# buq2/camera_calibrator

Hardware: AMD Instinct MI355X
Metric: LM residuals/sec (2*N_obs per LM iteration), single-camera intrinsics BA (higher is better)
Workload: dtype f64; 1 GPU; BASELINE.json configs[2]: single-camera intrinsics, 1000 frames x 500 pts per GPU, radial-tangential distortion, Zhang init, reference solver options (calibrator.cpp:314-321); frames_total=1000, points_per_frame=500, observations_total=500000, parallelism=frame-sharded x1, exchange=none

## Files before the change

### camera_calibrator_amd/capi.py

```python
import ctypes as C
import os

import numpy as np

_HERE = os.path.dirname(os.path.abspath(__file__))
LIB_PATH = os.environ.get("CC_LIB_PATH", os.path.join(_HERE, "libcc_hip.so"))

K_NAMES = ["sweep", "decide", "elim", "solve", "allreduce", "update", "reduce"]
TERMINATION = {0: "NO_CONVERGENCE", 1: "GRADIENT", 2: "PARAMETER", 3: "FUNCTION",
               4: "FAILURE_INVALID_STEPS", 5: "MIN_RADIUS", 6: "FAILURE_EXCHANGE"}


class CcError(RuntimeError):
    pass


class Options(C.Structure):
    _fields_ = [
        ("max_iterations", C.c_int32),
        ("use_nonmonotonic_steps", C.c_int32),
        ("max_consecutive_nonmonotonic_steps", C.c_int32),
        ("jacobi_scaling", C.c_int32),
        ("max_consecutive_invalid_steps", C.c_int32),
        ("check_interval", C.c_int32),
        ("function_tolerance", C.c_double),
        ("gradient_tolerance", C.c_double),
        ("parameter_tolerance", C.c_double),
        ("initial_radius", C.c_double),
        ("max_radius", C.c_double),
        ("min_radius", C.c_double),
        ("min_relative_decrease", C.c_double),
        ("min_lm_diagonal", C.c_double),
        ("max_lm_diagonal", C.c_double),
        ("use_graph", C.c_int32),
        ("profile_kernels", C.c_int32),
    ]


class Iteration(C.Structure):
    _fields_ = [
        ("cost", C.c_double),
        ("cost_change", C.c_double),
        ("model_cost_change", C.c_double),
        ("relative_decrease", C.c_double),
        ("gradient_max_norm", C.c_double),
        ("step_norm", C.c_double),
        ("radius", C.c_double),
        ("accepted", C.c_int32),
        ("valid", C.c_int32),
    ]


class IntrStartOptions(C.Structure):
    _fields_ = [
        ("centre", C.c_double * 2),
        ("theta_lo", C.c_double),
        ("theta_hi", C.c_double),
        ("candidates", C.c_int32),
        ("search_views", C.c_int32),
        ("refine_iterations", C.c_int32),
    ]


class IntrStartReport(C.Structure):
    _fields_ = [
        ("centre", C.c_double * 2),
        ("r_max", C.c_double),
        ("focal", C.c_double),
        ("best_candidate", C.c_int32),
        ("candidates_qualified", C.c_int32),
        ("views", C.c_int64),
        ("views_searched", C.c_int64),
        ("views_invalid", C.c_int64),
    ]


class Summary(C.Structure):
    _fields_ = [
        ("iterations", C.c_int32),
        ("successful_steps", C.c_int32),
        ("termination", C.c_int32),
        ("log_len", C.c_int32),
        ("initial_cost", C.c_double),
        ("final_cost", C.c_double),
        ("seconds", C.c_double),
        ("log", C.POINTER(Iteration)),
        ("log_capacity", C.c_int32),
        ("sweeps", C.c_int32),
        ("kernel_ms", C.c_double * 8),
        ("kernel_launches", C.c_int32 * 8),
        ("kernel_idle_ms", C.c_double * 8),
        ("kernel_idle_launches", C.c_int32 * 8),
    ]


EXPORTED_SYMBOLS = [
    "cc_options_init", "cc_last_error", "cc_version", "cc_device_count", "cc_release_caches", "cc_parallel_for", "cc_parallel_parts", "cc_host_pool_threads", "cc_last_call_solver_status",
    "cc_intrinsics_create", "cc_intrinsics_destroy", "cc_intrinsics_set_state",
    "cc_intrinsics_reset", "cc_intrinsics_get_state", "cc_intrinsics_eval",
    "cc_intrinsics_solve", "cc_intrinsics_solver_form", "cc_intrinsics_solver_status", "cc_intrinsics_profile_sweep", "cc_intrinsics_profile_solve", "cc_intrinsics_optimize", "cc_intrinsics_estimate", "cc_intrinsics_estimate_views", "cc_intrinsics_optimize_views", "cc_host_staging_acquire", "cc_host_staging_release", "cc_last_call_timing", "cc_comm_get_unique_id",
    "cc_intrinsics_comm_init", "cc_intrinsics_exchange_export", "cc_intrinsics_exchange_attach", "cc_partition_frames", "cc_distort", "cc_undistort",
    "cc_rig_create", "cc_rig_destroy", "cc_rig_set_state", "cc_rig_reset", "cc_rig_solve",
    "cc_rig_get_state", "cc_rig_solver_form", "cc_rig_solver_status", "cc_rig_eval", "cc_rig_optimize", "cc_rig_comm_init", "cc_rig_exchange_export", "cc_rig_exchange_attach", "cc_rigk_create",
    "cc_rigk_set_intrinsics", "cc_rigk_get_intrinsics", "cc_rigk_create_per_camera", "cc_rigk_set_camera_intrinsics",
    "cc_rigk_get_camera_intrinsics", "cc_rigk_set_model", "cc_rigk_get_model", "cc_rigk_set_camera_model", "cc_rigk_get_camera_model", "cc_rigk_estimate_start", "cc_rigk_start_points", "cc_rigk_estimate_start_bearing", "cc_rigk_start_bearings", "cc_zhang_init", "cc_intrinsics_optimize_multi", "cc_rig_optimize_multi", "cc_rig_optimize_frames", "cc_rig_optimize_columns",
    "cc_rig_set_inner_iterations", "cc_rig_inner_pass", "cc_rig_inner_status",
    "cc_rig_start_options_init", "cc_rig_estimate_start", "cc_rig_start_views", "cc_rig_estimate",
    "cc_intrinsics_batch_create", "cc_intrinsics_batch_destroy", "cc_intrinsics_batch_set_state", "cc_intrinsics_batch_get_state",
    "cc_intrinsics_batch_solve", "cc_intrinsics_batch_optimize", "cc_intrinsics_batch_estimate",
    "cc_intrinsics_set_huber", "cc_intrinsics_obs_cost", "cc_intrinsics_optimize_views_huber", "cc_intrinsics_estimate_views_huber",
    "cc_intrinsics_batch_set_huber", "cc_intrinsics_batch_estimate_huber",
    "cc_intrinsics_set_model", "cc_intrinsics_get_model", "cc_intrinsics_optimize_views_model", "cc_intrinsics_estimate_views_model",
    "cc_distort_fisheye", "cc_undistort_fisheye",
    "cc_intrinsics_batch_set_model", "cc_intrinsics_batch_get_model", "cc_intrinsics_batch_estimate_model",
    "cc_intr_start_options_init", "cc_intrinsics_estimate_start_fisheye", "cc_intrinsics_start_scores", "cc_intrinsics_estimate_views_start",
]
MODEL_RADTAN, MODEL_FISHEYE = 0, 1
MODEL_MIXED = 2
HARNESS_SYMBOLS = [
    "cc_generator_create", "cc_generator_destroy", "cc_generator_set_k", "cc_generator_set_distortion",
    "cc_generator_set_noise", "cc_generator_planar", "cc_generator_points", "cc_rig_scenario", "cc_affine_to_qt",
]

_lib = None


def lib():
    global _lib
    if _lib is None:
        if not os.path.exists(LIB_PATH):
            raise CcError(f"{LIB_PATH} is missing: build it with __graft_entry__.build() "
                          "(hipcc --offload-arch=gfx950); there is no CPU fallback")
        _lib = C.CDLL(LIB_PATH)
        _lib.cc_last_error.restype = C.c_char_p
        _lib.cc_version.restype = C.c_char_p
        _lib.cc_generator_create.restype = C.c_void_p
        _lib.cc_generator_planar.restype = C.c_int64
        _lib.cc_generator_points.restype = C.c_int64
    return _lib


def _check(rc):
    if rc != 0:
        raise CcError(f"cc error {rc}: {lib().cc_last_error().decode()}")


def _p(a, t):
    return a.ctypes.data_as(C.POINTER(t))


def _f32(a):
    return np.ascontiguousarray(a, dtype=np.float32)


def _f64(a):
    return np.ascontiguousarray(a, dtype=np.float64)


def default_options(**kw):
    o = Options()
    lib().cc_options_init(C.byref(o))
    for k, v in kw.items():
        if not hasattr(o, k):
            raise AttributeError(k)
        setattr(o, k, v)
    return o


def intr_start_options(**kw):
    o = IntrStartOptions()
    lib().cc_intr_start_options_init(C.byref(o))
    for k, v in kw.items():
        if not hasattr(o, k):
            raise AttributeError(k)
        if k == "centre":
            o.centre[0], o.centre[1] = float(v[0]), float(v[1])
        else:
            setattr(o, k, v)
    return o


def device_count():
    return int(lib().cc_device_count())


def partition_frames(frame_offsets, nranks):
    off = np.ascontiguousarray(frame_offsets, dtype=np.int64)
    first = np.zeros(nranks + 1, dtype=np.int64)
    _check(lib().cc_partition_frames(C.c_int64(len(off) - 1), _p(off, C.c_int64), C.c_int32(nranks),
                                     _p(first, C.c_int64)))
    return first


def _summary_dict(s, log):
    names = [f[0] for f in Iteration._fields_]
    return {
        "iterations": s.iterations, "successful_steps": s.successful_steps,
        "termination": TERMINATION.get(s.termination, str(s.termination)),
        "initial_cost": s.initial_cost, "final_cost": s.final_cost, "seconds": s.seconds,
        "sweeps": s.sweeps,
        "kernel_ms": {K_NAMES[i]: s.kernel_ms[i] for i in range(len(K_NAMES))},
        "kernel_launches": {K_NAMES[i]: s.kernel_launches[i] for i in range(len(K_NAMES))},
        "kernel_idle_ms": {K_NAMES[i]: s.kernel_idle_ms[i] for i in range(len(K_NAMES))},
        "kernel_idle_launches": {K_NAMES[i]: s.kernel_idle_launches[i] for i in range(len(K_NAMES))},
        "log": [{k: getattr(log[i], k) for k in names} for i in range(s.log_len)],
    }


class IntrinsicsProblem:

    def __init__(self, frame_offsets, uv, xyz, device=0):
        self._h = C.c_void_p()
        off = np.ascontiguousarray(frame_offsets, dtype=np.int64)
        self.n_frames = len(off) - 1
        self.n_obs = int(off[-1])
        uv, xyz = _f32(uv), _f32(xyz)
        assert uv.size == 2 * self.n_obs and xyz.size == 3 * self.n_obs
        _check(lib().cc_intrinsics_create(C.c_int32(device), C.c_int64(self.n_frames),
                                          _p(off, C.c_int64), _p(uv, C.c_float), _p(xyz, C.c_float),
                                          C.byref(self._h)))

    def close(self):
        if self._h:
            lib().cc_intrinsics_destroy(self._h)
            self._h = C.c_void_p()

    def __del__(self):
        try:
            self.close()
        except Exception:
            pass

    def set_state(self, intr, q, t, const_mask=0):
        intr, q, t = _f64(intr), _f64(q), _f64(t)
        assert intr.size == 9 and q.size == 4 * self.n_frames and t.size == 3 * self.n_frames
        _check(lib().cc_intrinsics_set_state(self._h, _p(intr, C.c_double), C.c_uint32(const_mask),
                                             _p(q, C.c_double), _p(t, C.c_double)))

    def reset(self):
        _check(lib().cc_intrinsics_reset(self._h))

    def get_state(self):
        intr = np.zeros(9)
        q = np.zeros((self.n_frames, 4))
        t = np.zeros((self.n_frames, 3))
        _check(lib().cc_intrinsics_get_state(self._h, _p(intr, C.c_double), _p(q, C.c_double),
                                             _p(t, C.c_double)))
        return intr, q, t

    def eval(self, want_blocks=True):
        blocks = np.zeros((self.n_frames, 16, 16)) if want_blocks else None
        cost = C.c_double()
        _check(lib().cc_intrinsics_eval(self._h, _p(blocks, C.c_double) if want_blocks else None,
                                        C.byref(cost)))
        return cost.value, blocks

    def solve(self, options=None, log_capacity=1024):
        opt = options if options is not None else default_options()
        log = (Iteration * max(1, log_capacity))()
        s = Summary()
        s.log = C.cast(log, C.POINTER(Iteration))
        s.log_capacity = log_capacity
        _check(lib().cc_intrinsics_solve(self._h, C.byref(opt), C.byref(s)))
        return _summary_dict(s, log)

    def solve_lean(self, options):
        s = getattr(self, "_lean_summary", None)
        if s is None:
            s = self._lean_summary = Summary()
            s.log = None
            s.log_capacity = 0
        _check(lib().cc_intrinsics_solve(self._h, C.byref(options), C.byref(s)))
        return s.iterations

    def set_huber(self, a):
        _check(lib().cc_intrinsics_set_huber(self._h, C.c_double(a)))

    def set_model(self, model):
        _check(lib().cc_intrinsics_set_model(self._h, C.c_int32(model)))

    def get_model(self):
        return int(lib().cc_intrinsics_get_model(self._h))

    def obs_cost(self):
        out = np.zeros(self.n_obs)
        _check(lib().cc_intrinsics_obs_cost(self._h, _p(out, C.c_double)))
        return out

    def estimate_start_fisheye(self, **options):
        o = intr_start_options(**options)
        intr, q, t = np.zeros(9), np.zeros((self.n_frames, 4)), np.zeros((self.n_frames, 3))
        r = IntrStartReport()
        _check(lib().cc_intrinsics_estimate_start_fisheye(self._h, C.byref(o), _p(intr, C.c_double), _p(q, C.c_double),
                                                          _p(t, C.c_double), C.byref(r)))
        report = {k: getattr(r, k) for k, _ in IntrStartReport._fields_ if k != "centre"}
        report["centre"] = (r.centre[0], r.centre[1])
        return intr, q, t, report

    def start_scores(self):
        f, score, qualified = np.zeros(64), np.zeros(64), np.full(64, -1, dtype=np.int32)
        _check(lib().cc_intrinsics_start_scores(self._h, _p(f, C.c_double), _p(score, C.c_double), _p(qualified, C.c_int32)))
        n = int((qualified >= 0).sum())
        return f[:n].copy(), score[:n].copy(), qualified[:n].copy()

    def profile_sweep(self, n=50):
        ms = C.c_double()
        _check(lib().cc_intrinsics_profile_sweep(self._h, C.c_int32(n), C.byref(ms)))
        return ms.value

    def solver_form(self):
        return int(lib().cc_intrinsics_solver_form(self._h))

    def solver_status(self):
        form, reruns = C.c_int32(), C.c_int32()
        note = C.create_string_buffer(2048)
        _check(lib().cc_intrinsics_solver_status(self._h, C.byref(form), C.byref(reruns), note, 2048))
        return form.value, reruns.value, note.value.decode()

    def profile_solve(self, options=None, n=20):
        options = options if options is not None else default_options()
        ms, sw = C.c_double(), C.c_int32()
        _check(lib().cc_intrinsics_profile_solve(self._h, C.byref(options), C.c_int32(n), C.byref(ms), C.byref(sw)))
        return ms.value, sw.value

    def comm_init(self, unique_id, rank, nranks):
        buf = (C.c_uint8 * 128).from_buffer_copy(bytes(unique_id))
        _check(lib().cc_intrinsics_comm_init(self._h, buf, C.c_int32(rank), C.c_int32(nranks)))

    def exchange_export(self):
        buf = (C.c_uint8 * 64)()
        _check(lib().cc_intrinsics_exchange_export(self._h, buf))
        return bytes(buf)

    def exchange_attach(self, rank, handles):
        blob = b"".join(bytes(x) for x in handles)
        assert len(blob) == 64 * len(handles)
        buf = (C.c_uint8 * len(blob)).from_buffer_copy(blob)
        _check(lib().cc_intrinsics_exchange_attach(self._h, C.c_int32(rank), C.c_int32(len(handles)), buf))


def comm_get_unique_id():
    buf = (C.c_uint8 * 128)()
    _check(lib().cc_comm_get_unique_id(buf))
    return bytes(buf)


def _views(off, uv, xyz):
    F = len(off) - 1
    parts_uv = [np.array(uv.reshape(-1, 2)[off[f]:off[f + 1]], dtype=np.float32, order="C") for f in range(F)]
    parts_xyz = [np.array(xyz.reshape(-1, 3)[off[f]:off[f + 1]], dtype=np.float32, order="C") for f in range(F)]
    fp = C.POINTER(C.c_float)
    uv_views = (fp * F)(*[a.ctypes.data_as(fp) for a in parts_uv])
    xyz_views = (fp * F)(*[a.ctypes.data_as(fp) for a in parts_xyz])
    counts = np.ascontiguousarray(np.diff(off), dtype=np.int64)
    return uv_views, xyz_views, counts, (parts_uv, parts_xyz)


def intrinsics_optimize(frame_offsets, uv, xyz, intr, q, t, const_mask=0, options=None, device=0,
                        log_capacity=1024, devices=None, views=False, huber_a=0.0, model=0):
    off = np.ascontiguousarray(frame_offsets, dtype=np.int64)
    F = len(off) - 1
    uv, xyz = _f32(uv), _f32(xyz)
    intr, q, t = _f64(intr).copy(), _f64(q).copy(), _f64(t).copy()
    opt = options if options is not None else default_options()
    log = (Iteration * max(1, log_capacity))()
    s = Summary()
    s.log = C.cast(log, C.POINTER(Iteration))
    s.log_capacity = log_capacity
    if model != 0:
        if devices is not None:
            raise ValueError("model is for one device only")
        uv_views, xyz_views, counts, _keep = _views(off, uv, xyz)
        _check(lib().cc_intrinsics_optimize_views_model(C.byref(opt), C.c_int32(device), C.c_int64(F), uv_views, xyz_views,
                                                        _p(counts, C.c_int64), _p(intr, C.c_double), C.c_uint32(const_mask),
                                                        _p(q, C.c_double), _p(t, C.c_double), C.byref(s), C.c_double(huber_a),
                                                        C.c_int32(model)))
        return intr, q, t, _summary_dict(s, log)
    if not huber_a <= 0:
        if devices is not None:
            raise ValueError("huber_a is for one device only")
        uv_views, xyz_views, counts, _keep = _views(off, uv, xyz)
        _check(lib().cc_intrinsics_optimize_views_huber(C.byref(opt), C.c_int32(device), C.c_int64(F), uv_views, xyz_views,
                                                        _p(counts, C.c_int64), _p(intr, C.c_double), C.c_uint32(const_mask),
                                                        _p(q, C.c_double), _p(t, C.c_double), C.byref(s), C.c_double(huber_a)))
        return intr, q, t, _summary_dict(s, log)
    if devices is not None:
        devs = np.ascontiguousarray(devices, dtype=np.int32)
        _check(lib().cc_intrinsics_optimize_multi(C.byref(opt), C.c_int32(len(devs)), _p(devs, C.c_int32), C.c_int64(F),
                                                  _p(off, C.c_int64), _p(uv, C.c_float), _p(xyz, C.c_float),
                                                  _p(intr, C.c_double), C.c_uint32(const_mask),
                                                  _p(q, C.c_double), _p(t, C.c_double), C.byref(s)))
        return intr, q, t, _summary_dict(s, log)
    if views:
        uv_views, xyz_views, counts, _keep = _views(off, uv, xyz)
        _check(lib().cc_intrinsics_optimize_views(C.byref(opt), C.c_int32(device), C.c_int64(F), uv_views, xyz_views,
                                                  _p(counts, C.c_int64), _p(intr, C.c_double), C.c_uint32(const_mask),
                                                  _p(q, C.c_double), _p(t, C.c_double), C.byref(s)))
        return intr, q, t, _summary_dict(s, log)
    _check(lib().cc_intrinsics_optimize(C.byref(opt), C.c_int32(device), C.c_int64(F),
                                        _p(off, C.c_int64), _p(uv, C.c_float), _p(xyz, C.c_float),
                                        _p(intr, C.c_double), C.c_uint32(const_mask),
                                        _p(q, C.c_double), _p(t, C.c_double), C.byref(s)))
    return intr, q, t, _summary_dict(s, log)


def intrinsics_estimate(frame_offsets, uv, xyz, distortion5=None, const_mask=0, options=None, device=0, log_capacity=1024,
                        views=False, huber_a=0.0, model=0, start="zhang", start_options=None):
    if start not in ("zhang", "fisheye"):
        raise ValueError(f"start must be 'zhang' or 'fisheye', not {start!r}")
    if start == "zhang" and start_options is not None:
        raise ValueError("start_options belong to start='fisheye'")
    off = np.ascontiguousarray(frame_offsets, dtype=np.int64)
    F = len(off) - 1
    uv, xyz = _f32(uv), _f32(xyz)
    opt = options if options is not None else default_options()
    log = (Iteration * max(1, log_capacity))()
    s = Summary()
    s.log = C.cast(log, C.POINTER(Iteration))
    s.log_capacity = log_capacity
    K = np.zeros(9, dtype=np.float32)
    intr, q, t = np.zeros(9), np.zeros((F, 4)), np.zeros((F, 3))
    d5 = _f64(distortion5) if distortion5 is not None else None
    if start == "fisheye":
        so = start_options if isinstance(start_options, IntrStartOptions) else intr_start_options(**(start_options or {}))
        uv_views, xyz_views, counts, _keep = _views(off, uv, xyz)
        _check(lib().cc_intrinsics_estimate_views_start(C.byref(opt), C.c_int32(device), C.c_int64(F), uv_views, xyz_views,
                                                        _p(counts, C.c_int64), _p(d5, C.c_double) if d5 is not None else None,
                                                        C.c_uint32(const_mask), _p(K, C.c_float), _p(intr, C.c_double),
                                                        _p(q, C.c_double), _p(t, C.c_double), C.byref(s), C.c_double(huber_a),
                                                        C.c_int32(model), C.byref(so)))
        return K.reshape(3, 3), intr, q, t, _summary_dict(s, log)
    if model != 0:
        uv_views, xyz_views, counts, _keep = _views(off, uv, xyz)
        _check(lib().cc_intrinsics_estimate_views_model(C.byref(opt), C.c_int32(device), C.c_int64(F), uv_views, xyz_views,
                                                        _p(counts, C.c_int64), _p(d5, C.c_double) if d5 is not None else None,
                                                        C.c_uint32(const_mask), _p(K, C.c_float), _p(intr, C.c_double),
                                                        _p(q, C.c_double), _p(t, C.c_double), C.byref(s), C.c_double(huber_a),
                                                        C.c_int32(model)))
        return K.reshape(3, 3), intr, q, t, _summary_dict(s, log)
    if not huber_a <= 0:
        uv_views, xyz_views, counts, _keep = _views(off, uv, xyz)
        _check(lib().cc_intrinsics_estimate_views_huber(C.byref(opt), C.c_int32(device), C.c_int64(F), uv_views, xyz_views,
                                                        _p(counts, C.c_int64), _p(d5, C.c_double) if d5 is not None else None,
                                                        C.c_uint32(const_mask), _p(K, C.c_float), _p(intr, C.c_double),
                                                        _p(q, C.c_double), _p(t, C.c_double), C.byref(s), C.c_double(huber_a)))
        return K.reshape(3, 3), intr, q, t, _summary_dict(s, log)
    if views:
        uv_views, xyz_views, counts, _keep = _views(off, uv, xyz)
        _check(lib().cc_intrinsics_estimate_views(C.byref(opt), C.c_int32(device), C.c_int64(F), uv_views, xyz_views,
                                                  _p(counts, C.c_int64), _p(d5, C.c_double) if d5 is not None else None,
                                                  C.c_uint32(const_mask), _p(K, C.c_float), _p(intr, C.c_double),
                                                  _p(q, C.c_double), _p(t, C.c_double), C.byref(s)))
        return K.reshape(3, 3), intr, q, t, _summary_dict(s, log)
    _check(lib().cc_intrinsics_estimate(C.byref(opt), C.c_int32(device), C.c_int64(F), _p(off, C.c_int64), _p(uv, C.c_float),
                                        _p(xyz, C.c_float), _p(d5, C.c_double) if d5 is not None else None,
                                        C.c_uint32(const_mask), _p(K, C.c_float), _p(intr, C.c_double), _p(q, C.c_double),
                                        _p(t, C.c_double), C.byref(s)))
    return K.reshape(3, 3), intr, q, t, _summary_dict(s, log)


def _batch_layout(problems):
    poff, foff, uvs, xyzs = [0], [0], [], []
    for off, uv, xyz in problems:
        off = np.ascontiguousarray(off, dtype=np.int64)
        uv, xyz = _f32(uv).reshape(-1, 2), _f32(xyz).reshape(-1, 3)
        assert off[0] == 0 and len(uv) == off[-1] and len(xyz) == off[-1]
        foff.extend((off[1:] + foff[-1]).tolist())
        poff.append(poff[-1] + len(off) - 1)
        uvs.append(uv)
        xyzs.append(xyz)
    uv = np.ascontiguousarray(np.concatenate(uvs), dtype=np.float32) if uvs else np.zeros((0, 2), np.float32)
    xyz = np.ascontiguousarray(np.concatenate(xyzs), dtype=np.float32) if xyzs else np.zeros((0, 3), np.float32)
    return np.array(poff, dtype=np.int64), np.array(foff, dtype=np.int64), uv, xyz


def _batch_summaries(B, log_capacity):
    logs = [(Iteration * max(1, log_capacity))() for _ in range(B)]
    ss = (Summary * B)()
    for p in range(B):
        ss[p].log = C.cast(logs[p], C.POINTER(Iteration))
        ss[p].log_capacity = log_capacity
    return ss, logs


class IntrinsicsBatch:

    def __init__(self, problems, device=0):
        self._h = C.c_void_p()
        self.problem_offsets, self.frame_offsets, uv, xyz = _batch_layout(problems)
        self.n_problems = len(self.problem_offsets) - 1
        self.n_frames = int(self.problem_offsets[-1])
        _check(lib().cc_intrinsics_batch_create(C.c_int32(device), C.c_int64(self.n_problems), _p(self.problem_offsets, C.c_int64),
                                                _p(self.frame_offsets, C.c_int64), _p(uv, C.c_float), _p(xyz, C.c_float),
                                                C.byref(self._h)))

    def close(self):
        if self._h:
            lib().cc_intrinsics_batch_destroy(self._h)
            self._h = C.c_void_p()

    def __del__(self):
        try:
            self.close()
        except Exception:
            pass

    def _split(self, a, width):
        a = a.reshape(-1, width)
        return [a[self.problem_offsets[p]:self.problem_offsets[p + 1]].copy() for p in range(self.n_problems)]

    def set_state(self, intr, q, t, const_mask=None):
        intr = _f64(np.asarray(intr, dtype=np.float64).reshape(-1))
        q = _f64(np.concatenate([np.asarray(x, dtype=np.float64).reshape(-1, 4) for x in q]) if isinstance(q, (list, tuple)) else q)
        t = _f64(np.concatenate([np.asarray(x, dtype=np.float64).reshape(-1, 3) for x in t]) if isinstance(t, (list, tuple)) else t)
        assert intr.size == 9 * self.n_problems and q.size == 4 * self.n_frames and t.size == 3 * self.n_frames
        mask = np.zeros(self.n_problems, dtype=np.uint32) if const_mask is None else np.ascontiguousarray(const_mask, dtype=np.uint32)
        assert mask.size == self.n_problems
        _check(lib().cc_intrinsics_batch_set_state(self._h, _p(intr, C.c_double), _p(mask, C.c_uint32), _p(q, C.c_double),
                                                   _p(t, C.c_double)))

    def set_huber(self, a_list):
        if a_list is None:
            _check(lib().cc_intrinsics_batch_set_huber(self._h, None))
            return
        a = _f64(np.asarray(a_list, dtype=np.float64).reshape(-1))
        assert a.size == self.n_problems
        _check(lib().cc_intrinsics_batch_set_huber(self._h, _p(a, C.c_double)))

    def set_model(self, model):
        _check(lib().cc_intrinsics_batch_set_model(self._h, C.c_int32(model)))

    def get_model(self):
        model = C.c_int32(-1)
        _check(lib().cc_intrinsics_batch_get_model(self._h, C.byref(model)))
        return int(model.value)

    def get_state(self):
        intr = np.zeros((self.n_problems, 9))
        q = np.zeros((self.n_frames, 4))
        t = np.zeros((self.n_frames, 3))
        _check(lib().cc_intrinsics_batch_get_state(self._h, _p(intr, C.c_double), _p(q, C.c_double), _p(t, C.c_double)))
        return intr, self._split(q, 4), self._split(t, 3)

    def solve(self, options=None, log_capacity=1024):
        opt = options if options is not None else default_options()
        ss, logs = _batch_summaries(self.n_problems, log_capacity)
        _check(lib().cc_intrinsics_batch_solve(self._h, C.byref(opt), ss))
        return [_summary_dict(ss[p], logs[p]) for p in range(self.n_problems)]

    def solve_lean(self, options):
        ss = getattr(self, "_lean", None)
        if ss is None:
            ss = self._lean = (Summary * self.n_problems)()
        _check(lib().cc_intrinsics_batch_solve(self._h, C.byref(options), ss))
        return [ss[p].iterations for p in range(self.n_problems)]


def intrinsics_batch_optimize(problems, intr, q, t, const_mask=None, options=None, device=0, log_capacity=1024, model=0):
    if model != 0:
        h = IntrinsicsBatch(problems, device=device)
        try:
            h.set_model(model)
            h.set_state(intr, q, t, const_mask)
            ss = h.solve(options, log_capacity)
            io, qs, ts = h.get_state()
        finally:
            h.close()
        return io, qs, ts, ss
    poff, foff, uv, xyz = _batch_layout(problems)
    B = len(poff) - 1
    intr = _f64(np.asarray(intr, dtype=np.float64).reshape(-1)).copy()
    q = _f64(np.concatenate([np.asarray(x, dtype=np.float64).reshape(-1, 4) for x in q])).copy()
    t = _f64(np.concatenate([np.asarray(x, dtype=np.float64).reshape(-1, 3) for x in t])).copy()
    mask = np.zeros(B, dtype=np.uint32) if const_mask is None else np.ascontiguousarray(const_mask, dtype=np.uint32)
    opt = options if options is not None else default_options()
    ss, logs = _batch_summaries(B, log_capacity)
    _check(lib().cc_intrinsics_batch_optimize(C.byref(opt), C.c_int32(device), C.c_int64(B), _p(poff, C.c_int64), _p(foff, C.c_int64),
                                              _p(uv, C.c_float), _p(xyz, C.c_float), _p(intr, C.c_double), _p(mask, C.c_uint32),
                                              _p(q, C.c_double), _p(t, C.c_double), ss))
# ... 551 lines not shown
```

### camera_calibrator_amd/csrc/cc_intrinsics.hip

```cpp
#include "cc_common.hpp"
#include "cc_device.hpp"
#include "cc_intrinsics_dev.hpp"
#include "cc_intrinsics_persist.hpp"


#include <algorithm>
#include <chrono>
#include <climits>
#include <cstdlib>
#include <cstring>
#include <vector>

namespace cc {

__global__ __launch_bounds__(kSweepThreads, 4) void k_intr_sweep(IntrDev P, int flags) {
  extern __shared__ __attribute__((aligned(16))) char smem_raw[];
  double* s_stage = reinterpret_cast<double*>(smem_raw);
  double* s_blk = s_stage;
  double* sm = s_stage + 4 * kStageDoublesPerWave;
  const int tid = threadIdx.x, lane = tid & 63, wave = tid >> 6;
  const int T = P.T;
  const int64_t f = (int64_t)blockIdx.x / T;
  const int tile = (int)(blockIdx.x - f * T);
  const bool in_solve = (flags & 1) != 0, restart = (flags & 2) != 0;
// ... 488 lines not shown
      }
#pragma unroll
      for (int u = 0; u < 16; ++u) Gs[u * 256 + tid] = a[u];
      __syncthreads();
    }
    const double* Gl = Gs + g * 256;
    auto gsum = [&](int idx) { return T > 1 ? Gl[idx] : G[idx]; };
    double fail = 0.0;
    double gv[5];
#pragma unroll
    for (int r = 0; r < 5; ++r) gv[r] = gsum(gi[r]);
    const double gpe = gsum((9 + l6) * 16 + 15);
    const double* qf = P.pose + ((size_t)cur * P.F + (valid ? f : 0)) * 8;
    const double qw = qf[0], qx = qf[1], qy = qf[2], qz = qf[3];
    const int col = l < 9 ? l : 15;
    double w[6];
#pragma unroll
    for (int i = 0; i < 6; ++i) w[i] = gsum((9 + i) * 16 + col);
    if (valid) {
      double s[6], L[21];
#pragma unroll
      for (int i = 0; i < 6; ++i)
#pragma unroll
        for (int j = 0; j <= i; ++j) L[tri(i, j)] = gsum((9 + i) * 16 + 9 + j);
      if (phase == 0) {
#pragma unroll
        for (int i = 0; i < 6; ++i) s[i] = jac ? 1.0 / (1.0 + sqrt(L[tri(i, i)])) : 1.0;
        if (l < 6) P.sp[f * 8 + l] = jac ? 1.0 / (1.0 + sqrt(gsum((9 + l) * 17))) : 1.0;
      } else {
#pragma unroll
        for (int i = 0; i < 6; ++i) s[i] = P.sp[f * 8 + i];
      }
#pragma unroll
      for (int i = 0; i < 6; ++i)
#pragma unroll
        for (int j = 0; j <= i; ++j) L[tri(i, j)] = s[i] * L[tri(i, j)] * s[j];
#pragma unroll
      for (int i = 0; i < 6; ++i) L[tri(i, i)] += clampd(L[tri(i, i)], mn, mx) * inv_radius;
      bool ok = true;
      double Li[6];
#pragma unroll
      for (int j = 0; j < 6; ++j) {
        double d = L[tri(j, j)];
#pragma unroll
        for (int k = 0; k < j; ++k) d -= L[tri(j, k)] * L[tri(j, k)];
        ok = ok && (d > 0.0) && isfinite(d);
        const double inv = rsqrt_pos(d);
        L[tri(j, j)] = d * inv;
        Li[j] = inv;
#pragma unroll
        for (int i = j + 1; i < 6; ++i) {
          double a = L[tri(i, j)];
#pragma unroll
          for (int k = 0; k < j; ++k) a -= L[tri(i, k)] * L[tri(j, k)];
          L[tri(i, j)] = a * inv;
        }
      }
      if (!ok) fail = 1.0;
      if (l < 10) {
        const double sc = l < 9 ? s_ss[l] : 1.0;
        double z[6], y[6];
#pragma unroll
        for (int i = 0; i < 6; ++i) {
          double a = s[i] * w[i] * sc;
#pragma unroll
          for (int k = 0; k < i; ++k) a -= L[tri(i, k)] * z[k];
          z[i] = a * Li[i];
        }
#pragma unroll
        for (int i = 5; i >= 0; --i) {
          double a = z[i];
#pragma unroll
          for (int k = i + 1; k < 6; ++k) a -= L[tri(k, i)] * y[k];
          y[i] = a * Li[i];
        }
#pragma unroll
        for (int i = 0; i < 6; ++i) {
          Zs[g][i * 10 + l] = z[i];
          P.Y[f * kYStride + i * 10 + l] = y[i];
        }
      }
    }
    __syncthreads();
    if (valid) {
#pragma unroll
      for (int r = 0; r < 5; ++r) {
        double zz = 0.0;
#pragma unroll
        for (int i = 0; i < 6; ++i) zz += Zs[g][i * 10 + zj[r]] * Zs[g][i * 10 + zk[r]];
        acc[r] += sa[r] * gv[r] * sb[r] - (use_z[r] ? zz : 0.0);
      }
      {
        const int base16 = (threadIdx.x & 63) & ~15;
        double g6[6];
#pragma unroll
        for (int i = 0; i < 6; ++i) g6[i] = __shfl(gpe, base16 + i, 64);
        const double q4[4] = {qw, qx, qy, qz};
        gacc = fmax(gacc, pose_grad_proj_max(q4, g6));
      }
      facc += fail;
    }
    __syncthreads();
  }
#pragma unroll
  for (int r = 0; r < 5; ++r)
    if (l * 5 + r != PC_FAIL && l * 5 + r != PC_GMAXP) red[g][l * 5 + r] = acc[r];
  gacc = row16_max(gacc);
  if (l == 0) { red[g][PC_FAIL] = facc; red[g][PC_GMAXP] = gacc; }
  __syncthreads();
  if (tid < kPartialCols) {
    double a = 0.0;
    if (tid == PC_GMAXP) { for (int g2 = 0; g2 < 16; ++g2) a = fmax(a, red[g2][tid]); }
    else { for (int g2 = 0; g2 < 16; ++g2) a += red[g2][tid]; }
    if (kFused)
      __hip_atomic_store(reinterpret_cast<unsigned long long*>(P.partial) + blockIdx.x * kPartialCols + tid,
                         (unsigned long long)__double_as_longlong(a), __ATOMIC_RELAXED, __HIP_MEMORY_SCOPE_AGENT);
    else
      P.partial[blockIdx.x * kPartialCols + tid] = a;
  }
  }
  if (!kFused) return;

  asm volatile("s_waitcnt vmcnt(0)" ::: "memory");
  __syncthreads();
  if (tid == 0) {
    const unsigned prev = __hip_atomic_fetch_add(P.arrive, 1u, __ATOMIC_RELAXED, __HIP_MEMORY_SCOPE_AGENT);
    s_last = prev + 1u == gridDim.x;
  }
  __syncthreads();
  if (!s_last) return;
  if (tid == 0) __hip_atomic_store(P.arrive, 0u, __ATOMIC_RELAXED, __HIP_MEMORY_SCOPE_AGENT);
  double* sv = &red[0][0];
  double* s_part = &red[2][0];
  if (!stop) {
    const bool active = true;
    {
      const int col = tid % kPartialCols, grp = tid / kPartialCols;
      const int nblk = (int)gridDim.x;
      if (grp < 3) {
        const unsigned long long* src = reinterpret_cast<const unsigned long long*>(P.partial) + col;
        double v[22];
#pragma unroll
        for (int u = 0; u < 22; ++u) {
          const int b = grp + 3 * u;
          v[u] = b < nblk ? __longlong_as_double((long long)__hip_atomic_load(src + b * kPartialCols, __ATOMIC_RELAXED, __HIP_MEMORY_SCOPE_AGENT)) : 0.0;
        }
        double a = 0.0;
        if (col == PC_GMAXP) {
#pragma unroll
          for (int u = 0; u < 22; ++u) a = fmax(a, v[u]);
        } else {
#pragma unroll
          for (int u = 0; u < 22; ++u) a += v[u];
        }
        s_part[grp * kPartialCols + col] = a;
      }
    }
    __syncthreads();
    if (tid < kVecSolve) {
      double a = 0.0;
      if (tid < kPartialCols) {
        if (tid != PC_GMAXP) a = (s_part[tid] + s_part[kPartialCols + tid]) + s_part[2 * kPartialCols + tid];
      } else if (tid == kPartialCols + P.rank) {
        a = fmax(fmax(s_part[PC_GMAXP], s_part[kPartialCols + PC_GMAXP]), s_part[2 * kPartialCols + PC_GMAXP]);
      }
      sv[tid] = a;
    }
    __syncthreads();
    if (MODE == 3 && active) {
      __shared__ int s_ok2;
      const unsigned long long epoch = P.x.seq[0] + 1ull;
      p2p_post(P.x, 0, epoch, P.rank, P.nranks, sv, kVecSolve);
      const double a = p2p_collect(P.x, 0, epoch, P.rank, P.nranks, kVecSolve, &s_ok2);
      exchange_ok = s_ok2 != 0;
      if (tid < kVecSolve) sv[tid] = exchange_ok ? a : 0.0;
      if (tid == 0) P.x.seq[0] = epoch;
      __syncthreads();
    }
  }
  if (tid != 0) return;
  LmCtl c = s_ctl;
  cc_iteration* e = s_logged ? &s_log : nullptr;
  if (!exchange_ok) { c.done = 1; c.term = CC_FAILURE_EXCHANGE; }
  else if (!stop) intr_solve_step(P, sv, c, e, o_in);
  if (publish == 2) return;
  if (e && c.log_len <= P.log_cap) P.log[c.log_len - 1] = *e;
  *P.ctl = c;
  *P.ctl_next = c;
  if (publish) publish_to_host(P, c);
}

constexpr int kSolveThreads = 8 * kPartialCols;

template <int MODE>
__global__ __launch_bounds__(kSolveThreads) void k_intr_solve(IntrDev P, int nblk, int publish) {
  static_assert(MODE == 1 || MODE == 2, "single-GPU and mailbox solves are fused into k_intr_decide_elim");
  __shared__ double sv[kVecSolve];
  __shared__ double s_part[8][kPartialCols];
  const int tid = threadIdx.x;
  const LmCtl* cn = P.ctl_next;
  const bool active = !cn->done && cn->phase != 0;
  if (MODE == 1) {
    const int col = tid % kPartialCols, grp = tid / kPartialCols;
    double v[8];
#pragma unroll
    for (int u = 0; u < 8; ++u) {
      const int b = grp + 8 * u;
      v[u] = b < nblk ? P.partial[b * kPartialCols + col] : 0.0;
    }
    double a = 0.0;
    if (active) {
      if (col == PC_GMAXP) a = fmax(fmax(fmax(v[0], v[1]), fmax(v[2], v[3])), fmax(fmax(v[4], v[5]), fmax(v[6], v[7])));
      else a = ((v[0] + v[1]) + (v[2] + v[3])) + ((v[4] + v[5]) + (v[6] + v[7]));
    }
    s_part[grp][col] = a;
    if (tid >= kPartialCols && tid < kVecSolve) sv[tid] = 0.0;
    __syncthreads();
    if (tid < kPartialCols) {
      double a2 = 0.0;
      if (tid == PC_GMAXP) {
        if (active) for (int g2 = 0; g2 < 8; ++g2) a2 = fmax(a2, s_part[g2][tid]);
        sv[kPartialCols + P.rank] = a2;
        sv[tid] = 0.0;
      } else {
        if (active)
          a2 = ((s_part[0][tid] + s_part[1][tid]) + (s_part[2][tid] + s_part[3][tid])) +
               ((s_part[4][tid] + s_part[5][tid]) + (s_part[6][tid] + s_part[7][tid]));
        sv[tid] = a2;
      }
    }
    __syncthreads();
    if (tid < kVecSolve) P.vec_solve[tid] = sv[tid];
    return;
  }
  if (tid < kVecSolve) sv[tid] = P.vec_solve[tid];
  __syncthreads();
  if (tid != 0) return;
  LmCtl c = *cn;
  if (active) {
    cc_iteration* e = (c.log_len > 0 && c.log_len <= P.log_cap) ? &P.log[c.log_len - 1] : nullptr;
    cc_iteration rec;
    if (e) rec = *e;
    const LmOpts o = *P.opts;
    intr_solve_step(P, sv, c, e ? &rec : nullptr, o);
    if (e && rec.accepted) e->gradient_max_norm = rec.gradient_max_norm;
  }
  *P.ctl = c;
  *P.ctl_next = c;
  if (publish) publish_to_host(P, c);
}

__global__ __launch_bounds__(64) void k_intr_flag_exchange(IntrDev P, double mine, double* out, int* ok) {
  __shared__ double s_post[16];
  __shared__ int s_ok;
  const int tid = threadIdx.x;
  if (tid < 16) s_post[tid] = tid == 0 ? mine : 0.0;
  __syncthreads();
  const unsigned long long epoch = P.x.seq[1] + 1ull;
  p2p_post(P.x, 1, epoch, P.rank, P.nranks, s_post, 16);
  const double a = p2p_collect(P.x, 1, epoch, P.rank, P.nranks, 16, &s_ok);
  if (tid == 0) { *out = a; P.x.seq[1] = epoch; *ok = s_ok; }
}

__global__ __launch_bounds__(256) void k_intr_reset(IntrDev P, const double* init_intr, const double* init_pose) {
  const int64_t i = (int64_t)blockIdx.x * blockDim.x + threadIdx.x;
  if (i < P.F * 8) P.pose[i] = init_pose[i];
  if (i < 16) P.intr[i] = init_intr[i];
  if (i < (int64_t)(sizeof(LmCtl) / sizeof(double))) {
    reinterpret_cast<double*>(P.ctl)[i] = 0.0;
    reinterpret_cast<double*>(P.ctl_next)[i] = 0.0;
  }
  if (i == 0) *P.arrive = 0u;
}

}

#include "cc_intrinsics_huber.hpp"
#include "cc_intrinsics_fisheye.hpp"

#include "cc_solve_host.hpp"

struct cc_intrinsics : cc::SolveHost {
  cc::IntrDev d{};
  int64_t F = 0, N = 0;
  int elim_blocks = 1;
  void* arena = nullptr;
  bool arena_cached = false;
  size_t extra_bytes = 0;
  char* extra = nullptr;
  bool one_shot = false;
  bool no_obs_upload = false;
  double* init_intr = nullptr;
  double* init_pose = nullptr;
  bool have_state = false;
  cc::LmOpts* h_opts = nullptr;
  bool ctl_fresh = false;
  bool reset_pending = false;
  bool persist_ok = false;
  bool persist_x_ok = false;
  int p_resident = 0;
  cc::PersistDev pq{};
  uint32_t p_epoch = 0;
  size_t p_box_bytes = 0;
  double huber_a = 0.0;
  int model = CC_MODEL_RADTAN;
  void* start_work = nullptr;
  size_t start_work_bytes = 0;
  int start_candidates = 0;
  const double* start_srec = nullptr;
  const double* start_view = nullptr;
  int64_t start_searched = 0;
  bool start_marks = false;
  bool own_sweep() const { return huber_a > 0.0 || model != CC_MODEL_RADTAN; }
};

namespace cc {

static void exchange_release(cc_intrinsics* h) {
  mailbox_release(&h->mailbox);
  h->d.x = P2pDev{};
  h->exchange = false;
}

static void launch_sweep(cc_intrinsics* h, bool profile, int flags = 0) {
  Probe p(h, CC_K_SWEEP, profile);
  flags |= 4;
  if (h->model == CC_MODEL_FISHEYE)
    hipLaunchKernelGGL(k_intr_sweep_fisheye, dim3((unsigned)(h->F * h->d.T)), dim3(kSweepThreads), kSweepLdsBytes, h->stream, h->d, flags, h->huber_a);
  else if (h->huber_a > 0.0)
    hipLaunchKernelGGL(k_intr_sweep_huber, dim3((unsigned)(h->F * h->d.T)), dim3(kSweepThreads), kSweepLdsBytes, h->stream, h->d, flags, h->huber_a);
  else
    hipLaunchKernelGGL(k_intr_sweep, dim3((unsigned)(h->F * h->d.T)), dim3(kSweepThreads), kSweepLdsBytes, h->stream, h->d, flags);
}

static void launch_reset(cc_intrinsics* h) {
  const unsigned blocks = (unsigned)((h->F * 8 + 255) / 256);
  hipLaunchKernelGGL(k_intr_reset, dim3(blocks), dim3(256), 0, h->stream, h->d, h->init_intr, h->init_pose);
}

static int enqueue_round(cc_intrinsics* h, bool profile, bool initial, bool publish, bool restart = false) {
  const int pub = (publish ? 1 : 0) | (restart ? 4 : 0);
  const int sweep_flags = 1 | (restart ? 2 : 0);
  struct RoundCount { cc_intrinsics* h; ~RoundCount() { h->enq_round++; } } count_round{h};
  if (h->comm) {
    if (!initial) {
      { Probe p(h, CC_K_SOLVE, profile, -1); hipLaunchKernelGGL(k_intr_solve<1>, dim3(1), dim3(kSolveThreads), 0, h->stream, h->d, h->elim_blocks, 0); }
      { Probe p(h, CC_K_ALLREDUCE, profile, -1); if (int rc = comm_allreduce_sum(h->comm, h->d.vec_solve, kVecSolve, h->stream)) return rc; }
      { Probe p(h, CC_K_SOLVE, profile, -1); hipLaunchKernelGGL(k_intr_solve<2>, dim3(1), dim3(kSolveThreads), 0, h->stream, h->d, h->elim_blocks, 0); }
    }
    launch_sweep(h, profile, 1);
    { Probe p(h, CC_K_DECIDE, profile); hipLaunchKernelGGL(k_intr_stats_reduce, dim3(1), dim3(256), 0, h->stream, h->d); }
    { Probe p(h, CC_K_ALLREDUCE, profile); if (int rc = comm_allreduce_sum(h->comm, h->d.vec_decide, 16, h->stream)) return rc; }
    { Probe p(h, CC_K_ELIM, profile); hipLaunchKernelGGL(k_intr_decide_elim<2>, dim3(h->elim_blocks), dim3(256), 0, h->stream, h->d, 0); }
    return 0;
  }
  launch_sweep(h, profile, sweep_flags);
  Probe p(h, CC_K_ELIM, profile);
  if (h->exchange) hipLaunchKernelGGL(k_intr_decide_elim<3>, dim3(h->elim_blocks), dim3(256), 0, h->stream, h->d, pub);
  else hipLaunchKernelGGL(k_intr_decide_elim<0>, dim3(h->elim_blocks), dim3(256), 0, h->stream, h->d, pub);
  return 0;
}

static int flush_reset(cc_intrinsics* h) {
  if (!h->reset_pending) return 0;
  launch_reset(h);
  CC_HIP(hipGetLastError());
  h->reset_pending = false;
  return 0;
}

static int read_ctl(cc_intrinsics* h, LmCtl* c) {
  if (int rc = flush_reset(h)) return rc;
  CC_HIP(hipMemcpyAsync(h->h_ctl, h->d.ctl_next, sizeof(LmCtl), hipMemcpyDeviceToHost, h->stream));
  CC_HIP(hipStreamSynchronize(h->stream));
  *c = *h->h_ctl;
  return 0;
}

static int wait_chunk(cc_intrinsics* h, LmCtl* c) {
  return wait_published(h, nullptr, c, nullptr, "the solver", [=] { return read_ctl(h, c); });
}

static int wait_solve(cc_intrinsics* h, LmCtl* c) {
  return wait_published_tagged(h, c, "the solver", [=] { return read_ctl(h, c); });
}

}

namespace cc {
int intr_create_impl(cc_intrinsics* h, const int64_t* off, const float* uv, const float* xyz);
static thread_local bool g_create_one_shot = false;
static thread_local bool g_create_no_obs = false;
static thread_local size_t g_create_extra = 0;
struct OneShotCreate {
  OneShotCreate(size_t extra, bool no_obs = false) { g_create_one_shot = true; g_create_extra = extra; g_create_no_obs = no_obs; }
  ~OneShotCreate() { g_create_one_shot = false; g_create_extra = 0; g_create_no_obs = false; }
};
static double ms_since(std::chrono::steady_clock::time_point t0) { return std::chrono::duration<double, std::milli>(std::chrono::steady_clock::now() - t0).count(); }
}

extern "C" {

void cc_intrinsics_destroy(cc_intrinsics* h);

int cc_intrinsics_create(int32_t device, int64_t F, const int64_t* off, const float* uv,
                         const float* xyz, cc_intrinsics** out) {
  using namespace cc;
  if (!out || !off || F <= 0) return fail(CC_ERR_BAD_ARGUMENT, "cc_intrinsics_create: bad arguments");
  if (off[0] != 0) return fail(CC_ERR_BAD_ARGUMENT, "frame_offsets[0] must be 0");
  for (int64_t f = 0; f < F; ++f)
    if (off[f + 1] < off[f]) return fail(CC_ERR_BAD_ARGUMENT, "frame_offsets must be non-decreasing");
  const int64_t N = off[F];
  if (F >= ((int64_t)1 << 28) || N >= ((int64_t)1 << 40))
    return fail(CC_ERR_BAD_ARGUMENT, "cc_intrinsics_create: problem too large (frames < 2^28, observations < 2^40)");
  if (N > 0 && (!uv || !xyz) && !cc::g_create_no_obs) return fail(CC_ERR_BAD_ARGUMENT, "uv/xyz are NULL");
  if (int rc = select_device(device)) return rc;
  cc_intrinsics* h = new cc_intrinsics();
  h->device = device; h->F = F; h->N = N;
  h->one_shot = cc::g_create_one_shot;
  h->no_obs_upload = cc::g_create_no_obs;
  h->extra_bytes = cc::g_create_extra;
  const int rc_init = cc::intr_create_impl(h, off, uv, xyz);
  if (rc_init != CC_OK) {
    cc_intrinsics_destroy(h);
    return rc_init;
  }
  *out = h;
  return CC_OK;
}

int cc_intrinsics_exchange_export(cc_intrinsics* h, uint8_t handle[64]) {
  using namespace cc;
  if (h && handle && h->huber_a > 0.0) return fail(CC_ERR_STATE, "cc_intrinsics_exchange_export: the handle has a Huber loss set (one device only)");
  if (h && handle && h->model != CC_MODEL_RADTAN) return fail(CC_ERR_STATE, "cc_intrinsics_exchange_export: the handle has the fisheye model set (one device only)");
  if (int rc = exchange_export_begin(h, handle, "cc_intrinsics_exchange_export")) return rc;
  h->d.x = P2pDev{};
  return mailbox_export(&h->mailbox, kVecSolve, 16, handle);
}

int cc_intrinsics_exchange_attach(cc_intrinsics* h, int32_t rank, int32_t nranks, const uint8_t* handles) {
  using namespace cc;
  if (!h || !handles || rank < 0 || nranks < 1 || rank >= nranks || nranks > kP2pMaxRanks)
    return fail(CC_ERR_BAD_ARGUMENT, "cc_intrinsics_exchange_attach: bad arguments (nranks must be 1..%d)", kP2pMaxRanks);
  if (h->huber_a > 0.0) return fail(CC_ERR_STATE, "cc_intrinsics_exchange_attach: the handle has a Huber loss set (one device only)");
  if (h->model != CC_MODEL_RADTAN) return fail(CC_ERR_STATE, "cc_intrinsics_exchange_attach: the handle has the fisheye model set (one device only)");
  if (!h->mailbox.local) return fail(CC_ERR_STATE, "cc_intrinsics_exchange_attach: call cc_intrinsics_exchange_export first");
  if (h->comm) return fail(CC_ERR_STATE, "cc_intrinsics_exchange_attach: an RCCL communicator is already attached");
  CC_HIP(hipSetDevice(h->device));
  drop_graphs(h);
  if (int rc = mailbox_attach(&h->mailbox, rank, nranks, handles, &h->d.x)) return rc;
  h->d.rank = rank;
  h->d.nranks = nranks;
  h->exchange = true;
  h->persist_x_ok = false;
  if (h->persist_ok) {
    int ndev = 1;
    if (hipGetDeviceCount(&ndev) != hipSuccess || ndev < 1) ndev = 1;
    const int co = getenv("CC_INTR_CO_RESIDENT") ? std::max(1, atoi(getenv("CC_INTR_CO_RESIDENT"))) : (nranks + ndev - 1) / ndev;
    h->persist_x_ok = (int64_t)(h->pq.G + 1) * co <= h->p_resident;
  }
  if (nranks > 1) {
    double* d_out = nullptr;
    int* d_ok = nullptr;
    CC_HIP(hipMalloc(&d_out, sizeof(double)));
    CC_HIP(hipMalloc(&d_ok, sizeof(int)));
    hipLaunchKernelGGL(k_intr_flag_exchange, dim3(1), dim3(64), 0, h->stream, h->d, h->persist_x_ok ? 1.0 : 0.0, d_out, d_ok);
    double sum = 0.0;
    int ok = 0;
    const hipError_t e1 = hipMemcpyAsync(&sum, d_out, sizeof(double), hipMemcpyDeviceToHost, h->stream);
    const hipError_t e2 = hipMemcpyAsync(&ok, d_ok, sizeof(int), hipMemcpyDeviceToHost, h->stream);
    const hipError_t e3 = hipStreamSynchronize(h->stream);
    hipFree(d_out);
    hipFree(d_ok);
    CC_HIP(e1); CC_HIP(e2); CC_HIP(e3);
    if (!ok) return fail(CC_ERR_COMM, "cc_intrinsics_exchange_attach: a peer rank did not attach within 10 s");
    h->persist_x_ok = sum == (double)nranks;
  }
  return CC_OK;
}

}

namespace cc {
int intr_create_impl(cc_intrinsics* h, const int64_t* off, const float* uv, const float* xyz) {
  const int64_t F = h->F, N = h->N;
  if (int rc = stream_get(h->device, &h->stream)) return rc;
  IntrDev& d = h->d;
  d.F = F; d.N = N; d.rank = 0; d.nranks = 1; d.mask = 0;
  {
    const int64_t per_frame = F > 0 ? (N + F - 1) / F : 0;
    int64_t T = std::min<int64_t>((per_frame + 2 * kSweepThreads - 1) / (2 * kSweepThreads), 256 / std::max<int64_t>(F, 1));
    if (const char* env = getenv("CC_SWEEP_TILES")) T = atoi(env);
    d.T = (int32_t)std::max<int64_t>(1, std::min<int64_t>(T, 8));
    d.tpad_ = 0;
    if (F * d.T >= (int64_t)INT32_MAX)
      return fail(CC_ERR_BAD_ARGUMENT, "cc_intrinsics_create: %lld frames x %d sweep tiles exceed the launch grid", (long long)F, (int)d.T);
  }
  const size_t FT = (size_t)F * d.T;
  const size_t n1 = (size_t)std::max<int64_t>(N, 1);
  size_t cursor = 0;
  auto take = [&](size_t bytes) { const size_t at = cursor; cursor += (bytes + 255) & ~(size_t)255; return at; };
  d.log_cap = 4096;
  const size_t o_intr = take(2 * 16 * sizeof(double));
  const size_t o_pose = take((size_t)2 * F * 8 * sizeof(double));
  const size_t o_stats = take(FT * kStatsCols * sizeof(double));
  const size_t o_hd0 = take(FT * 16 * sizeof(double));
  const size_t o_sp = take((size_t)F * 8 * sizeof(double));
  const size_t o_Y = take((size_t)F * kYStride * sizeof(double));
  const size_t o_partial = take((size_t)kElimMaxBlocks * kPartialCols * sizeof(double));
  const size_t o_vs = take(kVecSolve * sizeof(double));
  const size_t o_vd = take(16 * sizeof(double));
  const size_t o_ds = take(16 * sizeof(double));
  const size_t o_ss = take(16 * sizeof(double));
  const size_t o_ctl = take(sizeof(LmCtl));
  const size_t o_ctln = take(sizeof(LmCtl));
  const size_t o_sync = take(64);
  const size_t o_opts = take(sizeof(LmOpts));
  const size_t o_iintr = take(16 * sizeof(double));
  const size_t o_ipose = take((size_t)F * 8 * sizeof(double));
  int p_teams = 0;
  const bool want_persist = d.T == 1 && !(getenv("CC_INTR_PERSIST") && atoi(getenv("CC_INTR_PERSIST")) == 0);
  if (want_persist) {
    for (int t = 1; t <= kPMaxTeams && !p_teams; t *= 2) {
      int resident = 0;
      if (int rc = persist_resident_workgroups(h->device, t, &resident)) return rc;
      if ((F + t - 1) / t + 1 <= resident && (F + t - 1) / t <= kPMaxWorkers) { p_teams = t; h->p_resident = resident; }
    }
    if (const char* e = getenv("CC_INTR_PERSIST_TEAMS")) {
      const int t = atoi(e);
      int resident = 0;
      if ((t == 1 || t == 2 || t == 4) && !persist_resident_workgroups(h->device, t, &resident) && (F + t - 1) / t + 1 <= resident && (F + t - 1) / t <= kPMaxWorkers) { p_teams = t; h->p_resident = resident; }
    }
  }
  const int64_t PG = p_teams ? (F + p_teams - 1) / p_teams : 1;
  const size_t pgn = (size_t)PG;
  const size_t o_pbox0 = cursor;
  const size_t o_sbox = take(pgn * 2 * kPStatCols * sizeof(unsigned long long));
  const size_t o_pbox = take(pgn * 2 * kPartialCols * sizeof(unsigned long long));
  const size_t o_rbox = take(pgn * 2 * kPartialCols * sizeof(unsigned long long));
  const size_t o_lbox = take((size_t)2 * kPartialCols * sizeof(unsigned long long));
  const size_t o_xbox = take(kPBcastWords * sizeof(unsigned long long));
  const size_t o_pfail = take(64);
  h->p_box_bytes = cursor - o_pbox0;
  const size_t zeroed = cursor;
  const size_t o_blocks = take((size_t)2 * FT * 256 * sizeof(double));
  const size_t o_log = take((size_t)d.log_cap * sizeof(cc_iteration));
  const size_t o_uv = take(n1 * 2 * sizeof(float));
  const size_t o_xyz = take(n1 * 3 * sizeof(float));
  const size_t o_off = take((size_t)(F + 1) * sizeof(int64_t));
  const size_t o_extra = take(h->extra_bytes);
  if (int rc = arena_get(h->device, cursor, &h->arena, &h->arena_cached)) return rc;
  char* base = static_cast<char*>(h->arena);
  h->extra = h->extra_bytes ? base + o_extra : nullptr;
  CC_HIP(hipMemsetAsync(base, 0, zeroed, h->stream));
  if (N > 0 && !h->no_obs_upload) {
    CC_HIP(hipMemcpyAsync(base + o_uv, uv, (size_t)N * 2 * sizeof(float), hipMemcpyHostToDevice, h->stream));
    CC_HIP(hipMemcpyAsync(base + o_xyz, xyz, (size_t)N * 3 * sizeof(float), hipMemcpyHostToDevice, h->stream));
  }
  CC_HIP(hipMemcpyAsync(base + o_off, off, (size_t)(F + 1) * sizeof(int64_t), hipMemcpyHostToDevice, h->stream));
  if (!h->one_shot) CC_HIP(hipStreamSynchronize(h->stream));
  d.uv = reinterpret_cast<const float*>(base + o_uv);
  d.xyz = reinterpret_cast<const float*>(base + o_xyz);
  d.off = reinterpret_cast<const int64_t*>(base + o_off);
  d.intr = reinterpret_cast<double*>(base + o_intr);
  d.pose = reinterpret_cast<double*>(base + o_pose);
  d.blocks = reinterpret_cast<double*>(base + o_blocks);
  d.stats = reinterpret_cast<double*>(base + o_stats);
  d.hd0 = reinterpret_cast<double*>(base + o_hd0);
  d.sp = reinterpret_cast<double*>(base + o_sp);
  d.Y = reinterpret_cast<double*>(base + o_Y);
  d.partial = reinterpret_cast<double*>(base + o_partial);
  d.vec_solve = reinterpret_cast<double*>(base + o_vs);
  d.vec_decide = reinterpret_cast<double*>(base + o_vd);
  d.ds = reinterpret_cast<double*>(base + o_ds);
  d.ss = reinterpret_cast<double*>(base + o_ss);
  d.ctl = reinterpret_cast<LmCtl*>(base + o_ctl);
  d.ctl_next = reinterpret_cast<LmCtl*>(base + o_ctln);
  d.arrive = reinterpret_cast<unsigned*>(base + o_sync);
  d.pub_seq = reinterpret_cast<unsigned long long*>(base + o_sync + 8);
  d.opts = reinterpret_cast<LmOpts*>(base + o_opts);
  d.log = reinterpret_cast<cc_iteration*>(base + o_log);
  h->init_intr = reinterpret_cast<double*>(base + o_iintr);
  h->init_pose = reinterpret_cast<double*>(base + o_ipose);
  d.init_intr = h->init_intr;
  d.init_pose = h->init_pose;
  static_assert(16 + sizeof(LmCtl) <= 192 && sizeof(LmCtl) <= 160 && sizeof(LmOpts) <= 160, "one cached 512-byte pinned block holds all three");
  h->pinned = pinned_block_get();
  if (!h->pinned) return fail(CC_ERR_HIP, "hipHostMalloc failed");
  h->host_pub = reinterpret_cast<volatile unsigned long long*>(h->pinned);
  h->h_ctl = reinterpret_cast<LmCtl*>(static_cast<char*>(h->pinned) + 192);
  h->h_opts = reinterpret_cast<LmOpts*>(static_cast<char*>(h->pinned) + 352);
  h->host_pub[0] = 0ull;
  static_assert((kPubTaggedAt + kPubWords) * 8 <= (int)kPinnedBlockBytes && kPubTaggedAt * 8 >= 512, "the tagged publication lies behind the three blocks");
  for (int i = 0; i < kPubWords; ++i) h->host_pub[kPubTaggedAt + i] = 0ull;
  h->pub_count = 0;
  {
    void* dev_view = nullptr;
    CC_HIP(hipHostGetDevicePointer(&dev_view, h->pinned, 0));
    d.host_pub = reinterpret_cast<unsigned long long*>(dev_view);
  }
  h->pq.sbox = reinterpret_cast<unsigned long long*>(base + o_sbox);
  h->pq.pbox = reinterpret_cast<unsigned long long*>(base + o_pbox);
  h->pq.rbox = reinterpret_cast<unsigned long long*>(base + o_rbox);
  h->pq.xbox = reinterpret_cast<unsigned long long*>(base + o_xbox);
  h->pq.fail = reinterpret_cast<unsigned*>(base + o_pfail);
  h->pq.lbox = reinterpret_cast<unsigned long long*>(base + o_lbox);
  h->pq.G = (int32_t)PG;
  h->pq.teams = p_teams;
  h->p_epoch = 0;
  h->persist_ok = p_teams != 0;
  h->elim_blocks = (int)std::min<int64_t>(kElimMaxBlocks, (F + 15) / 16);
  CC_HIP(hipFuncSetAttribute(reinterpret_cast<const void*>(k_intr_sweep),
                             hipFuncAttributeMaxDynamicSharedMemorySize, kSweepLdsBytes));
  CC_HIP(hipFuncSetAttribute(reinterpret_cast<const void*>(k_intr_sweep_huber),
                             hipFuncAttributeMaxDynamicSharedMemorySize, kSweepLdsBytes));
  CC_HIP(hipFuncSetAttribute(reinterpret_cast<const void*>(k_intr_sweep_fisheye),
                             hipFuncAttributeMaxDynamicSharedMemorySize, kSweepLdsBytes));
  return CC_OK;
}
}

extern "C" {

void cc_intrinsics_destroy(cc_intrinsics* h) {
  if (h) cc::last_call_status_record(h->ran_form >= 0 ? h->ran_form : cc_intrinsics_solver_form(h), h->form_reruns, h->form_note);
  if (!h) return;
  hipSetDevice(h->device);
  bool stream_ok = true;
  if (h->stream) {
    hipStreamCaptureStatus cap = hipStreamCaptureStatusNone;
    stream_ok = hipStreamSynchronize(h->stream) == hipSuccess &&
                hipStreamIsCapturing(h->stream, &cap) == hipSuccess && cap == hipStreamCaptureStatusNone;
    (void)hipGetLastError();
  }
  cc::drop_graphs(h);
  for (auto e : h->events) hipEventDestroy(e);
  if (h->comm) cc::comm_destroy(h->comm);
  cc::exchange_release(h);
  if (h->start_work) (void)hipFree(h->start_work);
  if (h->arena) cc::arena_put(h->device, h->arena, h->arena_cached);
  cc::pinned_block_put(h->pinned);
  if (stream_ok) cc::stream_put(h->device, h->stream);
  else if (h->stream) hipStreamDestroy(h->stream);
  delete h;
}

int cc_intrinsics_set_state(cc_intrinsics* h, const double* intr9, uint32_t mask, const double* q,
                            const double* t) {
  using namespace cc;
  if (!h || !intr9 || !q || !t) return fail(CC_ERR_BAD_ARGUMENT, "cc_intrinsics_set_state: NULL argument");
  CC_HIP(hipSetDevice(h->device));
  std::vector<double> pose((size_t)h->F * 8, 0.0);
  for (int64_t f = 0; f < h->F; ++f) {
    for (int i = 0; i < 4; ++i) pose[f * 8 + i] = q[f * 4 + i];
    for (int i = 0; i < 3; ++i) pose[f * 8 + 4 + i] = t[f * 3 + i];
  }
  double k[16] = {0};
  for (int i = 0; i < 9; ++i) k[i] = intr9[i];
  if (h->model == CC_MODEL_FISHEYE) { k[8] = 0.0; mask |= 1u << 8; }
  CC_HIP(hipStreamSynchronize(h->stream));
  CC_HIP(hipMemcpy(h->init_intr, k, sizeof(k), hipMemcpyHostToDevice));
  CC_HIP(hipMemcpy(h->init_pose, pose.data(), pose.size() * sizeof(double), hipMemcpyHostToDevice));
  if (h->d.mask != (mask & 0x1ffu)) drop_graphs(h);
  h->d.mask = mask & 0x1ffu;
  h->have_state = true;
  return cc_intrinsics_reset(h);
}

int cc_intrinsics_reset(cc_intrinsics* h) {
  using namespace cc;
  if (!h || !h->have_state) return fail(CC_ERR_STATE, "cc_intrinsics_reset: no state set");
  h->ctl_fresh = true;
  h->reset_pending = true;
  return CC_OK;
}

int cc_intrinsics_get_state(cc_intrinsics* h, double* intr9, double* q, double* t) {
  using namespace cc;
  if (!h) return fail(CC_ERR_BAD_ARGUMENT, "cc_intrinsics_get_state: NULL handle");
  CC_HIP(hipSetDevice(h->device));
  LmCtl c;
  if (int rc = read_ctl(h, &c)) return rc;
  const int cur = c.cur & 1;
  if (intr9) CC_HIP(hipMemcpy(intr9, h->d.intr + cur * 16, 9 * sizeof(double), hipMemcpyDeviceToHost));
  if (q || t) {
    std::vector<double> pose((size_t)h->F * 8);
    CC_HIP(hipMemcpy(pose.data(), h->d.pose + (size_t)cur * h->F * 8, pose.size() * sizeof(double), hipMemcpyDeviceToHost));
    for (int64_t f = 0; f < h->F; ++f) {
      if (q) for (int i = 0; i < 4; ++i) q[f * 4 + i] = pose[f * 8 + i];
      if (t) for (int i = 0; i < 3; ++i) t[f * 3 + i] = pose[f * 8 + 4 + i];
    }
  }
  return CC_OK;
}

int cc_intrinsics_eval(cc_intrinsics* h, double* blocks, double* cost) {
  using namespace cc;
  if (!h || !h->have_state) return fail(CC_ERR_STATE, "cc_intrinsics_eval: no state set");
  CC_HIP(hipSetDevice(h->device));
  LmCtl st;
  if (int rc = read_ctl(h, &st)) return rc;
  h->ctl_fresh = false;
  LmCtl ev{};
  ev.cur = st.cur & 1;
  CC_HIP(hipMemcpyAsync(h->d.ctl, &ev, sizeof(ev), hipMemcpyHostToDevice, h->stream));
  launch_sweep(h, false);
  CC_HIP(hipGetLastError());
  CC_HIP(hipMemcpyAsync(h->d.ctl, &st, sizeof(st), hipMemcpyHostToDevice, h->stream));
  CC_HIP(hipStreamSynchronize(h->stream));
  const int cur = st.cur & 1;
  const int64_t T = h->d.T, FT = h->F * T;
  if (blocks) {
    if (T == 1) {
      CC_HIP(hipMemcpy(blocks, h->d.blocks + (size_t)cur * h->F * 256, (size_t)h->F * 256 * sizeof(double), hipMemcpyDeviceToHost));
    } else {
      std::vector<double> tiles((size_t)FT * 256);
      CC_HIP(hipMemcpy(tiles.data(), h->d.blocks + (size_t)cur * FT * 256, tiles.size() * sizeof(double), hipMemcpyDeviceToHost));
      for (int64_t f = 0; f < h->F; ++f)
        for (int i = 0; i < 256; ++i) {
          double a = tiles[(size_t)(f * T) * 256 + i];
          for (int64_t k = 1; k < T; ++k) a += tiles[(size_t)(f * T + k) * 256 + i];
          blocks[(size_t)f * 256 + i] = a;
        }
    }
  }
  if (cost) {
    std::vector<double> stats((size_t)FT * kStatsCols);
    CC_HIP(hipMemcpy(stats.data(), h->d.stats, stats.size() * sizeof(double), hipMemcpyDeviceToHost));
    double c = 0.0;
    for (int64_t f = 0; f < FT; ++f) c += stats[f * kStatsCols + ST_COST];
    *cost = c;
  }
  return CC_OK;
}

int cc_intrinsics_set_huber(cc_intrinsics* h, double a_pixels) {
  using namespace cc;
  if (!h) return fail(CC_ERR_BAD_ARGUMENT, "cc_intrinsics_set_huber: NULL handle");
  if (a_pixels != a_pixels) return fail(CC_ERR_BAD_ARGUMENT, "cc_intrinsics_set_huber: a_pixels is NaN");
  if (h->exchange || h->comm || h->mailbox.local)
    return fail(CC_ERR_STATE, "cc_intrinsics_set_huber: the handle has an exchange or a communicator attached (the loss is for one device only)");
  const double a = a_pixels > 0.0 ? a_pixels : 0.0;
  if (a != h->huber_a) drop_graphs(h);
  h->huber_a = a;
  return CC_OK;
}

int cc_intrinsics_set_model(cc_intrinsics* h, int32_t model) {
  using namespace cc;
  if (!h) return fail(CC_ERR_BAD_ARGUMENT, "cc_intrinsics_set_model: NULL handle");
  if (model != CC_MODEL_RADTAN && model != CC_MODEL_FISHEYE) return fail(CC_ERR_BAD_ARGUMENT, "cc_intrinsics_set_model: unknown model %d", (int)model);
  if (model != CC_MODEL_RADTAN && (h->exchange || h->comm || h->mailbox.local))
    return fail(CC_ERR_STATE, "cc_intrinsics_set_model: the handle has an exchange or a communicator attached (the fisheye model is for one device only)");
  if (model == h->model) return CC_OK;
  drop_graphs(h);
  h->model = model;
  h->have_state = false;
  return CC_OK;
}

int32_t cc_intrinsics_get_model(cc_intrinsics* h) { return h ? h->model : CC_MODEL_RADTAN; }

int cc_intrinsics_obs_cost(cc_intrinsics* h, double* obs_cost) {
  using namespace cc;
  if (!h || !obs_cost) return fail(CC_ERR_BAD_ARGUMENT, "cc_intrinsics_obs_cost: NULL argument");
  if (!h->have_state) return fail(CC_ERR_STATE, "cc_intrinsics_obs_cost: no state set");
  if (h->N == 0) return CC_OK;
  CC_HIP(hipSetDevice(h->device));
  LmCtl st;
  if (int rc = read_ctl(h, &st)) return rc;
  const int64_t cost_blocks = (h->N + 255) / 256;
  if (cost_blocks > (int64_t)INT32_MAX) return fail(CC_ERR_BAD_ARGUMENT, "cc_intrinsics_obs_cost: %lld observations exceed the launch grid", (long long)h->N);
  double* d_out = nullptr;
  CC_HIP(hipMalloc(&d_out, (size_t)h->N * sizeof(double)));
  if (h->model == CC_MODEL_FISHEYE)
    hipLaunchKernelGGL(k_intr_obs_cost_fisheye, dim3((unsigned)cost_blocks), dim3(256), 0, h->stream, h->d, st.cur & 1, h->huber_a, d_out);
  else
    hipLaunchKernelGGL(k_intr_obs_cost, dim3((unsigned)cost_blocks), dim3(256), 0, h->stream, h->d, st.cur & 1, h->huber_a, d_out);
  hipError_t e = hipGetLastError();
  if (e == hipSuccess) e = hipMemcpyAsync(obs_cost, d_out, (size_t)h->N * sizeof(double), hipMemcpyDeviceToHost, h->stream);
  if (e == hipSuccess) e = hipStreamSynchronize(h->stream);
  hipFree(d_out);
  CC_HIP(e);
  return CC_OK;
}

}

namespace cc {
static int capture_chunk(cc_intrinsics* h, bool with_reset, bool initial, int rounds, hipGraphExec_t* out) {
  return capture_graph(h, out, [=] {
    int rc = 0;
    for (int i = 0; i < rounds && !rc; ++i) rc = enqueue_round(h, false, initial && i == 0, i == rounds - 1, with_reset && i == 0);
    return rc;
  });
}
}

namespace cc {
struct SolveRun : SolveRunBase {
  bool host_word = false;
};

static int solve_begin(cc_intrinsics* h, const cc_options* opt, SolveRun* r) {
  if (int rc = begin_common(h, opt, h->d.log_cap, r)) return rc;
  r->host_word = !h->comm;
  if (!h->ctl_fresh) {
    LmCtl st;
    if (int rc = read_ctl(h, &st)) return rc;
    if (st.cur & 1) {
      CC_HIP(hipMemcpyAsync(h->d.intr, h->d.intr + 16, 16 * sizeof(double), hipMemcpyDeviceToDevice, h->stream));
      CC_HIP(hipMemcpyAsync(h->d.pose, h->d.pose + (size_t)h->F * 8, (size_t)h->F * 8 * sizeof(double), hipMemcpyDeviceToDevice, h->stream));
    }
    LmCtl c{};
    if (int rc = write_ctl(h, c)) return rc;
    CC_HIP(hipMemsetAsync(h->d.arrive, 0, sizeof(unsigned), h->stream));
  }
  h->ctl_fresh = false;
  LmOpts lo;
  opts_from_public(r->o, &lo);
  if (opts_changed(h, lo)) {
    CC_HIP(hipStreamSynchronize(h->stream));
    *h->h_opts = lo;
    CC_HIP(hipMemcpyAsync(h->d.opts, h->h_opts, sizeof(lo), hipMemcpyHostToDevice, h->stream));
    h->opts_valid = true;
  }
  return 0;
}

static int solve_launch(cc_intrinsics* h, SolveRun* r, int chunk) {
  const cc_options& o = r->o;
  CC_HIP(hipSetDevice(h->device));
  const int n = o.check_interval + (chunk == 0 ? 1 : 0);
  if (r->use_graph) {
    const int which = chunk > 0 ? 1 : (h->reset_pending ? 0 : 2);
    if (!h->graph[which]) {
      const int rounds = o.check_interval + (which == 1 ? 0 : 1);
      if (int rc = capture_chunk(h, which == 0, which != 1, rounds, &h->graph[which])) { drop_graphs(h); return rc; }
    }
    CC_HIP(hipGraphLaunch(h->graph[which], h->stream));
    h->reset_pending = false;
  } else {
    const bool restart = chunk == 0 && h->reset_pending && !h->comm;
    if (restart) h->reset_pending = false;
    else if (int rc = flush_reset(h)) return rc;
    for (int i = 0; i < n; ++i)
      if (int rc = enqueue_round(h, r->profile, chunk == 0 && i == 0, i == n - 1, restart && i == 0)) return rc;
    CC_HIP(hipGetLastError());
  }
  r->launched += n;
  return 0;
}

static int solve_wait(cc_intrinsics* h, SolveRun* r) {
  CC_HIP(hipSetDevice(h->device));
  if (int rc = r->host_word ? wait_chunk(h, &r->st) : read_ctl(h, &r->st)) return rc;
  if (r->st.done && r->st.term == CC_FAILURE_EXCHANGE) {
    (void)hipStreamSynchronize(h->stream);
    const std::string where = h->exchange ? mailbox_describe(&h->mailbox, h->d.rank, h->d.nranks) : std::string();
    return fail(CC_ERR_COMM, "mailbox exchange timed out: a peer rank did not post within 10 s (iteration %d). %s", r->st.iter, where.c_str());
  }
  if (!r->st.done && r->launched > r->o.max_iterations + 2 * r->o.check_interval + 2)
    return fail(CC_ERR_STATE, "LM loop did not terminate (iter=%d)", r->st.iter);
  return 0;
}

static bool use_persistent(const cc_intrinsics* h, const SolveRun* r) {
  return !h->comm && !r->profile && !h->own_sweep() && (h->exchange ? h->persist_x_ok : h->persist_ok);
}

static int persistent_launch(cc_intrinsics* h, SolveRun* r) {
  CC_HIP(hipSetDevice(h->device));
  PersistDev q = h->pq;
  q.max_rounds = r->o.max_iterations + 2;
  q.restart = h->reset_pending ? 1 : 0;
  const uint32_t need = 3u * (uint32_t)q.max_rounds + 3u;
  if (h->p_epoch > 0xf0000000u - need) {
    CC_HIP(hipMemsetAsync(h->pq.sbox, 0, h->p_box_bytes, h->stream));
    h->p_epoch = 0;
  }
  q.epoch0 = h->p_epoch;
  h->p_epoch += need;
  q.timeout_shift = h->exchange ? 30 : 27;
  q.first_shift = h->exchange ? 30 : 20;
  static int drop_left = -2;
  const bool drop_control = !h->exchange && persist_test_drop_control("CC_INTR_PERSIST_TEST_NO_CONTROL", &drop_left);
  persist_launch(h->d, q, drop_control, h->stream);
  CC_HIP(hipGetLastError());
  h->reset_pending = false;
  r->launched = q.max_rounds;
  return 0;
}

static int persistent_wait(cc_intrinsics* h, SolveRun* r) {
  CC_HIP(hipSetDevice(h->device));
  if (int rc = wait_solve(h, &r->st)) return rc;
  if (r->st.done && r->st.term == CC_FAILURE_EXCHANGE) {
    CC_HIP(hipMemsetAsync(h->pq.fail, 0, sizeof(unsigned), h->stream));
    (void)hipStreamSynchronize(h->stream);
    const std::string where = h->exchange ? mailbox_describe(&h->mailbox, h->d.rank, h->d.nranks) : std::string();
    return fail(CC_ERR_COMM, "persistent solve: a wait inside the kernel timed out (iteration %d): its %d workgroups were not all "
                "resident, or a peer rank did not post within 10 s. %s", r->st.iter, h->pq.G + 1, where.c_str());
  }
  if (!r->st.done) {
    unsigned failed = 0;
    CC_HIP(hipStreamSynchronize(h->stream));
    CC_HIP(hipMemcpy(&failed, h->pq.fail, sizeof(failed), hipMemcpyDeviceToHost));
    if (failed) {
      CC_HIP(hipMemsetAsync(h->pq.fail, 0, sizeof(unsigned), h->stream));
      return fail(CC_ERR_COMM, "persistent solve: the workers' waits timed out and the control workgroup never ran (%d workgroups not all resident)", h->pq.G + 1);
    }
    return fail(CC_ERR_STATE, "persistent solve ended without a result (iter=%d)", r->st.iter);
  }
  return 0;
}

static int persistent_log_settled(cc_intrinsics* h, const cc_summary* summary) {
  if (summary && summary->log && summary->log_capacity > 0) CC_HIP(hipStreamSynchronize(h->stream));
  return 0;
}

static int solve_persistent(cc_intrinsics* h, SolveRun* r) {
  std::unique_lock<std::mutex> lk(persist_mutex(h->device), std::defer_lock);
  if (!h->exchange && !h->comm) lk.lock();
  if (int rc = persistent_launch(h, r)) return rc;
  return persistent_wait(h, r);
}

}

extern "C" {

int cc_intrinsics_solve(cc_intrinsics* h, const cc_options* opt, cc_summary* summary) {
  using namespace cc;
  if (!h || !h->have_state) return fail(CC_ERR_STATE, "cc_intrinsics_solve: no state set");
  SolveRun r;
  if (int rc = solve_begin(h, opt, &r)) return rc;
  const bool alone = !h->exchange && !h->comm;
  if (use_persistent(h, &r) && (!alone || persist_device_try(h->device, 0))) {
    const bool was_restart = h->reset_pending;
    PersistProbe probe(h->device, 0, alone);
    const int rc = solve_persistent(h, &r);
    if (rc == CC_OK) {
      probe.completed();
      h->ran_form = h->pq.teams;
      if (int rc2 = persistent_log_settled(h, summary)) return rc2;
      return finish_summary(h, &r, summary);
    }
    probe.gave_up();
    if (rc != CC_ERR_COMM || h->exchange) return rc;
    h->persist_ok = false;
    h->form_reruns++;
    h->form_note = last_error() + "; the solve was run again with two kernels per iteration and the handle stays on that form";
    CC_HIP(hipStreamSynchronize(h->stream));
    CC_HIP(hipMemsetAsync(h->pq.fail, 0, sizeof(unsigned), h->stream));
    if (was_restart) {
      h->reset_pending = true;
    } else {
      LmCtl zero{};
      if (int rc2 = write_ctl(h, zero)) return rc2;
      CC_HIP(hipMemsetAsync(h->d.arrive, 0, sizeof(unsigned), h->stream));
    }
    h->ctl_fresh = true;
    if (int rc2 = solve_begin(h, opt, &r)) return rc2;
  }
  for (int chunk = 0;; ++chunk) {
    if (int rc = solve_launch(h, &r, chunk)) return rc;
    if (int rc = solve_wait(h, &r)) return rc;
    if (r.st.done) break;
  }
  h->ran_form = 0;
  return finish_summary(h, &r, summary);
}

int cc_intrinsics_optimize_multi(const cc_options* opt, int32_t n_devices, const int32_t* devices, int64_t F,
                                 const int64_t* off, const float* uv, const float* xyz, double* intr9, uint32_t mask,
                                 double* q, double* t, cc_summary* summary) {
  cc::last_call_status_reset();
  using namespace cc;
  if (n_devices < 1 || !devices || n_devices > kP2pMaxRanks)
    return fail(CC_ERR_BAD_ARGUMENT, "cc_intrinsics_optimize_multi: 1..%d devices", kP2pMaxRanks);
  if (!off || F <= 0 || !intr9 || !q || !t) return fail(CC_ERR_BAD_ARGUMENT, "cc_intrinsics_optimize_multi: bad arguments");
  const int n = (int)std::min<int64_t>(n_devices, F);
  if (n == 1) return cc_intrinsics_optimize(opt, devices[0], F, off, uv, xyz, intr9, mask, q, t, summary);
  std::vector<int64_t> first((size_t)n + 1);
  if (int rc = cc_partition_frames(F, off, n, first.data())) return rc;
  std::vector<cc_intrinsics*> hs((size_t)n, nullptr);
  auto cleanup = [&]() {
    for (auto* h : hs) if (h) { hipSetDevice(h->device); hipStreamSynchronize(h->stream); }
    for (auto* h : hs) cc_intrinsics_destroy(h);
  };
  int rc = 0;
  for (int r = 0; r < n && !rc; ++r) {
    const int64_t f0 = first[(size_t)r], f1 = first[(size_t)r + 1], o0 = off[f0];
    std::vector<int64_t> so((size_t)(f1 - f0) + 1);
    for (int64_t f = f0; f <= f1; ++f) so[(size_t)(f - f0)] = off[f] - o0;
    rc = cc_intrinsics_create(devices[r], f1 - f0, so.data(), uv ? uv + 2 * o0 : nullptr, xyz ? xyz + 3 * o0 : nullptr, &hs[(size_t)r]);
    if (!rc) rc = cc_intrinsics_set_state(hs[(size_t)r], intr9, mask, q + 4 * f0, t + 3 * f0);
  }
  if (!rc) {
    std::vector<Mailbox*> boxes;
    std::vector<int> devs;
    for (auto* h : hs) { boxes.push_back(&h->mailbox); devs.push_back(h->device); }
    for (int r = 0; r < n && !rc; ++r) { rc = hipSetDevice(hs[(size_t)r]->device) == hipSuccess ? mailbox_alloc(&hs[(size_t)r]->mailbox, kVecSolve, 16) : fail(CC_ERR_HIP, "hipSetDevice failed"); }
    for (int r = 0; r < n && !rc; ++r) {
      cc_intrinsics* h = hs[(size_t)r];
      rc = mailbox_wire_local(&h->mailbox, r, n, boxes.data(), devs.data(), &h->d.x);
      if (!rc) { h->d.rank = r; h->d.nranks = n; h->exchange = true; }
    }
  }
  cc_options o;
  if (opt) o = *opt; else cc_options_init(&o);
  o.use_graph = 0;
  std::vector<SolveRun> runs((size_t)n);
  for (int r = 0; r < n && !rc; ++r) rc = solve_begin(hs[(size_t)r], &o, &runs[(size_t)r]);
  bool all_persist = !rc;
  for (int r = 0; r < n && all_persist; ++r) {
    cc_intrinsics* h = hs[(size_t)r];
    int co = 0;
    for (auto* g : hs) if (g->device == h->device) ++co;
    all_persist = h->persist_ok && (int64_t)(h->pq.G + 1) * co <= h->p_resident && !runs[(size_t)r].profile;
  }
  for (auto* h : hs) if (h) h->persist_x_ok = all_persist;
  if (all_persist) {
    for (int r = 0; r < n && !rc; ++r) rc = persistent_launch(hs[(size_t)r], &runs[(size_t)r]);
    for (int r = 0; r < n && !rc; ++r) rc = persistent_wait(hs[(size_t)r], &runs[(size_t)r]);
    if (!rc) rc = persistent_log_settled(hs[0], summary);
  }
  for (int chunk = 0; !rc && !all_persist; ++chunk) {
    for (int r = 0; r < n && !rc; ++r) rc = solve_launch(hs[(size_t)r], &runs[(size_t)r], chunk);
    for (int r = 0; r < n && !rc; ++r) rc = solve_wait(hs[(size_t)r], &runs[(size_t)r]);
    if (rc) break;
    bool all_done = true, any_done = false;
    for (auto& run : runs) { all_done = all_done && run.st.done; any_done = any_done || run.st.done; }
    if (all_done) break;
    if (any_done) rc = fail(CC_ERR_STATE, "cc_intrinsics_optimize_multi: the shards disagree about termination");
  }
  if (!rc) rc = finish_summary(hs[0], &runs[0], summary);
  for (int r = 0; r < n && !rc; ++r) {
    const int64_t f0 = first[(size_t)r];
    rc = cc_intrinsics_get_state(hs[(size_t)r], r == 0 ? intr9 : nullptr, q + 4 * f0, t + 3 * f0);
  }
  const std::string err = rc ? last_error() : std::string();
  cleanup();
  if (rc) last_error() = err;
  return rc;
}

int cc_intrinsics_debug_fetch(cc_intrinsics* h, const char* name, double* out, int64_t n) {
  using namespace cc;
  if (!h || !name || !out || n < 0) return fail(CC_ERR_BAD_ARGUMENT, "cc_intrinsics_debug_fetch: bad arguments");
  const std::string k(name);
  const double* src = nullptr;
  int64_t cap = 0;
  if (k == "vec_solve") { src = h->d.vec_solve; cap = kVecSolve; }
  else if (k == "stats") { src = h->d.stats; cap = h->F * h->d.T * kStatsCols; }
  else if (k == "ctl") { src = reinterpret_cast<const double*>(h->d.ctl_next); cap = sizeof(LmCtl) / 8; }
  else if (k == "start_records" && h->start_candidates > 0) { src = h->start_srec; cap = (int64_t)h->start_candidates * h->start_searched * 24; }
  else if (k == "start_views" && h->start_candidates > 0) { src = h->start_view; cap = h->F * 24; }
  if (!src || n > cap) return fail(CC_ERR_BAD_ARGUMENT, "cc_intrinsics_debug_fetch: unknown buffer or too long");
  CC_HIP(hipSetDevice(h->device));
  CC_HIP(hipStreamSynchronize(h->stream));
  CC_HIP(hipMemcpy(out, src, (size_t)n * sizeof(double), hipMemcpyDeviceToHost));
  return CC_OK;
}

int cc_intrinsics_solver_form(cc_intrinsics* h) {
  if (!h || h->comm || h->own_sweep()) return 0;
  return (h->exchange ? h->persist_x_ok : h->persist_ok) ? h->pq.teams : 0;
}

int cc_intrinsics_solver_status(cc_intrinsics* h, int32_t* form, int32_t* reruns, char* note, int32_t note_capacity) {
  using namespace cc;
  if (!h) return fail(CC_ERR_BAD_ARGUMENT, "cc_intrinsics_solver_status: NULL handle");
  return solver_status(h, cc_intrinsics_solver_form(h), form, reruns, note, note_capacity);
}

int cc_intrinsics_profile_solve(cc_intrinsics* h, const cc_options* opt, int32_t n, double* avg_launch_ms, int32_t* sweeps_per_launch) {
  using namespace cc;
  if (!h || n < 1 || !avg_launch_ms) return fail(CC_ERR_BAD_ARGUMENT, "cc_intrinsics_profile_solve: bad arguments");
  if (!h->have_state) return fail(CC_ERR_STATE, "cc_intrinsics_profile_solve: no state set");
  if (h->huber_a > 0.0) return fail(CC_ERR_STATE, "cc_intrinsics_profile_solve: the handle has a Huber loss set and solves in the two-kernel form");
  if (h->model != CC_MODEL_RADTAN) return fail(CC_ERR_STATE, "cc_intrinsics_profile_solve: the handle has the fisheye model set and solves in the two-kernel form");
  if (!h->persist_ok || h->comm || h->exchange) return fail(CC_ERR_STATE, "cc_intrinsics_profile_solve: the handle does not use the persistent form on a device of its own");
  CC_HIP(hipSetDevice(h->device));
  hipEvent_t e0, e1;
  CC_HIP(hipEventCreate(&e0));
  CC_HIP(hipEventCreate(&e1));
  double total = 0.0;
  int sweeps = 0, rc = 0;
  for (int i = 0; i <= n && !rc; ++i) {
    SolveRun r;
    if ((rc = cc_intrinsics_reset(h))) break;
    if ((rc = solve_begin(h, opt, &r))) break;
    if (r.profile) { rc = fail(CC_ERR_BAD_ARGUMENT, "cc_intrinsics_profile_solve: profile_kernels selects the two-kernel form"); break; }
    hipEventRecord(e0, h->stream);
    if ((rc = persistent_launch(h, &r))) break;
    hipEventRecord(e1, h->stream);
    if ((rc = persistent_wait(h, &r))) break;
    if (hipEventSynchronize(e1) != hipSuccess) { rc = fail(CC_ERR_HIP, "hipEventSynchronize failed"); break; }
    float ms = 0.f;
    if (hipEventElapsedTime(&ms, e0, e1) != hipSuccess) { rc = fail(CC_ERR_HIP, "hipEventElapsedTime failed"); break; }
    if (i > 0) total += ms;
    sweeps = r.st.sweeps;
  }
  hipEventDestroy(e0);
  hipEventDestroy(e1);
  if (rc) return rc;
  *avg_launch_ms = total / n;
  if (sweeps_per_launch) *sweeps_per_launch = sweeps;
  return CC_OK;
}

int cc_intrinsics_profile_sweep(cc_intrinsics* h, int32_t n, double* avg_ms) {
  using namespace cc;
  if (!h || n < 1 || !avg_ms) return fail(CC_ERR_BAD_ARGUMENT, "cc_intrinsics_profile_sweep: bad arguments");
  CC_HIP(hipSetDevice(h->device));
  LmCtl st;
  if (int rc = read_ctl(h, &st)) return rc;
  if (st.phase != 1) return fail(CC_ERR_STATE, "cc_intrinsics_profile_sweep: run cc_intrinsics_solve first");
  LmCtl run = st;
  run.done = 0; run.step_valid = 1;
  CC_HIP(hipMemcpyAsync(h->d.ctl, &run, sizeof(run), hipMemcpyHostToDevice, h->stream));
  hipEvent_t e0, e1;
  CC_HIP(hipEventCreate(&e0));
  CC_HIP(hipEventCreate(&e1));
  launch_sweep(h, false);
  CC_HIP(hipEventRecord(e0, h->stream));
  for (int i = 0; i < n; ++i) launch_sweep(h, false);
  CC_HIP(hipEventRecord(e1, h->stream));
  CC_HIP(hipGetLastError());
  CC_HIP(hipStreamSynchronize(h->stream));
  float ms = 0.f;
  CC_HIP(hipEventElapsedTime(&ms, e0, e1));
  hipEventDestroy(e0);
  hipEventDestroy(e1);
  *avg_ms = (double)ms / n;
  CC_HIP(hipMemcpy(h->d.ctl, &st, sizeof(st), hipMemcpyHostToDevice));
  return CC_OK;
}

int cc_intrinsics_profile_kernel(cc_intrinsics* h, int32_t which, int32_t n, double* avg_ms) {
  using namespace cc;
  if (!h || n < 1 || !avg_ms || which != 1) return fail(CC_ERR_BAD_ARGUMENT, "cc_intrinsics_profile_kernel: bad arguments");
  if (h->comm || h->exchange) return fail(CC_ERR_STATE, "cc_intrinsics_profile_kernel: single-GPU handles only");
  CC_HIP(hipSetDevice(h->device));
  LmCtl st;
  if (int rc = read_ctl(h, &st)) return rc;
  if (st.phase != 1) return fail(CC_ERR_STATE, "cc_intrinsics_profile_kernel: run cc_intrinsics_solve first");
  LmCtl run = st;
  run.done = 0; run.step_valid = 1; run.cand_pending = 1; run.log_len = 1; run.iter = 1;
  run.gmax = 1e30;
  run.x_cost = run.current_cost = run.reference_cost = run.candidate_cost = run.minimum_cost = 2.0 * st.x_cost + 1.0;
  LmOpts lo = h->cached_opts;
  lo.function_tolerance = lo.parameter_tolerance = lo.gradient_tolerance = -1.0;
  lo.max_iterations = 1 << 30;
  CC_HIP(hipMemcpy(h->d.opts, &lo, sizeof(lo), hipMemcpyHostToDevice));
  h->opts_valid = false;
  CC_HIP(hipMemcpyAsync(h->d.ctl, &run, sizeof(run), hipMemcpyHostToDevice, h->stream));
  CC_HIP(hipMemcpyAsync(h->d.ctl_next, &run, sizeof(run), hipMemcpyHostToDevice, h->stream));
  hipEvent_t e0, e1;
  CC_HIP(hipEventCreate(&e0));
  CC_HIP(hipEventCreate(&e1));
  auto launch = [&]() { hipLaunchKernelGGL(k_intr_decide_elim<0>, dim3(h->elim_blocks), dim3(256), 0, h->stream, h->d, 2); };
  launch();
  CC_HIP(hipEventRecord(e0, h->stream));
  for (int i = 0; i < n; ++i) launch();
  CC_HIP(hipEventRecord(e1, h->stream));
  CC_HIP(hipGetLastError());
  CC_HIP(hipStreamSynchronize(h->stream));
  float ms = 0.f;
  CC_HIP(hipEventElapsedTime(&ms, e0, e1));
  hipEventDestroy(e0);
  hipEventDestroy(e1);
  *avg_ms = (double)ms / n;
  CC_HIP(hipMemcpy(h->d.ctl, &st, sizeof(st), hipMemcpyHostToDevice));
  CC_HIP(hipMemcpy(h->d.ctl_next, &st, sizeof(st), hipMemcpyHostToDevice));
  return CC_OK;
}

int cc_intrinsics_optimize(const cc_options* opt, int32_t device, int64_t F, const int64_t* off,
                           const float* uv, const float* xyz, double* intr9, uint32_t mask,
                           double* q, double* t, cc_summary* summary) {
  cc::last_call_status_reset();
  cc_intrinsics* h = nullptr;
  double* tm = cc::last_timing();
  for (int i = 0; i < 5; ++i) tm[i] = 0.0;
// ... 251 lines not shown
```

### camera_calibrator_amd/csrc/cc_intrinsics_dev.hpp

```cpp
#pragma once
#include "cc_common.hpp"
#include "cc_device.hpp"

namespace cc {

constexpr int kSweepThreads = 256;
constexpr int kSweepLdsBytes = (4 * kStageDoublesPerWave + 256) * 8;
constexpr int kStatsCols = 4;
constexpr int kYStride = 64;
constexpr int kPartialCols = 80;
constexpr int kElimMaxBlocks = 64;
constexpr int kVecSolve = kPartialCols + 32;

enum { ST_COST = 0, ST_QMODEL = 1, ST_STEP2 = 2, ST_XNORM2 = 3 };
enum { PC_S = 0, PC_B = 45, PC_HDIAG = 54, PC_FAIL = 63, PC_GS = 64, PC_GMAXP = 73 };

struct IntrDev {
  int64_t F, N;
  int32_t T, tpad_;
  const float* uv;
  const float* xyz;
  const int64_t* off;
  double* intr;
  const double* init_intr;
  const double* init_pose;
  double* pose;
  double* blocks;
  double* stats;
  double* hd0;
  double* sp;
  double* Y;
  double* partial;
  double* vec_solve;
  double* vec_decide;
  double* ds;
  double* ss;
  LmCtl* ctl;
  LmCtl* ctl_next;
  unsigned* arrive;
  unsigned long long* pub_seq;
  unsigned long long* host_pub;
  LmOpts* opts;
  cc_iteration* log;
  int32_t log_cap;
  uint32_t mask;
  int32_t rank, nranks;
  P2pDev x;
};

struct ObsCommon {
  double a0, a1, a2, x, y, iz, xy, r2, r4, r6, ax, ay, xd, yd, dxx, dxy, dyy;
};

__device__ __forceinline__ void obs_common(const double* k, const double* R, const double* t,
                                           double X0, double X1, double X2, ObsCommon& c) {
  c.a0 = R[0] * X0 + R[1] * X1 + R[2] * X2;
  c.a1 = R[3] * X0 + R[4] * X1 + R[5] * X2;
  c.a2 = R[6] * X0 + R[7] * X1 + R[8] * X2;
  const double xc = c.a0 + t[0], yc = c.a1 + t[1], zc = c.a2 + t[2];
  c.iz = 1.0 / zc;
  c.x = xc * c.iz;
  c.y = yc * c.iz;
  const double k1 = k[4], k2 = k[5], p1 = k[6], p2 = k[7], k3 = k[8];
  const double xx = c.x * c.x, yy = c.y * c.y;
  c.xy = c.x * c.y;
  c.r2 = xx + yy;
  c.r4 = c.r2 * c.r2;
  c.r6 = c.r4 * c.r2;
  const double m = 1.0 + k1 * c.r2 + k2 * c.r4 + k3 * c.r6;
  c.ax = c.r2 + 2.0 * xx;
  c.ay = c.r2 + 2.0 * yy;
  c.xd = c.x * m + 2.0 * p1 * c.xy + p2 * c.ax;
  c.yd = c.y * m + 2.0 * p2 * c.xy + p1 * c.ay;
  const double mp = k1 + 2.0 * k2 * c.r2 + 3.0 * k3 * c.r4;
  c.dxx = m + 2.0 * mp * xx + 2.0 * p1 * c.y + 6.0 * p2 * c.x;
  c.dxy = 2.0 * mp * c.xy + 2.0 * p1 * c.x + 2.0 * p2 * c.y;
  c.dyy = m + 2.0 * mp * yy + 2.0 * p2 * c.x + 6.0 * p1 * c.y;
}

__device__ __forceinline__ void row_u(const double* k, const ObsCommon& c, double u, double* v, double w = 1.0) {
  const double fx = k[0] * w;
  v[15] = (k[0] * c.xd + k[2] - u) * w;
  v[0] = c.xd * w; v[1] = 0.0; v[2] = w; v[3] = 0.0;
  const double fxx = fx * c.x;
  v[4] = fxx * c.r2; v[5] = fxx * c.r4; v[6] = fx * 2.0 * c.xy; v[7] = fx * c.ax; v[8] = fxx * c.r6;
  const double b0 = fx * c.dxx * c.iz, b1 = fx * c.dxy * c.iz, b2 = -(b0 * c.x + b1 * c.y);
  v[9] = 2.0 * (b2 * c.a1 - b1 * c.a2); v[10] = 2.0 * (b0 * c.a2 - b2 * c.a0); v[11] = 2.0 * (b1 * c.a0 - b0 * c.a1);
  v[12] = b0; v[13] = b1; v[14] = b2;
}

__device__ __forceinline__ void row_v(const double* k, const ObsCommon& c, double vm, double* v, double w = 1.0) {
  const double fy = k[1] * w;
  v[15] = (k[1] * c.yd + k[3] - vm) * w;
  v[0] = 0.0; v[1] = c.yd * w; v[2] = 0.0; v[3] = w;
  const double fyy = fy * c.y;
  v[4] = fyy * c.r2; v[5] = fyy * c.r4; v[6] = fy * c.ay; v[7] = fy * 2.0 * c.xy; v[8] = fyy * c.r6;
  const double b0 = fy * c.dxy * c.iz, b1 = fy * c.dyy * c.iz, b2 = -(b0 * c.x + b1 * c.y);
  v[9] = 2.0 * (b2 * c.a1 - b1 * c.a2); v[10] = 2.0 * (b0 * c.a2 - b2 * c.a0); v[11] = 2.0 * (b1 * c.a0 - b0 * c.a1);
  v[12] = b0; v[13] = b1; v[14] = b2;
}
__device__ __forceinline__ bool gram_entry_held(uint32_t mask, int e) { return (((mask >> (e >> 4)) | (mask >> (e & 15))) & 1u) != 0; }

__device__ __forceinline__ void intr_huber(double a, double s, double& rho, double& sr) {
  const double b = a * a;
  const double y = rsqrt_pos(s);
  const double r = s * y;
  const double q = fmax(2.2250738585072014e-308, a * y);
  const double tail_sr = q * rsqrt_pos(q);
  const double tail_rho = 2.0 * a * r - b;
  const bool tail = s > b;
  rho = tail ? tail_rho : s;
  sr = tail ? tail_sr : 1.0;
}

__device__ __forceinline__ void publish_to_host(const IntrDev& P, const LmCtl& c) {
  if (!P.host_pub) return;
  const unsigned long long* w = reinterpret_cast<const unsigned long long*>(&c);
#pragma unroll
  for (int i = 0; i < (int)(sizeof(LmCtl) / 8); ++i)
    __hip_atomic_store(P.host_pub + 2 + i, w[i], __ATOMIC_RELAXED, __HIP_MEMORY_SCOPE_SYSTEM);
  const unsigned long long seq = *P.pub_seq + 1ull;
  *P.pub_seq = seq;
  __hip_atomic_store(P.host_pub, seq, __ATOMIC_RELEASE, __HIP_MEMORY_SCOPE_SYSTEM);
}

}
```

### camera_calibrator_amd/csrc/cc_intrinsics_huber.hpp

```cpp
#pragma once
#include "cc_common.hpp"
#include "cc_device.hpp"
#include "cc_intrinsics_dev.hpp"

namespace cc {

__device__ __forceinline__ void huber_obs_common(const double* k, const double* R, const double* t,
                                                 double X0, double X1, double X2, ObsCommon& c) {
#pragma clang fp contract(off)
  c.a0 = fma(R[2], X2, fma(R[1], X1, R[0] * X0));
  c.a1 = fma(R[5], X2, fma(R[3], X0, R[4] * X1));
  c.a2 = fma(R[8], X2, fma(R[6], X0, R[7] * X1));
  const double xc = c.a0 + t[0], yc = c.a1 + t[1], zc = c.a2 + t[2];
  c.iz = 1.0 / zc;
  c.x = xc * c.iz;
  c.y = yc * c.iz;
  const double k1 = k[4], k2 = k[5], p1 = k[6], p2 = k[7], k3 = k[8];
  const double xx = c.x * c.x, yy = c.y * c.y;
  c.xy = c.x * c.y;
  c.r2 = fma(c.y, c.y, xx);
  c.r4 = c.r2 * c.r2;
  c.r6 = c.r4 * c.r2;
  const double m = fma(k3, c.r6, fma(k2, c.r4, fma(k1, c.r2, 1.0)));
  c.ax = fma(2.0, xx, c.r2);
  c.ay = fma(2.0, yy, c.r2);
  c.xd = fma(p2, c.ax, fma(2.0 * p1, c.xy, c.x * m));
  c.yd = fma(p1, c.ay, fma(2.0 * p2, c.xy, c.y * m));
  const double mp2 = 2.0 * fma(3.0 * k3, c.r4, fma(2.0 * k2, c.r2, k1));
  c.dxx = fma(6.0 * p2, c.x, fma(2.0 * p1, c.y, fma(mp2, xx, m)));
  c.dxy = fma(2.0 * p2, c.y, fma(2.0 * p1, c.x, mp2 * c.xy));
  c.dyy = fma(6.0 * p1, c.y, fma(2.0 * p2, c.x, fma(mp2, yy, m)));
}

__device__ __forceinline__ void huber_row_tail(const ObsCommon& c, double b0, double b1, double b2, double rw, double* v) {
#pragma clang fp contract(off)
  v[9] = 2.0 * fma(b2, c.a1, -(b1 * c.a2)); v[10] = 2.0 * fma(b0, c.a2, -(b2 * c.a0)); v[11] = 2.0 * fma(b1, c.a0, -(b0 * c.a1));
  v[12] = b0; v[13] = b1; v[14] = b2; v[15] = rw;
}

__device__ __forceinline__ void huber_row_u(const double* k, const ObsCommon& c, double r, double* v, double w) {
#pragma clang fp contract(off)
  const double fx = k[0] * w;
  v[0] = c.xd * w; v[1] = 0.0; v[2] = w; v[3] = 0.0;
  const double fxx = fx * c.x;
  v[4] = fxx * c.r2; v[5] = fxx * c.r4; v[6] = fx * 2.0 * c.xy; v[7] = fx * c.ax; v[8] = fxx * c.r6;
  const double b0 = fx * c.dxx * c.iz, b1 = fx * c.dxy * c.iz, b2 = -fma(b1, c.y, b0 * c.x);
  huber_row_tail(c, b0, b1, b2, r * w, v);
}

__device__ __forceinline__ void huber_row_v(const double* k, const ObsCommon& c, double r, double* v, double w) {
#pragma clang fp contract(off)
  const double fy = k[1] * w;
  v[0] = 0.0; v[1] = c.yd * w; v[2] = 0.0; v[3] = w;
  const double fyy = fy * c.y;
  v[4] = fyy * c.r2; v[5] = fyy * c.r4; v[6] = fy * c.ay; v[7] = fy * 2.0 * c.xy; v[8] = fyy * c.r6;
  const double b0 = fy * c.dxy * c.iz, b1 = fy * c.dyy * c.iz, b2 = -fma(b0, c.x, b1 * c.y);
  huber_row_tail(c, b0, b1, b2, r * w, v);
}

__device__ __forceinline__ void huber_residuals(const double* k, const ObsCommon& c, double u, double vm, double& ru, double& rv) {
#pragma clang fp contract(off)
  ru = fma(k[0], c.xd, k[2]) - u;
  rv = fma(k[1], c.yd, k[3]) - vm;
}

__global__ __launch_bounds__(kSweepThreads, 4) void k_intr_sweep_huber(IntrDev P, int flags, double huber_a) {
  extern __shared__ __attribute__((aligned(16))) char smem_raw[];
  double* s_stage = reinterpret_cast<double*>(smem_raw);
  double* s_blk = s_stage;
  double* sm = s_stage + 4 * kStageDoublesPerWave;
  const int tid = threadIdx.x, lane = tid & 63, wave = tid >> 6;
  const int T = P.T;
  const int64_t f = (int64_t)blockIdx.x / T;
  const int tile = (int)(blockIdx.x - f * T);
  const bool in_solve = (flags & 1) != 0, restart = (flags & 2) != 0;
  const LmCtl* ctl = P.ctl;
  const int c_done = ctl->done, c_phase = ctl->phase, c_valid = ctl->step_valid, c_cur = ctl->cur;
  const int done = restart ? 0 : c_done, phase = restart ? 0 : c_phase, step_valid = restart ? 0 : c_valid,
            cur = restart ? 0 : c_cur;
  int64_t s0 = P.off[f], s1 = P.off[f + 1];
  if (T > 1) {
    const int64_t len = (s1 - s0 + T - 1) / T;
    s0 = s0 + tile * len < s1 ? s0 + tile * len : s1;
    s1 = s0 + len < s1 ? s0 + len : s1;
  }
  const float2* uv2 = reinterpret_cast<const float2*>(P.uv);
  const int64_t wrem = s1 - s0 - wave * 64;
  const int npass = wrem > 0 ? (int)((wrem + kSweepThreads - 1) / kSweepThreads) : 0;
  const int64_t safe0 = s0 < P.N ? s0 : 0;
  float2 nm;
  float nX0, nX1, nX2;
  {
    const int64_t idx = s0 + tid;
    const int64_t ic = idx < s1 ? idx : safe0;
    nm = uv2[ic];
    nX0 = P.xyz[ic * 3]; nX1 = P.xyz[ic * 3 + 1]; nX2 = P.xyz[ic * 3 + 2];
  }
  double gv;
  {
    const double* src;
    if (tid < 60) src = P.Y + f * kYStride + tid;
    else if (tid < 67) src = (restart ? P.init_pose : P.pose) + (size_t)f * 8 + (tid - 60);
    else if (tid < 74) src = P.pose + ((size_t)P.F + f) * 8 + (tid - 67);
    else if (tid < 83) src = (restart ? P.init_intr : P.intr) + (tid - 74);
    else if (tid < 92) src = P.intr + 16 + (tid - 83);
    else if (tid < 101) src = P.ds + (tid - 92);
    else if (tid < 110) src = P.ss + (tid - 101);
    else if (tid < 116) src = P.sp + f * 8 + (tid - 110);
    else src = P.ss;
    gv = *src;
  }
  double g_old = 0.0;
  if (tile == 0) {
    const size_t base = cur ? (size_t)P.F : 0;
    if (T == 1) g_old = P.blocks[(base + f) * 256 + tid];
    else for (int k = 0; k < T; ++k) g_old += P.blocks[((base + f) * T + k) * 256 + tid];
  }
  if (tid < 116) sm[tid] = gv;
  if (done) return;
  if (phase != 0 && !step_valid) return;
  if (P.x.on && in_solve && blockIdx.x == 0 && tid == 0) P.x.seq[1] += 1ull;
  if (restart) {
    if (tile == 0 && tid >= 60 && tid < 67) P.pose[(size_t)f * 8 + (tid - 60)] = sm[tid];
    if (blockIdx.x == 0 && tid >= 74 && tid < 83) P.intr[tid - 74] = sm[tid];
    if (blockIdx.x == 0 && tid == 0) *P.arrive = 0u;
  }
  const int dst = phase == 0 ? cur : (cur ^ 1);
  __syncthreads();
  const int pose_o = cur ? 67 : 60, intr_o = cur ? 83 : 74;
  if (tid < 6) {
    const double* Yr = sm + tid * 10;
    double a = Yr[9];
#pragma unroll
    for (int j = 0; j < 9; ++j) a += Yr[j] * sm[92 + j];
    sm[129 + tid] = phase != 0 ? -a * sm[110 + tid] : 0.0;
  } else if (tid >= 8 && tid < 17) {
    const int j = tid - 8;
    const double d = (phase == 0 || (P.mask & (1u << j))) ? 0.0 : sm[92 + j] * sm[101 + j];
    sm[120 + j] = d;
    const double kc = sm[intr_o + j] + d;
    sm[148 + j] = kc;
    if (blockIdx.x == 0 && phase != 0) P.intr[dst * 16 + j] = kc;
  }
  __syncthreads();
  if (tid == 0) {
    double q[4], t[3], dp[6];
#pragma unroll
    for (int i = 0; i < 4; ++i) q[i] = sm[pose_o + i];
#pragma unroll
    for (int i = 0; i < 3; ++i) t[i] = sm[pose_o + 4 + i];
#pragma unroll
    for (int i = 0; i < 6; ++i) dp[i] = sm[129 + i];
    double step2 = 0.0;
    if (phase != 0) {
      double qn[4];
      quat_plus(q, dp, qn);
#pragma unroll
      for (int i = 0; i < 4; ++i) { const double d = qn[i] - q[i]; step2 += d * d; q[i] = qn[i]; }
#pragma unroll
      for (int i = 0; i < 3; ++i) { const double tn = t[i] + dp[3 + i]; const double d = tn - t[i]; step2 += d * d; t[i] = tn; }
      if (tile == 0) {
        double* pose_dst = P.pose + ((size_t)dst * P.F + f) * 8;
#pragma unroll
        for (int i = 0; i < 4; ++i) pose_dst[i] = q[i];
#pragma unroll
        for (int i = 0; i < 3; ++i) pose_dst[4 + i] = t[i];
      }
    }
    double R[9];
    quat_to_R(q, R);
#pragma unroll
    for (int i = 0; i < 9; ++i) sm[136 + i] = R[i];
#pragma unroll
    for (int i = 0; i < 3; ++i) sm[145 + i] = t[i];
    sm[158] = step2;
    sm[159] = q[0] * q[0] + q[1] * q[1] + q[2] * q[2] + q[3] * q[3] + t[0] * t[0] + t[1] * t[1] + t[2] * t[2];
  }
  __syncthreads();

  double qterm = 0.0;
  if (phase != 0 && tile == 0) {
    const int a = tid >> 4, b = tid & 15;
    if (a < 15) qterm = b < 15 ? 0.5 * sm[120 + a] * g_old * sm[120 + b] : sm[120 + a] * g_old;
  }
  {
    const double qw = wave_sum(qterm);
    if (lane == 0) sm[170 + wave] = qw;
  }

  double R[9], tt[3], kk[9];
#pragma unroll
  for (int i = 0; i < 9; ++i) R[i] = rfl(sm[136 + i]);
#pragma unroll
  for (int i = 0; i < 3; ++i) tt[i] = rfl(sm[145 + i]);
#pragma unroll
  for (int i = 0; i < 9; ++i) kk[i] = rfl(sm[148 + i]);
  const uint32_t mask = P.mask;

  double* stage = s_stage + wave * kStageDoublesPerWave;
  d4 acc0 = {0.0, 0.0, 0.0, 0.0}, acc1 = {0.0, 0.0, 0.0, 0.0};
  double hcost = 0.0;
  for (int p = 0; p < npass; ++p) {
    const int64_t idx = s0 + (int64_t)p * kSweepThreads + tid;
    const bool valid = idx < s1;
    const float2 m = nm;
    const float X0 = nX0, X1 = nX1, X2 = nX2;
    {
      const int64_t nidx = idx + kSweepThreads;
      const int64_t ic = nidx < s1 ? nidx : safe0;
      nm = uv2[ic];
      nX0 = P.xyz[ic * 3]; nX1 = P.xyz[ic * 3 + 1]; nX2 = P.xyz[ic * 3 + 2];
    }
    ObsCommon oc;
    huber_obs_common(kk, R, tt, (double)X0, (double)X1, (double)X2, oc);
    double ru, rv;
    huber_residuals(kk, oc, (double)m.x, (double)m.y, ru, rv);
    double rho, sr;
    intr_huber(huber_a, ru * ru + rv * rv, rho, sr);
    const double wrow = valid ? sr : 0.0;
    hcost += valid ? 0.5 * rho : 0.0;
    double v[16];
    huber_row_u(kk, oc, ru, v, wrow);
    stage_row(stage, lane, v);
    wave_lds_fence();
    gram_rows(stage, lane, acc0, acc1);
    wave_lds_fence();
    huber_row_v(kk, oc, rv, v, wrow);
    stage_row(stage, lane, v);
    wave_lds_fence();
    gram_rows(stage, lane, acc0, acc1);
    wave_lds_fence();
  }
  {
    const double hw = wave_sum(hcost);
    if (lane == 0) sm[176 + wave] = hw;
  }

  __syncthreads();
#pragma unroll
  for (int r = 0; r < 4; ++r) s_blk[wave * 256 + ((lane >> 4) + 4 * r) * 16 + (lane & 15)] = acc0[r] + acc1[r];
  __syncthreads();
  const double g = gram_entry_held(mask, tid) ? 0.0 : (s_blk[tid] + s_blk[256 + tid]) + (s_blk[512 + tid] + s_blk[768 + tid]);
  P.blocks[(((size_t)dst * P.F + f) * T + tile) * 256 + tid] = g;
  if (tid == 255) {
    double* st = P.stats + (size_t)blockIdx.x * kStatsCols;
    st[ST_COST] = (sm[176] + sm[177]) + (sm[178] + sm[179]);
    st[ST_QMODEL] = (sm[170] + sm[171]) + (sm[172] + sm[173]);
    st[ST_STEP2] = tile == 0 ? sm[158] : 0.0;
    st[ST_XNORM2] = tile == 0 ? sm[159] : 0.0;
  }
  if (phase == 0 && tid < 9 * 17 && tid % 17 == 0) P.hd0[(size_t)blockIdx.x * 16 + tid / 17] = g;
}

__global__ __launch_bounds__(256) void k_intr_obs_cost(IntrDev P, int cur, double huber_a, double* out ) {
  const int64_t i = (int64_t)blockIdx.x * blockDim.x + threadIdx.x;
  if (i >= P.N) return;
  int64_t lo = 0, hi = P.F;
  while (hi - lo > 1) {
    const int64_t mid = (lo + hi) >> 1;
    if (P.off[mid] <= i) lo = mid; else hi = mid;
  }
  const double* pose = P.pose + ((size_t)cur * P.F + lo) * 8;
  const double* k = P.intr + cur * 16;
  double kk[9], R[9];
#pragma unroll
  for (int j = 0; j < 9; ++j) kk[j] = k[j];
  const double q[4] = {pose[0], pose[1], pose[2], pose[3]}, t[3] = {pose[4], pose[5], pose[6]};
  quat_to_R(q, R);
  ObsCommon oc;
  obs_common(kk, R, t, (double)P.xyz[i * 3], (double)P.xyz[i * 3 + 1], (double)P.xyz[i * 3 + 2], oc);
  const double ru = kk[0] * oc.xd + kk[2] - (double)P.uv[i * 2], rv = kk[1] * oc.yd + kk[3] - (double)P.uv[i * 2 + 1];
  const double s = ru * ru + rv * rv, b = huber_a * huber_a;
  out[i] = 0.5 * ((huber_a > 0.0 && s > b) ? 2.0 * huber_a * sqrt(s) - b : s);
}

}
```

### camera_calibrator_amd/csrc/cc_intrinsics_persist.hip

```cpp
#include "cc_intrinsics_persist.hpp"
#include "cc_persist_dev.hpp"
#include "cc_persist_publish.hpp"
#include "cc_persist_sum.hpp"

namespace cc {


constexpr int persist_lds_doubles(int teams) { return teams * 4 * kStageDoublesPerWave + teams * 2 * 256 + teams * 192 + 512; }

enum { TM_Y = 0, TM_POSE = 60, TM_SP = 76, TM_STEP = 84, TM_R = 100, TM_T = 109, TM_KC = 112, TM_STEP2 = 122, TM_XN2 = 123,
       TM_QW = 124, TM_STAT = 128  };
enum { WG_INTR = 0 , WG_X = 64 , WG_DS = 66 ,
       WG_SS = 80 , WG_R0 = 96 , WG_OPT = 100 ,
       WG_TAB = 104 ,
       WG_TGI = 416 , WG_TZ = 456  };

static_assert(TM_POSE - TM_Y >= 6 * 10 && TM_SP - TM_POSE >= 2 * 8 && TM_STEP - TM_SP >= 6 && TM_R - TM_STEP >= 15 && TM_T - TM_R >= 9 && TM_KC - TM_T >= 3 &&
              TM_STEP2 - TM_KC >= 9 && TM_QW - TM_XN2 >= 1 && TM_STAT - TM_QW >= 4 && TM_STAT + 4 + 9 <= 192,
              "per-team scratch: Y (6 x 10), two poses, pose scale, step (9 + 6), R, t, intrinsics, scalars, statistics row -- inside the 192 doubles persist_lds_doubles gives a team");
static_assert(WG_X - WG_INTR >= 2 * 16 && WG_DS - WG_X >= 2 && WG_SS - WG_DS >= 9 && WG_R0 - WG_SS >= 9 && WG_OPT - WG_R0 >= 1 && WG_TAB - WG_OPT >= 4 &&
              WG_TZ - WG_TGI >= 80 / 2 && WG_TZ + 80 / 2 <= 512,
              "workgroup scratch: both intrinsics, broadcast (2 + 9), scales, options, tables of the 80-slot row -- inside the 512 doubles of persist_lds_doubles");

template <int NC, int NG, int BATCH = 8>
__device__ __forceinline__ void gather_rows(const u64* box, int G, unsigned tag, int ncols, int maxcol, double* s_part,
                                            double* out, unsigned* fail, int* s_ok, int tshift) {
  const int tid = threadIdx.x, col = tid % NC, grp = tid / NC;
  if (tid == 0) *s_ok = 1;
  __syncthreads();
  if (grp < NG && col < ncols) {
    double acc = 0.0;
    bool good = true;
    const long long t0 = wall_clock64();
    for (int r0 = grp; r0 < G && good; r0 += BATCH * NG) {
      u64 lo[BATCH], hi[BATCH];
      for (unsigned spins = 0;; ++spins) {
#pragma unroll
        for (int u = 0; u < BATCH; ++u) {
          const int r = r0 + u * NG;
          const u64* p = box + (size_t)(r < G ? r : r0) * (2 * NC) + 2 * col;
          lo[u] = ag_ld(p);
          hi[u] = ag_ld(p + 1);
        }
        bool ok = true;
#pragma unroll
        for (int u = 0; u < BATCH; ++u) ok = ok && (unsigned)(lo[u] >> 32) == tag && (unsigned)(hi[u] >> 32) == tag;
        if (ok) break;
        if ((spins & 63u) == 63u && (timed_out(t0, tshift) || ag_ld32(fail) != 0u)) { good = false; break; }
        __builtin_amdgcn_s_sleep(1);
      }
      if (!good) break;
#pragma unroll
      for (int u = 0; u < BATCH; ++u) {
        if (r0 + u * NG < G) {
          const double v = ungranule(lo[u], hi[u]);
          acc = col == maxcol ? fmax(acc, v) : acc + v;
        }
      }
    }
    s_part[grp * NC + col] = acc;
    if (!good) *s_ok = 0;
  }
  __syncthreads();
  if (tid < ncols) {
    double a = 0.0;
    if (tid == maxcol) { for (int g = 0; g < NG; ++g) a = fmax(a, s_part[g * NC + tid]); }
    else { for (int g = 0; g < NG; ++g) a += s_part[g * NC + tid]; }
    out[tid] = a;
  }
  __syncthreads();
}

template <int THREADS>
__device__ __forceinline__ void gather_stats4(const u64* box, int G, unsigned tag, double* s_part, double* out, unsigned* fail, int* s_ok, int tshift) {
  constexpr int RPT = 1024 / THREADS;
  static_assert(THREADS / 4 * RPT == kPMaxWorkers, "one statistics row per four threads: the host caps the worker grid at kPMaxWorkers");
  const int tid = threadIdx.x, col = tid & 3, lane = tid & 63, wave = tid >> 6;
  if (tid == 0) *s_ok = 1;
  __syncthreads();
  u64 lo[RPT], hi[RPT];
  bool good = true;
  const long long t0 = wall_clock64();
  for (unsigned spins = 0;; ++spins) {
    bool ok = true;
#pragma unroll
    for (int k = 0; k < RPT; ++k) {
      const int r = (tid >> 2) + k * (THREADS / 4);
      const u64* p = box + (size_t)(r < G ? r : 0) * (2 * kPStatCols) + 2 * col;
      lo[k] = ag_ld(p);
      hi[k] = ag_ld(p + 1);
    }
#pragma unroll
    for (int k = 0; k < RPT; ++k) ok = ok && (unsigned)(lo[k] >> 32) == tag && (unsigned)(hi[k] >> 32) == tag;
    if (ok) break;
    if ((spins & 63u) == 63u && (timed_out(t0, tshift) || ag_ld32(fail) != 0u)) { good = false; break; }
    __builtin_amdgcn_s_sleep(1);
  }
  double acc = 0.0;
#pragma unroll
  for (int k = 0; k < RPT; ++k)
    if ((tid >> 2) + k * (THREADS / 4) < G) acc += ungranule(lo[k], hi[k]);
  acc = wave_sum_mod<2>(acc);
  if (lane < 4) s_part[wave * 4 + lane] = acc;
  if (!good) *s_ok = 0;
  __syncthreads();
  if (tid < 4) {
    double a = 0.0;
#pragma unroll
    for (int w = 0; w < THREADS / 64; ++w) a += s_part[w * 4 + tid];
    out[tid] = a;
  }
  __syncthreads();
}

__device__ __forceinline__ size_t persist_box_word(int c, int g, int G) {
  return kPBoxColumnMajor ? ((size_t)c * (size_t)G + (size_t)g) * 2 : ((size_t)g * kPartialCols + (size_t)c) * 2;
}

template <int NG>
__device__ __forceinline__ void own_columns(const u64* box, u64* obox, int G, int w, unsigned tag, double* vals, unsigned* fail, int tid0, int tshift) {
  constexpr int kPer = (kPMaxWorkers + 63) / 64;
  int lane = tid0 & 63;
  asm volatile("" : "+v"(lane));
  asm volatile("" : "+s"(G));
  const int nc = (kPartialCols - 1 - w) / G + 1, items = nc * G, nL = persist_sum_groups(G);
  const u64* p[kPer];
#pragma unroll
  for (int u = 0; u < kPer; ++u) {
    const int i = lane + 64 * u, ic = i < items ? i : 0, k = ic / G;
    p[u] = box + persist_box_word(w + k * G, ic - k * G, G);
  }
  int gv[2], gn[2], gm[2];
#pragma unroll
  for (int u = 0; u < 2; ++u) {
    const int t = lane + 64 * u, tc = t < nc * nL ? t : 0, k = tc / nL, j = tc - k * nL;
    gv[u] = k * G + j * kPSumRows;
    gn[u] = persist_sum_group_rows(G, j);
    gm[u] = w + k * G == PC_GMAXP;
  }
  asm volatile("" : "+v"(gv[0]), "+v"(gv[1]), "+v"(gn[0]), "+v"(gn[1]), "+v"(gm[0]), "+v"(gm[1]));
  u64 lo[kPer], hi[kPer];
  bool good = true;
  const long long t0 = wall_clock64();
  for (unsigned spins = 0;; ++spins) {
#pragma unroll
    for (int u = 0; u < kPer; ++u) {
      lo[u] = ag_ld(p[u]);
      hi[u] = ag_ld(p[u] + 1);
    }
    bool ok = true;
#pragma unroll
    for (int u = 0; u < kPer; ++u) ok = ok && (unsigned)(lo[u] >> 32) == tag && (unsigned)(hi[u] >> 32) == tag;
    if (ok) break;
    if ((spins & 63u) == 63u && (timed_out(t0, tshift) || ag_ld32(fail) != 0u)) { good = false; break; }
    __builtin_amdgcn_s_sleep(1);
  }
  if (__any(!good)) {
    if (lane == 0) __hip_atomic_store(fail, 1u, __ATOMIC_RELAXED, __HIP_MEMORY_SCOPE_AGENT);
    return;
  }
#pragma unroll
  for (int u = 0; u < kPer; ++u)
    if (lane + 64 * u < items) vals[lane + 64 * u] = ungranule(lo[u], hi[u]);
  wave_lds_fence();
  double* Ls = vals + kPMaxWorkers + kPSumRows;
#pragma unroll
  for (int u = 0; u < 2; ++u)
    if (lane + 64 * u < nc * nL) Ls[lane + 64 * u] = persist_sum_group<NG>(vals + gv[u], gn[u], gm[u] != 0);
  wave_lds_fence();
  for (int k = lane; k < nc; k += 64) {
    const int c = w + k * G;
    const double total = persist_sum_group<NG>(Ls + k * nL, nL, c == PC_GMAXP);
    ag_st(obox + 2 * c, granule(tag, total, 0));
    ag_st(obox + 2 * c + 1, granule(tag, total, 1));
  }
}

__device__ __forceinline__ void gather_totals(const u64* box, unsigned tag, double* out, unsigned* fail, int* s_ok, int tshift) {
  const int tid = threadIdx.x;
  if (tid == 0) *s_ok = 1;
  __syncthreads();
  if (tid < kPartialCols) {
    const u64* p = box + 2 * tid;
    u64 lo, hi;
    bool good = true;
    const long long t0 = wall_clock64();
    for (unsigned spins = 0;; ++spins) {
      lo = ag_ld(p);
      hi = ag_ld(p + 1);
      if ((unsigned)(lo >> 32) == tag && (unsigned)(hi >> 32) == tag) break;
      if ((spins & 63u) == 63u && (timed_out(t0, tshift) || ag_ld32(fail) != 0u)) { good = false; break; }
      __builtin_amdgcn_s_sleep(1);
    }
    out[tid] = ungranule(lo, hi);
    if (!good) *s_ok = 0;
  }
  __syncthreads();
}

template <int THREADS>
__device__ __forceinline__ void persist_control(const IntrDev& P, const PersistDev& Q, double* lds) {
  double* s_part = lds;
  double* sv = lds + 1024;
  double* s_tot = lds + 1152;
  double* s_bc = lds + 1168;
  double* s_intr = lds + 1184;
  double* s_ss = lds + 1216;
  LmCtl* s_ctl = reinterpret_cast<LmCtl*>(lds + 1232);
  LmOpts* s_opts = reinterpret_cast<LmOpts*>(lds + 1252);
  cc_iteration* s_log = reinterpret_cast<cc_iteration*>(lds + 1264);
  int* s_int = reinterpret_cast<int*>(lds + 1296);
  u64* s_seq = reinterpret_cast<u64*>(lds + 1300);
  const int tid = threadIdx.x, wave = tid >> 6;
  static_assert(sizeof(cc_iteration) <= 32 * 8, "log record scratch");
  if (tid < (int)(sizeof(LmCtl) / 8)) reinterpret_cast<double*>(s_ctl)[tid] = 0.0;
  if (tid >= 32 && tid < 32 + (int)(sizeof(LmOpts) / 8)) reinterpret_cast<u64*>(s_opts)[tid - 32] = reinterpret_cast<const u64*>(P.opts)[tid - 32];
  if (tid >= 64 && tid < 64 + 32) s_intr[tid - 64] = 0.0;
  if (tid == 48 && P.host_pub) *s_seq = *P.pub_seq + 1ull;
  __syncthreads();
  if (tid < 9) s_intr[tid] = (Q.restart ? P.init_intr : P.intr)[tid];
  if (tid == 0) s_int[1] = 0;
  __syncthreads();
  const LmOpts& o = *s_opts;
  const uint32_t mask = P.mask;

  for (int round = 0; round < Q.max_rounds; ++round) {
    const unsigned e1 = Q.epoch0 + 3u * (unsigned)round + 1u, e2 = e1 + 1u, e3 = e1 + 2u;
    const bool phase0 = round == 0;
    if (phase0) gather_rows<kPStatCols, THREADS / kPStatCols>(Q.sbox, Q.G, e1, 13, -1, s_part, s_tot, Q.fail, s_int, (phase0 ? Q.first_shift : Q.timeout_shift));
    else gather_stats4<THREADS>(Q.sbox, Q.G, e1, s_part, s_tot, Q.fail, s_int, (phase0 ? Q.first_shift : Q.timeout_shift));
    if (P.x.on) {
      const bool need = phase0 || (s_ctl->cand_pending && s_ctl->step_valid);
      if (need) {
        if (tid >= 13 && tid < 16) s_tot[tid] = 0.0;
        __syncthreads();
        const unsigned long long epoch = P.x.seq[1] + 1ull;
        p2p_post(P.x, 1, epoch, P.rank, P.nranks, s_tot, 16);
        int* s_ok2 = s_int + 4;
        const double a = p2p_collect(P.x, 1, epoch, P.rank, P.nranks, 16, s_ok2);
        if (tid < 16) s_tot[tid] = a;
        if (tid == 0) { P.x.seq[1] = epoch; if (!*s_ok2) s_int[0] = 0; }
        __syncthreads();
      }
    }
    if (tid == 0) {
      LmCtl c = *s_ctl;
      const int len0 = c.log_len, prev_cur = c.cur & 1, was_valid = c.step_valid;
      const double prev_radius = c.radius;
      const double* kc0 = s_intr + (c.cur ? 16 : 0);
      const double* kc1 = s_intr + (c.cur ? 0 : 16);
      if (!s_int[0]) {
        __hip_atomic_store(Q.fail, 1u, __ATOMIC_RELAXED, __HIP_MEMORY_SCOPE_AGENT);
        c.done = 1; c.term = CC_FAILURE_EXCHANGE;
      } else if (phase0) {
        double xn2 = s_tot[ST_XNORM2];
#pragma unroll
        for (int i = 0; i < 9; ++i) {
          const double ki = kc0[i];
          xn2 += ki * ki;
          s_ss[i] = o.jacobi_scaling ? 1.0 / (1.0 + sqrt(s_tot[4 + i])) : 1.0;
        }
        lm_init(c, o, s_tot[ST_COST], sqrt(xn2));
      } else if (c.cand_pending) {
        double step2 = s_tot[ST_STEP2], xn2 = s_tot[ST_XNORM2];
        if (c.step_valid) {
#pragma unroll
          for (int i = 0; i < 9; ++i) {
            const double kc = kc1[i], k0 = kc0[i];
            const double d = kc - k0;
            step2 += d * d;
            xn2 += kc * kc;
          }
        }
        lm_decide(c, o, s_log, s_tot[ST_COST], s_tot[ST_QMODEL], step2, xn2);
      }
      if (!c.done && round + 1 >= Q.max_rounds) { c.done = 1; c.term = CC_NO_CONVERGENCE; }
      *s_ctl = c;
      s_int[1] = c.log_len != len0;
      s_int[2] = phase0 ? (!c.done && c.radius == o.initial_radius)
                        : (was_valid && !c.done && (c.cur & 1) == (prev_cur ^ 1) && c.radius == persist_spec_radius(prev_radius, o.max_radius));
      s_bc[0] = (double)((c.done ? 1 : 0) | ((c.cur & 1) << 3));
      s_bc[1] = c.radius;
#pragma unroll
      for (int i = 0; i < 9; ++i) s_bc[2 + i] = 0.0;
    }
    __syncthreads();
    const bool hit = s_int[2] != 0;
    if (s_ctl->done || !hit) {
      if (tid < 22) ag_st(Q.xbox + tid, granule(e2, s_bc[tid >> 1], tid & 1));
      if (s_ctl->done) break;
    }
    const unsigned erow = hit ? e2 : e3;
    gather_totals(Q.lbox, erow, sv, Q.fail, s_int, (phase0 ? Q.first_shift : Q.timeout_shift));
    if (P.x.on) {
      if (tid >= kPartialCols && tid < kVecSolve) sv[tid] = 0.0;
      __syncthreads();
      if (tid == 0) { sv[kPartialCols + P.rank] = sv[PC_GMAXP]; sv[PC_GMAXP] = 0.0; }
      __syncthreads();
      const unsigned long long epoch = P.x.seq[0] + 1ull;
      p2p_post(P.x, 0, epoch, P.rank, P.nranks, sv, kVecSolve);
      int* s_ok2 = s_int + 4;
      const double a = p2p_collect(P.x, 0, epoch, P.rank, P.nranks, kVecSolve, s_ok2);
      if (tid < kVecSolve) sv[tid] = a;
      if (tid == 0) { P.x.seq[0] = epoch; if (!*s_ok2) s_int[0] = 0; }
      __syncthreads();
      if (tid == 0) {
        double g = 0.0;
        for (int r = 0; r < P.nranks && r < 32; ++r) g = fmax(g, sv[kPartialCols + r]);
        sv[PC_GMAXP] = g;
      }
      __syncthreads();
    }
    if (wave == 0) {
      int lane = tid & 63;
      asm volatile("" : "+v"(lane));
      const int cur = s_ctl->cur & 1;
      const double radius = s_ctl->radius;
      const double gl = (lane < 9 && !((mask >> lane) & 1u)) ? fabs(sv[PC_GS + lane]) : sv[PC_GMAXP];
      const double k_l = s_intr[cur * 16 + (lane < 9 ? lane : 8)], ss_l = s_ss[lane < 9 ? lane : 8];
      bool ok = !(sv[PC_FAIL] > 0.0);
      double x[9];
      {
#pragma clang fp contract(off)
        const int i = lane < 9 ? lane : 8;
        const bool pin_i = (mask >> i) & 1u;
        const double si = s_ss[i];
        const double damp = clampd(sv[PC_HDIAG + i] * (si * si), o.min_lm_diagonal, o.max_lm_diagonal) / radius;
        double a[9];
#pragma unroll
        for (int k = 0; k < 9; ++k) {
          const int kk = k <= i ? k : i;
          const int idx = kk * 9 - kk * (kk - 1) / 2 + (i - kk);
          double v = sv[idx] * (s_ss[kk] * si);
          if (k == i) v += damp;
          const bool pin_k = (mask >> kk) & 1u;
          if (pin_i || pin_k) v = (k == i) ? 1.0 : 0.0;
          a[k] = v;
        }
        const double b = pin_i ? 0.0 : sv[PC_B + i] * si;
        ok = chol_solve_rows<9>(a, b, x) && ok;
#pragma unroll
        for (int j = 0; j < 9; ++j) ok = ok && isfinite(x[j]);
      }
      const double gmax = row16_max(gl);
      const bool go = s_int[0] && !(gmax <= o.gradient_tolerance) && !(radius < o.min_radius);
      if (lane < 9) {
        double xs = 0.0;
#pragma unroll
        for (int j = 0; j < 9; ++j) xs = lane == j ? x[j] : xs;
        const double ds = go ? -xs : 0.0;
        const double d = ((mask >> lane) & 1u) ? 0.0 : ds * ss_l;
        s_bc[2 + lane] = d;
        s_intr[(cur ^ 1) * 16 + lane] = k_l + d;
      }
      if (lane == 0) {
        s_bc[0] = (double)((go ? 0 : 1) | (go && ok ? 2 : 0) | (hit ? 4 : 0) | (cur << 3));
        s_bc[1] = radius;
        s_bc[12] = gmax;
      }
      wave_lds_fence();
      if (lane < 22) ag_st(Q.xbox + lane, granule(erow, s_bc[lane >> 1], lane & 1));
    }
    if (tid == 0) {
      const double gmax = s_bc[12];
      const bool ok = ((int)s_bc[0] & 2) != 0;
      cc_iteration* e = s_int[1] ? s_log : nullptr;
      if (e && e->accepted) e->gradient_max_norm = gmax;
      if (!s_int[0]) { __hip_atomic_store(Q.fail, 1u, __ATOMIC_RELAXED, __HIP_MEMORY_SCOPE_AGENT); s_ctl->done = 1; s_ctl->term = CC_FAILURE_EXCHANGE; }
      else if (lm_finalize(*s_ctl, o, gmax)) { s_ctl->step_valid = ok ? 1 : 0; s_ctl->cand_pending = 1; }
      if (e && s_ctl->log_len <= P.log_cap && !s_ctl->done) P.log[s_ctl->log_len - 1] = *e;
    }
    __syncthreads();
    if (s_ctl->done) break;
  }
  if (wave != 0) return;
  int lane = threadIdx.x;
  asm volatile("" : "+v"(lane));
  wave_lds_fence();
  const unsigned failed = ag_ld32(Q.fail);
  constexpr int kLogWords = (int)(sizeof(cc_iteration) / 8);
  static_assert(sizeof(LmCtl) == kPubDoubles * 8 && sizeof(cc_iteration) % 8 == 0 && kLogWords <= 64 && kPubWords <= 64, "one word per lane");
  static_assert(offsetof(LmCtl, done) == 0 && offsetof(LmCtl, term) == 4, "lanes 0 and 1 hold done and term");
  unsigned half = reinterpret_cast<const unsigned*>(s_ctl)[lane < kPubWords ? lane : 0];
  const int done = s_ctl->done, log_len = s_ctl->log_len;
  const bool owes_record = s_int[1] && log_len <= P.log_cap;
  const double intr_l = s_intr[lane & 31];
  const u64 log_l = reinterpret_cast<const u64*>(s_log)[lane < kLogWords ? lane : 0];
  if (failed != 0u) half = lane == 0 ? 1u : lane == 1 ? (unsigned)CC_FAILURE_EXCHANGE : half;
  else if (!done) half = lane == 0 ? 1u : lane == 1 ? (unsigned)CC_NO_CONVERGENCE : half;
  if (P.host_pub) {
    const u64 seq = *s_seq;
    if (lane < kPubWords) __hip_atomic_store(P.host_pub + kPubTaggedAt + lane, publish_word(publish_tag(seq), half), __ATOMIC_RELAXED, __HIP_MEMORY_SCOPE_SYSTEM);
    if (lane == 0) {
      __hip_atomic_store(P.host_pub, seq, __ATOMIC_RELAXED, __HIP_MEMORY_SCOPE_SYSTEM);
      *P.pub_seq = seq;
    }
  }
  if (lane < kPubWords) {
    reinterpret_cast<unsigned*>(P.ctl)[lane] = half;
    reinterpret_cast<unsigned*>(P.ctl_next)[lane] = half;
  }
  if (lane < 32 && failed == 0u) P.intr[lane] = intr_l;
  if (owes_record && lane < kLogWords) reinterpret_cast<u64*>(P.log + (log_len - 1))[lane] = log_l;
}

template <int TEAMS>
__global__ __launch_bounds__(TEAMS * 256, TEAMS) void k_intr_persist(IntrDev P, PersistDev Q) {
  constexpr int THREADS = TEAMS * 256;
  extern __shared__ __attribute__((aligned(16))) char smem_raw[];
  double* s_stage = reinterpret_cast<double*>(smem_raw);
  if ((int)blockIdx.x == Q.G) { persist_control<THREADS>(P, Q, s_stage); return; }
  double* s_G = s_stage + TEAMS * 4 * kStageDoublesPerWave;
  double* s_tm = s_G + TEAMS * 2 * 256;
  double* s_wg = s_tm + TEAMS * 192;
#define CC_FRESH_TID(name) int name = tid0; asm volatile("" : "+v"(name))
  const int tid0 = threadIdx.x, wave = __builtin_amdgcn_readfirstlane(tid0 >> 6), team = wave >> 2, twave = wave & 3;
  const int sbase = (team & 3) * 64;
  const int64_t f = (int64_t)blockIdx.x * TEAMS + team;
  const bool has_frame = f < P.F;
  double* sm = s_tm + team * 192;
  double* tstage = s_stage + team * 4 * kStageDoublesPerWave;
  double* s_blk = tstage;
  double* Zs = tstage + 1024;
  double* red = tstage + 1100;
  unsigned char* pj = reinterpret_cast<unsigned char*>(s_wg + WG_TAB);
  unsigned char* pk = pj + 48;
  const uint32_t mask = P.mask;

  {
  const int tid = tid0, ttid = tid0 & 255;
  if (has_frame && ttid < 8) {
    const double v = ttid < 7 ? (Q.restart ? P.init_pose : P.pose)[(size_t)f * 8 + ttid] : 0.0;
    sm[TM_POSE + ttid] = v;
    sm[TM_POSE + 8 + ttid] = v;
  }
  if (ttid >= 64 && ttid < 64 + 60) sm[TM_Y + ttid - 64] = 0.0;
  if (tid < 32) s_wg[WG_INTR + tid] = 0.0;
  if (tid == 32) {
    const LmOpts* o = P.opts;
    s_wg[WG_OPT] = o->jacobi_scaling ? 1.0 : 0.0;
    s_wg[WG_OPT + 1] = o->min_lm_diagonal;
    s_wg[WG_OPT + 2] = o->max_lm_diagonal;
    s_wg[WG_OPT + 3] = o->max_radius;
    s_wg[WG_R0] = o->initial_radius;
  }
  if (tid == 33) {
    int oo = 0;
    for (int j = 0; j < 9; ++j)
      for (int k = j; k < 9; ++k) { pj[oo] = (unsigned char)j; pk[oo] = (unsigned char)k; ++oo; }
  }
  if (tid >= 64 && tid < 64 + 16) s_wg[WG_X + tid - 64] = 0.0;
  if (tid >= 80 && tid < 80 + 16) s_wg[WG_SS + tid - 80] = 1.0;
  __syncthreads();
  if (tid < 9) s_wg[WG_INTR + tid] = (Q.restart ? P.init_intr : P.intr)[tid];
  if (tid >= 128 && tid < 128 + kPartialCols) {
    const int o = tid - 128;
    int gi = 0, z = 0;
    if (o < 45) {
      const int j = pj[o], k = pk[o];
      gi = j * 16 + k; z = j | (k << 8) | (1 << 16);
    } else if (o < 54) {
      const int j = o - 45;
      gi = j * 16 + 15; z = j | (9 << 8) | (1 << 16);
    } else if (o < 63) {
      const int j = o - 54;
      gi = j * 17;
    } else if (o >= PC_GS && o < PC_GS + 9) {
      gi = (o - PC_GS) * 16 + 15;
    }
    reinterpret_cast<int*>(s_wg + WG_TGI)[o] = gi;
    reinterpret_cast<int*>(s_wg + WG_TZ)[o] = z;
  }
  }

  int64_t s0 = 0, s1 = 0;
  if (has_frame) { s0 = P.off[f]; s1 = P.off[f + 1]; }
  const float2* uv2 = reinterpret_cast<const float2*>(P.uv);
  const int64_t wrem = s1 - s0 - twave * 64;
  const int npass = wrem > 0 ? (int)((wrem + kSweepThreads - 1) / kSweepThreads) : 0;
  const int64_t safe0 = s0 < P.N ? s0 : 0;
  float2 nm;
  float nX0, nX1, nX2;
  {
    const int64_t first = s0 + (tid0 & 255);
    const int64_t firstc = first < s1 ? first : safe0;
    nm = uv2[firstc];
    nX0 = P.xyz[firstc * 3]; nX1 = P.xyz[firstc * 3 + 1]; nX2 = P.xyz[firstc * 3 + 2];
  }
  __syncthreads();

  int cur = 0;
  double radius = 1.0;
  bool step_valid = true, failed = false;
  for (int round = 0; round < Q.max_rounds; ++round) {
    const unsigned e1 = Q.epoch0 + 3u * (unsigned)round + 1u, e2 = e1 + 1u, e3 = e1 + 2u;
    const bool phase0 = round == 0;
    const bool do_sweep = phase0 || step_valid;
    const int dst = phase0 ? cur : (cur ^ 1);
    d4 acc0, acc1;
    if (do_sweep) {
      CC_FRESH_TID(tid);
      const int ttid = tid & 255, lane = tid & 63;
      const double* ds = s_wg + WG_DS;
      const double* ss = s_wg + WG_SS;
      if (has_frame) {
        const int st = ttid - sbase;
        if (st >= 0 && st < 6) {
          const double* Yr = sm + TM_Y + st * 10;
          double a = Yr[9];
#pragma unroll
          for (int j = 0; j < 9; ++j) a += Yr[j] * ds[j];
          sm[TM_STEP + 9 + st] = phase0 ? 0.0 : -a * sm[TM_SP + st];
        } else if (st >= 8 && st < 17) {
          const int j = st - 8;
          const double d = (phase0 || (mask & (1u << j))) ? 0.0 : ds[j] * ss[j];
          sm[TM_STEP + j] = d;
          const double kc = s_wg[WG_INTR + cur * 16 + j] + d;
          sm[TM_KC + j] = kc;
          if (team == 0 && !phase0) s_wg[WG_INTR + dst * 16 + j] = kc;
        }
      }
      __syncthreads();
      if (has_frame && ttid == sbase) {
        double q[4], t[3], dp[6];
#pragma unroll
        for (int i = 0; i < 4; ++i) q[i] = sm[TM_POSE + cur * 8 + i];
#pragma unroll
        for (int i = 0; i < 3; ++i) t[i] = sm[TM_POSE + cur * 8 + 4 + i];
#pragma unroll
        for (int i = 0; i < 6; ++i) dp[i] = sm[TM_STEP + 9 + i];
        double step2 = 0.0;
        if (!phase0) {
          double qn[4];
          quat_plus_tab(q, dp, qn);
#pragma unroll
          for (int i = 0; i < 4; ++i) { const double d = qn[i] - q[i]; step2 += d * d; q[i] = qn[i]; }
#pragma unroll
          for (int i = 0; i < 3; ++i) { const double tn = t[i] + dp[3 + i]; const double d = tn - t[i]; step2 += d * d; t[i] = tn; }
#pragma unroll
          for (int i = 0; i < 4; ++i) sm[TM_POSE + dst * 8 + i] = q[i];
#pragma unroll
          for (int i = 0; i < 3; ++i) sm[TM_POSE + dst * 8 + 4 + i] = t[i];
        }
        double R[9];
        quat_to_R(q, R);
#pragma unroll
        for (int i = 0; i < 9; ++i) sm[TM_R + i] = R[i];
#pragma unroll
        for (int i = 0; i < 3; ++i) sm[TM_T + i] = t[i];
        sm[TM_STEP2] = step2;
        sm[TM_XN2] = q[0] * q[0] + q[1] * q[1] + q[2] * q[2] + q[3] * q[3] + t[0] * t[0] + t[1] * t[1] + t[2] * t[2];
      }
      __syncthreads();
      {
        double qterm = 0.0;
        if (has_frame && !phase0) {
          const int a = ttid >> 4, b = ttid & 15;
          const double g_old = s_G[(team * 2 + cur) * 256 + ttid];
          if (a < 15) qterm = b < 15 ? 0.5 * sm[TM_STEP + a] * g_old * sm[TM_STEP + b] : sm[TM_STEP + a] * g_old;
        }
        const double qw = wave_sum(qterm);
        if (lane == 0) sm[TM_QW + twave] = qw;
      }
      double R[9], tt[3], kk[9];
#pragma unroll
      for (int i = 0; i < 9; ++i) R[i] = rfl(sm[TM_R + i]);
#pragma unroll
      for (int i = 0; i < 3; ++i) tt[i] = rfl(sm[TM_T + i]);
#pragma unroll
      for (int i = 0; i < 9; ++i) kk[i] = rfl(sm[TM_KC + i]);
      double* stage = s_stage + wave * kStageDoublesPerWave;
      acc0 = d4{0.0, 0.0, 0.0, 0.0};
      acc1 = d4{0.0, 0.0, 0.0, 0.0};
      for (int p = 0; p < npass; ++p) {
        const int64_t idx = s0 + (int64_t)p * kSweepThreads + ttid;
        const bool valid = idx < s1;
        const float2 m = nm;
        const float X0 = nX0, X1 = nX1, X2 = nX2;
        {
          const int64_t nidx = p + 1 < npass ? idx + kSweepThreads : s0 + ttid;
          const int64_t ic = nidx < s1 ? nidx : safe0;
          nm = uv2[ic];
          nX0 = P.xyz[ic * 3]; nX1 = P.xyz[ic * 3 + 1]; nX2 = P.xyz[ic * 3 + 2];
        }
        ObsCommon oc;
        obs_common(kk, R, tt, (double)X0, (double)X1, (double)X2, oc);
        double v[16];
        const double wrow = valid ? 1.0 : 0.0;
        row_u(kk, oc, (double)m.x, v, wrow);
        stage_row(stage, lane, v);
        wave_lds_fence();
        gram_rows_ahead(stage, lane, acc0, acc1);
        wave_lds_fence();
        row_v(kk, oc, (double)m.y, v, wrow);
        stage_row(stage, lane, v);
        wave_lds_fence();
        gram_rows_ahead(stage, lane, acc0, acc1);
        wave_lds_fence();
      }
      __syncthreads();
    }
    if (do_sweep) {
      CC_FRESH_TID(tid);
      const int ttid = tid & 255, lane = tid & 63;
#pragma unroll
      for (int r = 0; r < 4; ++r) s_blk[twave * 256 + ((lane >> 4) + 4 * r) * 16 + (lane & 15)] = acc0[r] + acc1[r];
      __syncthreads();
      const double g = gram_entry_held(mask, ttid) ? 0.0 : (s_blk[ttid] + s_blk[256 + ttid]) + (s_blk[512 + ttid] + s_blk[768 + ttid]);
      s_G[(team * 2 + dst) * 256 + ttid] = g;
      if (ttid == 255) {
        sm[TM_STAT + ST_COST] = 0.5 * g;
        sm[TM_STAT + ST_QMODEL] = (sm[TM_QW] + sm[TM_QW + 1]) + (sm[TM_QW + 2] + sm[TM_QW + 3]);
        sm[TM_STAT + ST_STEP2] = sm[TM_STEP2];
        sm[TM_STAT + ST_XNORM2] = sm[TM_XN2];
      }
      if (phase0 && ttid < 9 * 17 && ttid % 17 == 0) sm[TM_STAT + 4 + ttid / 17] = g;
      __syncthreads();
    }
    {
      CC_FRESH_TID(tid);
      const int ncols = phase0 ? 13 : 4;
      const int stid = tid - 128;
      if (stid >= 0 && stid < 2 * ncols) {
        const int c = stid >> 1;
        double a = 0.0;
        if (do_sweep) {
#pragma unroll
          for (int k = 0; k < TEAMS; ++k)
            if ((int64_t)blockIdx.x * TEAMS + k < P.F) a += s_tm[k * 192 + TM_STAT + c];
        }
        ag_st(Q.sbox + (size_t)blockIdx.x * (2 * kPStatCols) + stid, granule(e1, a, stid & 1));
      }
    }
    auto eliminate_and_post = [&](const int cur_e, const double radius_e, const bool first, u64* box, const unsigned tag) {
    CC_FRESH_TID(tid_e);
    if (has_frame && (tid_e & 255) >= sbase && (tid_e & 255) < sbase + 16) {
      const int l = (tid_e & 255) - sbase;
      const double* Gl = s_G + (team * 2 + cur_e) * 256;
      const double* ss = s_wg + WG_SS;
      const bool jac = s_wg[WG_OPT] != 0.0;
      const double mn = s_wg[WG_OPT + 1], mx = s_wg[WG_OPT + 2];
      const double inv_radius = 1.0 / radius_e;
      double s[6], L[21];
#pragma unroll
      for (int i = 0; i < 6; ++i)
#pragma unroll
        for (int j = 0; j <= i; ++j) L[tri(i, j)] = Gl[(9 + i) * 16 + 9 + j];
      if (first) {
#pragma unroll
        for (int i = 0; i < 6; ++i) s[i] = jac ? 1.0 / (1.0 + sqrt(L[tri(i, i)])) : 1.0;
        if (l < 6) {
          double sl = 0.0;
#pragma unroll
          for (int i = 0; i < 6; ++i) sl = l == i ? s[i] : sl;
          sm[TM_SP + l] = sl;
        }
      } else {
#pragma unroll
        for (int i = 0; i < 6; ++i) s[i] = sm[TM_SP + i];
      }
#pragma unroll
      for (int i = 0; i < 6; ++i)
#pragma unroll
        for (int j = 0; j <= i; ++j) L[tri(i, j)] = s[i] * L[tri(i, j)] * s[j];
#pragma unroll
      for (int i = 0; i < 6; ++i) L[tri(i, i)] += clampd(L[tri(i, i)], mn, mx) * inv_radius;
      bool ok = true;
      double Li[6];
#pragma unroll
      for (int j = 0; j < 6; ++j) {
        double d = L[tri(j, j)];
#pragma unroll
        for (int k = 0; k < j; ++k) d -= L[tri(j, k)] * L[tri(j, k)];
        ok = ok && (d > 0.0) && isfinite(d);
        const double inv = rsqrt_pos(d);
        L[tri(j, j)] = d * inv;
        Li[j] = inv;
#pragma unroll
        for (int i = j + 1; i < 6; ++i) {
          double a = L[tri(i, j)];
#pragma unroll
          for (int k = 0; k < j; ++k) a -= L[tri(i, k)] * L[tri(j, k)];
          L[tri(i, j)] = a * inv;
        }
      }
#pragma unroll
      for (int i = 0; i < 21; ++i) L[i] = rfl(L[i]);
#pragma unroll
      for (int i = 0; i < 6; ++i) { Li[i] = rfl(Li[i]); s[i] = rfl(s[i]); }
      if (l < 10) {
        const double sc = l < 9 ? ss[l] : 1.0;
        const int col = l < 9 ? l : 15;
        double w[6], z[6], y[6];
#pragma unroll
        for (int i = 0; i < 6; ++i) w[i] = Gl[(9 + i) * 16 + col];
#pragma unroll
        for (int i = 0; i < 6; ++i) {
          double a = s[i] * w[i] * sc;
#pragma unroll
          for (int k = 0; k < i; ++k) a -= L[tri(i, k)] * z[k];
          z[i] = a * Li[i];
        }
#pragma unroll
        for (int i = 5; i >= 0; --i) {
          double a = z[i];
#pragma unroll
          for (int k = i + 1; k < 6; ++k) a -= L[tri(k, i)] * y[k];
          y[i] = a * Li[i];
        }
#pragma unroll
        for (int i = 0; i < 6; ++i) {
          Zs[i * 10 + l] = z[i];
          sm[TM_Y + i * 10 + l] = y[i];
        }
      }
      if (l == 0) red[PC_FAIL] = ok ? 0.0 : 1.0;
    }
    if (has_frame && (tid_e & 255) >= sbase && (tid_e & 255) < sbase + 64) {
      const int l64 = (tid_e & 255) - sbase;
      const double* Gl = s_G + (team * 2 + cur_e) * 256;
      wave_lds_fence();
      const int* tgi = reinterpret_cast<const int*>(s_wg + WG_TGI);
      const int* tz = reinterpret_cast<const int*>(s_wg + WG_TZ);
      double accv[2];
      int zz_[2];
#pragma unroll
      for (int r = 0; r < 2; ++r) {
        const int o = l64 + 64 * r, oc = o < kPartialCols ? o : 0;
        zz_[r] = tz[oc];
        accv[r] = Gl[tgi[oc]];
      }
#pragma unroll
      for (int r = 0; r < 2; ++r) {
        const int zj = zz_[r] & 255, zk = (zz_[r] >> 8) & 255;
        double zz = 0.0;
#pragma unroll
        for (int i = 0; i < 6; ++i) zz += Zs[i * 10 + zj] * Zs[i * 10 + zk];
        const int o = l64 + 64 * r;
        const bool used = o < 63 || (o >= PC_GS && o < PC_GS + 9);
        if (o < kPartialCols && o != PC_FAIL && o != PC_GMAXP) red[o] = used ? accv[r] - ((zz_[r] >> 16) ? zz : 0.0) : 0.0;
      }
    }
    if (has_frame && (tid_e & 255) == (((team & 3) + 1) & 3) * 64) {
      const double* Gg = s_G + (team * 2 + cur_e) * 256;
      double q4[4], g6[6];
#pragma unroll
      for (int i = 0; i < 4; ++i) q4[i] = sm[TM_POSE + cur_e * 8 + i];
#pragma unroll
      for (int i = 0; i < 6; ++i) g6[i] = Gg[(9 + i) * 16 + 15];
      red[PC_GMAXP] = pose_grad_proj_max_tab(q4, g6);
    }
    __syncthreads();
    {
      CC_FRESH_TID(tid);
      if (tid < 2 * kPartialCols) {
        const int c = tid >> 1;
        double a = 0.0;
#pragma unroll
        for (int k = 0; k < TEAMS; ++k) {
          if ((int64_t)blockIdx.x * TEAMS + k < P.F) {
            const double v = s_stage[k * 4 * kStageDoublesPerWave + 1100 + c];
            a = c == PC_GMAXP ? fmax(a, v) : a + v;
          }
        }
        ag_st(box + persist_box_word(tid >> 1, (int)blockIdx.x, Q.G) + (tid & 1), granule(tag, a, tid & 1));
      }
    }
    if (wave == 3 && (int)blockIdx.x < kPartialCols)
      own_columns<THREADS / kPartialCols>(box, Q.lbox, Q.G, (int)blockIdx.x, tag, s_stage + 2048, Q.fail, tid0, (phase0 ? Q.first_shift : Q.timeout_shift));
    };
    auto wait_bcast = [&](const unsigned tag) {
      CC_FRESH_TID(tid);
      if (wave == 0 && !bcast_wait(Q.xbox, tag, 11, s_wg + WG_X, Q.fail, tid & 63, (phase0 ? Q.first_shift : Q.timeout_shift))) s_wg[WG_X] = 17.0;
      __syncthreads();
    };

    const bool spec = do_sweep;
    const double radius_spec = phase0 ? s_wg[WG_R0] : persist_spec_radius(radius, s_wg[WG_OPT + 3]);
    if (spec) eliminate_and_post(dst, radius_spec, phase0, Q.pbox, e2);
    wait_bcast(e2);
    int fl = (int)s_wg[WG_X];
    if (fl & 16) failed = true;
    if (fl & 1) { cur = (fl >> 3) & 1; break; }
    if (fl & 4) {
      cur = dst;
      radius = radius_spec;
    } else {
      cur = (fl >> 3) & 1;
      radius = s_wg[WG_X + 1];
      eliminate_and_post(cur, radius, false, Q.rbox, e3);
      wait_bcast(e3);
      fl = (int)s_wg[WG_X];
      if (fl & 16) failed = true;
      if (fl & 1) { cur = (fl >> 3) & 1; break; }
    }
    step_valid = (fl & 2) != 0;
  }
  if (!failed && ag_ld32(Q.fail) == 0u && has_frame && (tid0 & 255) < 7) P.pose[((size_t)cur * P.F + f) * 8 + (tid0 & 255)] = sm[TM_POSE + cur * 8 + (tid0 & 255)];
  asm volatile("" ::"v"(nm.x), "v"(nX0), "v"(nX1), "v"(nX2));
}

template <int TEAMS>
static int resident_of(int device, int* out) {
  const int lds = persist_lds_doubles(TEAMS) * 8;
  CC_HIP(hipFuncSetAttribute(reinterpret_cast<const void*>(k_intr_persist<TEAMS>), hipFuncAttributeMaxDynamicSharedMemorySize, lds));
  int per_cu = 0, cus = 0;
  CC_HIP(hipOccupancyMaxActiveBlocksPerMultiprocessor(&per_cu, k_intr_persist<TEAMS>, TEAMS * 256, lds));
  CC_HIP(hipDeviceGetAttribute(&cus, hipDeviceAttributeMultiprocessorCount, device));
  *out = per_cu >= 1 ? cus : 0;
  return 0;
}

int persist_resident_workgroups(int device, int teams, int* out) {
  return teams == 1 ? resident_of<1>(device, out) : teams == 2 ? resident_of<2>(device, out) : resident_of<4>(device, out);
}

void persist_launch(const IntrDev& P, const PersistDev& Q, bool drop_control, hipStream_t stream) {
  const dim3 grid((unsigned)Q.G + (drop_control ? 0u : 1u));
  if (Q.teams == 1) hipLaunchKernelGGL(k_intr_persist<1>, grid, dim3(256), persist_lds_doubles(1) * 8, stream, P, Q);
  else if (Q.teams == 2) hipLaunchKernelGGL(k_intr_persist<2>, grid, dim3(512), persist_lds_doubles(2) * 8, stream, P, Q);
  else hipLaunchKernelGGL(k_intr_persist<4>, grid, dim3(1024), persist_lds_doubles(4) * 8, stream, P, Q);
}

}
```

### camera_calibrator_amd/csrc/cc_intrinsics_persist.hpp

```cpp
#pragma once
#include "cc_intrinsics_dev.hpp"

namespace cc {

constexpr int kPMaxTeams = 4;
constexpr int kPStatCols = 16;
constexpr int kPBcastWords = 64;
constexpr int kPMaxWorkers = 256;
constexpr bool kPBoxColumnMajor = true;

struct PersistDev {
  unsigned long long* sbox;
  unsigned long long* pbox;
  unsigned long long* rbox;
  unsigned long long* lbox;
  unsigned long long* xbox;
  unsigned* fail;
  int32_t G;
  int32_t teams;
  uint32_t epoch0;
  int32_t max_rounds;
  int32_t restart;
  int32_t timeout_shift;
  int32_t first_shift;
};

int persist_resident_workgroups(int device, int teams, int* out);
void persist_launch(const IntrDev& P, const PersistDev& Q, bool drop_control, hipStream_t stream);

}
```

### include/cc_solver.h

```cpp
#ifndef CC_SOLVER_H
#define CC_SOLVER_H
#include <stddef.h>
#include <stdint.h>
#ifdef __cplusplus
extern "C" {
#endif

typedef enum cc_status {
  CC_OK = 0,
  CC_ERR_BAD_ARGUMENT = -1,
  CC_ERR_NO_DEVICE = -2,
  CC_ERR_HIP = -3,
  CC_ERR_COMM = -4,
  CC_ERR_STATE = -5
} cc_status;

enum {
  CC_NO_CONVERGENCE = 0,
  CC_CONVERGENCE_GRADIENT = 1,
  CC_CONVERGENCE_PARAMETER = 2,
  CC_CONVERGENCE_FUNCTION = 3,
  CC_FAILURE_INVALID_STEPS = 4,
  CC_MIN_RADIUS = 5,
  CC_FAILURE_EXCHANGE = 6
};

typedef struct cc_options {
  int32_t max_iterations;
  int32_t use_nonmonotonic_steps;
  int32_t max_consecutive_nonmonotonic_steps;
  int32_t jacobi_scaling;
  int32_t max_consecutive_invalid_steps;
  int32_t check_interval;
  double function_tolerance;
  double gradient_tolerance;
  double parameter_tolerance;
  double initial_radius;
  double max_radius;
  double min_radius;
  double min_relative_decrease;
  double min_lm_diagonal;
  double max_lm_diagonal;
  int32_t use_graph;
  int32_t profile_kernels;
} cc_options;

typedef struct cc_iteration {
  double cost;
  double cost_change;
  double model_cost_change;
  double relative_decrease;
  double gradient_max_norm;
  double step_norm;
  double radius;
  int32_t accepted;
  int32_t valid;
} cc_iteration;

enum { CC_K_SWEEP = 0, CC_K_DECIDE = 1, CC_K_ELIM = 2, CC_K_SOLVE = 3, CC_K_ALLREDUCE = 4, CC_K_UPDATE = 5, CC_K_REDUCE = 6, CC_K_COUNT = 8 };

typedef struct cc_summary {
  int32_t iterations;
  int32_t successful_steps;
  int32_t termination;
  int32_t log_len;
  double initial_cost;
  double final_cost;
  double seconds;
  cc_iteration* log;
  int32_t log_capacity;
  int32_t sweeps;
  double kernel_ms[CC_K_COUNT];
  int32_t kernel_launches[CC_K_COUNT];
  double kernel_idle_ms[CC_K_COUNT];
  int32_t kernel_idle_launches[CC_K_COUNT];
} cc_summary;

void cc_options_init(cc_options* o);
const char* cc_last_error(void);
void* cc_host_staging_acquire(size_t bytes);
void cc_host_staging_release(void* p);
void cc_last_call_timing(double out_ms[5]);
const char* cc_version(void);
void cc_release_caches(void);
int cc_last_call_solver_status(int32_t* form, int32_t* reruns, char* note, int32_t note_capacity);
void cc_parallel_for(int32_t parts, void (*fn)(void* ctx, int32_t part), void* ctx);
int32_t cc_parallel_parts(int64_t n, int64_t min_per_part);
int32_t cc_host_pool_threads(void);
int cc_device_count(void);

typedef struct cc_intrinsics cc_intrinsics;

int cc_intrinsics_create(int32_t device, int64_t n_frames, const int64_t* frame_offsets,
                         const float* uv, const float* xyz, cc_intrinsics** out);
void cc_intrinsics_destroy(cc_intrinsics* h);

int cc_intrinsics_set_state(cc_intrinsics* h, const double* intr9, uint32_t const_mask,
                            const double* q_wxyz, const double* t_xyz);
int cc_intrinsics_reset(cc_intrinsics* h);
int cc_intrinsics_get_state(cc_intrinsics* h, double* intr9, double* q_wxyz, double* t_xyz);

int cc_intrinsics_eval(cc_intrinsics* h, double* blocks, double* cost);

int cc_intrinsics_solve(cc_intrinsics* h, const cc_options* opt, cc_summary* summary);
int cc_intrinsics_solver_form(cc_intrinsics* h);
int cc_intrinsics_solver_status(cc_intrinsics* h, int32_t* form, int32_t* reruns, char* note, int32_t note_capacity);

int cc_intrinsics_profile_sweep(cc_intrinsics* h, int32_t n, double* avg_ms);
int cc_intrinsics_profile_solve(cc_intrinsics* h, const cc_options* opt, int32_t n, double* avg_launch_ms, int32_t* sweeps_per_launch);

int cc_intrinsics_optimize(const cc_options* opt, int32_t device, int64_t n_frames,
                           const int64_t* frame_offsets, const float* uv, const float* xyz,
                           double* intr9, uint32_t const_mask, double* q_wxyz, double* t_xyz,
                           cc_summary* summary);

int cc_intrinsics_estimate(const cc_options* opt, int32_t device, int64_t n_frames, const int64_t* frame_offsets,
                           const float* uv, const float* xyz, const double* distortion5, uint32_t const_mask,
                           float* K_init9, double* intr9, double* q_wxyz, double* t_xyz, cc_summary* summary);
int cc_intrinsics_estimate_views(const cc_options* opt, int32_t device, int64_t n_frames, const float* const* uv_views,
                                 const float* const* xyz_views, const int64_t* counts, const double* distortion5,
                                 uint32_t const_mask, float* K_init9, double* intr9, double* q_wxyz, double* t_xyz,
                                 cc_summary* summary);
int cc_intrinsics_optimize_views(const cc_options* opt, int32_t device, int64_t n_frames, const float* const* uv_views,
                                 const float* const* xyz_views, const int64_t* counts, double* intr9, uint32_t const_mask,
                                 double* q_wxyz, double* t_xyz, cc_summary* summary);

int cc_intrinsics_optimize_multi(const cc_options* opt, int32_t n_devices, const int32_t* devices,
                                 int64_t n_frames, const int64_t* frame_offsets, const float* uv,
                                 const float* xyz, double* intr9, uint32_t const_mask, double* q_wxyz,
                                 double* t_xyz, cc_summary* summary);

int cc_comm_get_unique_id(uint8_t id[128]);
int cc_intrinsics_comm_init(cc_intrinsics* h, const uint8_t id[128], int32_t rank, int32_t nranks);

int cc_intrinsics_exchange_export(cc_intrinsics* h, uint8_t handle[64]);
int cc_intrinsics_exchange_attach(cc_intrinsics* h, int32_t rank, int32_t nranks, const uint8_t* handles);

int cc_intrinsics_set_huber(cc_intrinsics* h, double a_pixels);
int cc_intrinsics_obs_cost(cc_intrinsics* h, double* obs_cost);
int cc_intrinsics_optimize_views_huber(const cc_options* opt, int32_t device, int64_t n_frames, const float* const* uv_views,
                                       const float* const* xyz_views, const int64_t* counts, double* intr9, uint32_t const_mask,
                                       double* q_wxyz, double* t_xyz, cc_summary* summary, double huber_a);
int cc_intrinsics_estimate_views_huber(const cc_options* opt, int32_t device, int64_t n_frames, const float* const* uv_views,
                                       const float* const* xyz_views, const int64_t* counts, const double* distortion5,
                                       uint32_t const_mask, float* K_init9, double* intr9, double* q_wxyz, double* t_xyz,
                                       cc_summary* summary, double huber_a);

enum { CC_MODEL_RADTAN = 0, CC_MODEL_FISHEYE = 1 };
int cc_intrinsics_set_model(cc_intrinsics* h, int32_t model);
int32_t cc_intrinsics_get_model(cc_intrinsics* h);
int cc_intrinsics_optimize_views_model(const cc_options* opt, int32_t device, int64_t n_frames, const float* const* uv_views,
                                       const float* const* xyz_views, const int64_t* counts, double* intr9, uint32_t const_mask,
                                       double* q_wxyz, double* t_xyz, cc_summary* summary, double huber_a, int32_t model);
int cc_intrinsics_estimate_views_model(const cc_options* opt, int32_t device, int64_t n_frames, const float* const* uv_views,
                                       const float* const* xyz_views, const int64_t* counts, const double* distortion5,
                                       uint32_t const_mask, float* K_init9, double* intr9, double* q_wxyz, double* t_xyz,
                                       cc_summary* summary, double huber_a, int32_t model);

typedef struct cc_intr_start_options {
  double centre[2];
  double theta_lo, theta_hi;
  int32_t candidates;
  int32_t search_views;
  int32_t refine_iterations;
} cc_intr_start_options;
void cc_intr_start_options_init(cc_intr_start_options* o);
typedef struct cc_intr_start_report {
  double centre[2], r_max, focal;
  int32_t best_candidate, candidates_qualified;
  int64_t views, views_searched, views_invalid;
} cc_intr_start_report;
int cc_intrinsics_estimate_start_fisheye(cc_intrinsics* h, const cc_intr_start_options* opt, double* intr9, double* q_wxyz,
                                         double* t_xyz, cc_intr_start_report* report);
int cc_intrinsics_start_scores(cc_intrinsics* h, double* f, double* score, int32_t* qualified);
int cc_intrinsics_estimate_views_start(const cc_options* opt, int32_t device, int64_t n_frames, const float* const* uv_views,
                                       const float* const* xyz_views, const int64_t* counts, const double* distortion5,
                                       uint32_t const_mask, float* K_init9, double* intr9, double* q_wxyz, double* t_xyz,
                                       cc_summary* summary, double huber_a, int32_t model, const cc_intr_start_options* start);

typedef struct cc_intrinsics_batch cc_intrinsics_batch;

int cc_intrinsics_batch_create(int32_t device, int64_t n_problems, const int64_t* problem_offsets ,
                               const int64_t* frame_offsets , const float* uv, const float* xyz,
                               cc_intrinsics_batch** out);
void cc_intrinsics_batch_destroy(cc_intrinsics_batch* h);
int cc_intrinsics_batch_set_state(cc_intrinsics_batch* h, const double* intr9, const uint32_t* const_mask,
                                  const double* q_wxyz, const double* t_xyz);
int cc_intrinsics_batch_get_state(cc_intrinsics_batch* h, double* intr9, double* q_wxyz, double* t_xyz);
int cc_intrinsics_batch_solve(cc_intrinsics_batch* h, const cc_options* opt, cc_summary* summaries);
int cc_intrinsics_batch_optimize(const cc_options* opt, int32_t device, int64_t n_problems, const int64_t* problem_offsets,
                                 const int64_t* frame_offsets, const float* uv, const float* xyz, double* intr9,
                                 const uint32_t* const_mask, double* q_wxyz, double* t_xyz, cc_summary* summaries);
int cc_intrinsics_batch_estimate(const cc_options* opt, int32_t device, int64_t n_problems, const int64_t* problem_offsets,
                                 const int64_t* frame_offsets, const float* uv, const float* xyz, const double* distortion5,
                                 const uint32_t* const_mask, float* K_init9, double* intr9, double* q_wxyz, double* t_xyz,
                                 cc_summary* summaries);
int cc_intrinsics_batch_set_huber(cc_intrinsics_batch* h, const double* a_pixels);
int cc_intrinsics_batch_estimate_huber(const cc_options* opt, int32_t device, int64_t n_problems, const int64_t* problem_offsets,
                                       const int64_t* frame_offsets, const float* uv, const float* xyz, const double* distortion5,
                                       const uint32_t* const_mask, float* K_init9, double* intr9, double* q_wxyz, double* t_xyz,
                                       cc_summary* summaries, const double* huber_a);
int cc_intrinsics_batch_set_model(cc_intrinsics_batch* h, int32_t model);
int cc_intrinsics_batch_get_model(const cc_intrinsics_batch* h, int32_t* model);
int cc_intrinsics_batch_estimate_model(const cc_options* opt, int32_t device, int64_t n_problems, const int64_t* problem_offsets,
                                       const int64_t* frame_offsets, const float* uv, const float* xyz, const double* distortion5,
                                       const uint32_t* const_mask, float* K_init9, double* intr9, double* q_wxyz, double* t_xyz,
                                       cc_summary* summaries, const double* huber_a, int32_t model);

int cc_partition_frames(int64_t n_frames, const int64_t* frame_offsets, int32_t nranks,
                        int64_t* first_frame);

typedef struct cc_rig cc_rig;

int cc_rig_create(int32_t device, int64_t n_cams, int64_t n_frames, int64_t n_world,
                  const int64_t* obs_frame_offsets, const uint32_t* obs_cam,
                  const uint64_t* obs_world, const float* obs_uv, const float* world_xyz,
                  const uint8_t* cam_frozen, double huber_a, cc_rig** out);
void cc_rig_destroy(cc_rig* h);
int cc_rig_set_state(cc_rig* h, const double* cam_q, const double* cam_t, const double* frame_q,
                     const double* frame_t);
int cc_rig_reset(cc_rig* h);
int cc_rig_solve(cc_rig* h, const cc_options* opt, cc_summary* summary);
int cc_rig_solver_form(cc_rig* h);
int cc_rig_solver_status(cc_rig* h, int32_t* form, int32_t* reruns, char* note, int32_t note_capacity);
int cc_rig_set_inner_iterations(cc_rig* h, int32_t enable, double tolerance);
int cc_rig_inner_pass(cc_rig* h, double* cost_before, double* cost_after, int32_t mini_iterations[4]);
int cc_rig_inner_status(cc_rig* h, int32_t* passes, int32_t* useful_passes, int32_t* enabled_at_end, double* cost_removed);
int cc_rig_get_state(cc_rig* h, double* cam_q, double* cam_t, double* frame_q, double* frame_t,
                     double* obs_cost);
int cc_rig_eval(cc_rig* h, double* cost);
typedef struct cc_rig_start_options {
  int32_t refine_iterations;
} cc_rig_start_options;
void cc_rig_start_options_init(cc_rig_start_options* o);
typedef struct cc_rig_start_report {
  int64_t views_valid, views_planar, views_general, views_invalid;
  int64_t frames_placed, frames_unplaced;
  int32_t cameras_placed, cameras_unplaced;
  int32_t root_camera;
  int32_t root_at_identity;
  int32_t* parent;
} cc_rig_start_report;
int cc_rig_estimate_start(cc_rig* h, const cc_rig_start_options* opt, const double* cam_q, const double* cam_t,
                          const double* frame_q, const double* frame_t, cc_rig_start_report* report);
int cc_rig_start_views(cc_rig* h, int64_t* n_views, int32_t* view_cam, int64_t* view_frame, int32_t* kind, double* q, double* t,
                       double* rms2);
int cc_rig_comm_init(cc_rig* h, const uint8_t id[128], int32_t rank, int32_t nranks);
int cc_rig_exchange_export(cc_rig* h, uint8_t handle[64]);
int cc_rig_exchange_attach(cc_rig* h, int32_t rank, int32_t nranks, const uint8_t* handles);

int cc_rigk_create(int32_t device, int64_t n_cams, int64_t n_frames, int64_t n_world,
                   const int64_t* obs_frame_offsets, const uint32_t* obs_cam, const uint64_t* obs_world,
                   const float* obs_uv_pixels, const float* world_xyz, const uint8_t* cam_frozen,
                   double huber_a, cc_rig** out);
int cc_rigk_set_intrinsics(cc_rig* h, const double* intr9, uint32_t const_mask);
int cc_rigk_get_intrinsics(cc_rig* h, double* intr9);
int cc_rigk_create_per_camera(int32_t device, int64_t n_cams, int64_t n_frames, int64_t n_world,
                              const int64_t* obs_frame_offsets, const uint32_t* obs_cam, const uint64_t* obs_world,
                              const float* obs_uv_pixels, const float* world_xyz, const uint8_t* cam_frozen,
                              double huber_a, cc_rig** out);
int cc_rigk_set_camera_intrinsics(cc_rig* h, int64_t camera, const double* intr9, uint32_t const_mask);
int cc_rigk_get_camera_intrinsics(cc_rig* h, int64_t camera, double* intr9);
int cc_rigk_set_model(cc_rig* h, int32_t model);
int cc_rigk_get_model(cc_rig* h, int32_t* model);
enum { CC_MODEL_MIXED = 2 };
int cc_rigk_set_camera_model(cc_rig* h, int64_t camera, int32_t model);
int cc_rigk_get_camera_model(cc_rig* h, int64_t camera, int32_t* model);
int cc_rigk_estimate_start(cc_rig* h, const cc_rig_start_options* opt, const double* cam_q, const double* cam_t,
                           const double* frame_q, const double* frame_t, cc_rig_start_report* report);
int cc_rigk_start_points(cc_rig* h, float* uv_normalised, int64_t* n_without_root);
int cc_rigk_estimate_start_bearing(cc_rig* h, const cc_rig_start_options* opt, const double* cam_q, const double* cam_t,
                                   const double* frame_q, const double* frame_t, cc_rig_start_report* report);
int cc_rigk_start_bearings(cc_rig* h, float* bearing_xyz, int64_t* n_without_root);

int cc_rig_optimize(const cc_options* opt, int32_t device, int64_t n_cams, int64_t n_frames,
                    int64_t n_world, const int64_t* obs_frame_offsets, const uint32_t* obs_cam,
                    const uint64_t* obs_world, const float* obs_uv, const float* world_xyz,
                    double* cam_q, double* cam_t, const uint8_t* cam_frozen, double* frame_q,
                    double* frame_t, double huber_a, double* obs_cost, cc_summary* summary);
int cc_rig_estimate(const cc_options* opt, int32_t device, int64_t n_cams, int64_t n_frames,
                    int64_t n_world, const int64_t* obs_frame_offsets, const uint32_t* obs_cam,
                    const uint64_t* obs_world, const float* obs_uv, const float* world_xyz,
                    double* cam_q, double* cam_t, const uint8_t* cam_frozen, double* frame_q,
                    double* frame_t, double huber_a, double* obs_cost, cc_summary* summary);

typedef struct cc_obs_layout {
  int64_t stride, camera_offset, world_offset, uv_offset, cost_offset;
} cc_obs_layout;
int cc_rig_optimize_frames(const cc_options* opt, int32_t device, int64_t n_cams, int64_t n_frames, int64_t n_world,
                           void* const* frame_records, const int64_t* counts, const cc_obs_layout* layout,
                           const float* world_xyz, double* cam_q, double* cam_t, const uint8_t* cam_frozen,
                           double* frame_q, double* frame_t, double huber_a, cc_summary* summary);

typedef struct cc_obs_columns {
  const void* const* camera; int64_t camera_stride; int32_t camera_width;
  const void* const* world;  int64_t world_stride;  int32_t world_width;
  const void* const* uv;     int64_t uv_stride;
  void* const* cost;         int64_t cost_stride;
} cc_obs_columns;
int cc_rig_optimize_columns(const cc_options* opt, int32_t device, int64_t n_cams, int64_t n_frames, int64_t n_world,
                            const cc_obs_columns* columns, const int64_t* counts,
                            const float* world_xyz, double* cam_q, double* cam_t, const uint8_t* cam_frozen,
                            double* frame_q, double* frame_t, double huber_a, cc_summary* summary);

int cc_rig_optimize_multi(const cc_options* opt, int32_t n_devices, const int32_t* devices, int64_t n_cams,
                          int64_t n_frames, int64_t n_world, const int64_t* obs_frame_offsets,
                          const uint32_t* obs_cam, const uint64_t* obs_world, const float* obs_uv,
                          const float* world_xyz, double* cam_q, double* cam_t, const uint8_t* cam_frozen,
                          double* frame_q, double* frame_t, double huber_a, double* obs_cost,
                          cc_summary* summary);

int cc_zhang_init(int32_t device, int64_t n_frames, const int64_t* frame_offsets, const float* uv,
                  const float* xyz, float* K9, float* q_wxyz, float* t_xyz, float* homographies);

int cc_distort(int32_t device, const float* K9, const float* dist5, int64_t n,
               const float* xy_normalized, float* uv_out);
int cc_undistort(int32_t device, const float* K9, const float* dist5, int64_t n, const float* uv,
                 float* xy_out);
int cc_distort_fisheye(int32_t device, const float* K9, const float* dist4, int64_t n,
                       const float* xy_normalized, float* uv_out);
int cc_undistort_fisheye(int32_t device, const float* K9, const float* dist4, int64_t n, const float* uv,
                         float* xy_out);

#ifdef __cplusplus
}
#endif
#endif
```

Baseline: 33.03 billion residuals/s.

## Predict final LM iteration and run residual-only sweep instead of full Jacobian sweep

The control workgroup predicts from the cost-change trend or the iteration limit when the next accepted step is likely the last one, and signals this through a broadcast flag. On that round, teams whose frames fit a bounded pass count evaluate only residuals, reduced with an MFMA-packed sum of squares, and skip the full Jacobian/Gram accumulation and speculative elimination. If the prediction is wrong and the step must continue, the full sweep is redone. This saves one full Jacobian sweep per solve but adds control logic, a possible extra sweep on misprediction, and loss of speculative overlap on that round.

```diff
diff --git a/camera_calibrator_amd/capi.py b/camera_calibrator_amd/capi.py
--- a/camera_calibrator_amd/capi.py
+++ b/camera_calibrator_amd/capi.py
@@ -110,6 +110,7 @@
     "cc_intrinsics_batch_solve", "cc_intrinsics_batch_optimize", "cc_intrinsics_batch_estimate",
     "cc_intrinsics_set_huber", "cc_intrinsics_obs_cost", "cc_intrinsics_optimize_views_huber", "cc_intrinsics_estimate_views_huber",
     "cc_intrinsics_batch_set_huber", "cc_intrinsics_batch_estimate_huber",
+    "cc_intrinsics_set_final_sweep", "cc_intrinsics_final_sweep_counts",
     "cc_intrinsics_set_model", "cc_intrinsics_get_model", "cc_intrinsics_optimize_views_model", "cc_intrinsics_estimate_views_model",
     "cc_distort_fisheye", "cc_undistort_fisheye",
     "cc_intrinsics_batch_set_model", "cc_intrinsics_batch_get_model", "cc_intrinsics_batch_estimate_model",
@@ -275,6 +276,14 @@
 
     def set_huber(self, a):
         _check(lib().cc_intrinsics_set_huber(self._h, C.c_double(a)))
+
+    def set_final_sweep(self, mode):
+        _check(lib().cc_intrinsics_set_final_sweep(self._h, C.c_int32(mode)))
+
+    def final_sweep_counts(self):
+        a, b = C.c_int32(0), C.c_int32(0)
+        _check(lib().cc_intrinsics_final_sweep_counts(self._h, C.byref(a), C.byref(b)))
+        return int(a.value), int(b.value)
 
     def set_model(self, model):
         _check(lib().cc_intrinsics_set_model(self._h, C.c_int32(model)))
diff --git a/camera_calibrator_amd/csrc/cc_intrinsics.hip b/camera_calibrator_amd/csrc/cc_intrinsics.hip
--- a/camera_calibrator_amd/csrc/cc_intrinsics.hip
+++ b/camera_calibrator_amd/csrc/cc_intrinsics.hip
@@ -814,6 +814,7 @@
   cc::PersistDev pq{};
   uint32_t p_epoch = 0;
   size_t p_box_bytes = 0;
+  int final_sweep = 1;
   double huber_a = 0.0;
   int model = CC_MODEL_RADTAN;
   void* start_work = nullptr;
@@ -1117,6 +1118,7 @@
   h->pq.xbox = reinterpret_cast<unsigned long long*>(base + o_xbox);
   h->pq.fail = reinterpret_cast<unsigned*>(base + o_pfail);
   h->pq.lbox = reinterpret_cast<unsigned long long*>(base + o_lbox);
+  h->pq.fs_counts = reinterpret_cast<unsigned*>(base + o_sync + 16);
   h->pq.G = (int32_t)PG;
   h->pq.teams = p_teams;
   h->p_epoch = 0;
@@ -1258,6 +1260,26 @@
   return CC_OK;
 }
 
+int cc_intrinsics_set_final_sweep(cc_intrinsics* h, int32_t mode) {
+  using namespace cc;
+  if (!h) return fail(CC_ERR_BAD_ARGUMENT, "cc_intrinsics_set_final_sweep: NULL handle");
+  if (mode < 0 || mode > 2) return fail(CC_ERR_BAD_ARGUMENT, "cc_intrinsics_set_final_sweep: mode %d is not 0, 1 or 2", (int)mode);
+  h->final_sweep = mode;
+  return CC_OK;
+}
+
+int cc_intrinsics_final_sweep_counts(cc_intrinsics* h, int32_t* residual_only, int32_t* redone) {
+  using namespace cc;
+  if (!h || !residual_only || !redone) return fail(CC_ERR_BAD_ARGUMENT, "cc_intrinsics_final_sweep_counts: NULL argument");
+  CC_HIP(hipSetDevice(h->device));
+  unsigned w[2] = {0u, 0u};
+  CC_HIP(hipMemcpyAsync(w, h->pq.fs_counts, sizeof(w), hipMemcpyDeviceToHost, h->stream));
+  CC_HIP(hipStreamSynchronize(h->stream));
+  *residual_only = (int32_t)w[0];
+  *redone = (int32_t)w[1];
+  return CC_OK;
+}
+
 int cc_intrinsics_set_model(cc_intrinsics* h, int32_t model) {
   using namespace cc;
   if (!h) return fail(CC_ERR_BAD_ARGUMENT, "cc_intrinsics_set_model: NULL handle");
@@ -1395,6 +1417,7 @@
   h->p_epoch += need;
   q.timeout_shift = h->exchange ? 30 : 27;
   q.first_shift = h->exchange ? 30 : 20;
+  q.final_sweep = h->final_sweep;
   static int drop_left = -2;
   const bool drop_control = !h->exchange && persist_test_drop_control("CC_INTR_PERSIST_TEST_NO_CONTROL", &drop_left);
   persist_launch(h->d, q, drop_control, h->stream);
diff --git a/camera_calibrator_amd/csrc/cc_intrinsics_dev.hpp b/camera_calibrator_amd/csrc/cc_intrinsics_dev.hpp
--- a/camera_calibrator_amd/csrc/cc_intrinsics_dev.hpp
+++ b/camera_calibrator_amd/csrc/cc_intrinsics_dev.hpp
@@ -101,6 +101,66 @@
 }
 __device__ __forceinline__ bool gram_entry_held(uint32_t mask, int e) { return (((mask >> (e >> 4)) | (mask >> (e & 15))) & 1u) != 0; }
 
+template <bool ONE_TEAM = false>
+__device__ __forceinline__ void huber_obs_common(const double* k, const double* R, const double* t,
+                                                 double X0, double X1, double X2, ObsCommon& c) {
+#pragma clang fp contract(off)
+  c.a0 = ONE_TEAM ? fma(R[2], X2, fma(R[0], X0, R[1] * X1)) : fma(R[2], X2, fma(R[1], X1, R[0] * X0));
+  c.a1 = ONE_TEAM ? fma(R[5], X2, fma(R[4], X1, R[3] * X0)) : fma(R[5], X2, fma(R[3], X0, R[4] * X1));
+  c.a2 = fma(R[8], X2, fma(R[6], X0, R[7] * X1));
+  const double xc = c.a0 + t[0], yc = c.a1 + t[1], zc = c.a2 + t[2];
+  c.iz = 1.0 / zc;
+  c.x = xc * c.iz;
+  c.y = yc * c.iz;
+  const double k1 = k[4], k2 = k[5], p1 = k[6], p2 = k[7], k3 = k[8];
+  const double xx = c.x * c.x, yy = c.y * c.y;
+  c.xy = c.x * c.y;
+  c.r2 = fma(c.y, c.y, xx);
+  c.r4 = c.r2 * c.r2;
+  c.r6 = c.r4 * c.r2;
+  const double m = fma(k3, c.r6, fma(k2, c.r4, fma(k1, c.r2, 1.0)));
+  c.ax = fma(2.0, xx, c.r2);
+  c.ay = fma(2.0, yy, c.r2);
+  c.xd = fma(p2, c.ax, fma(2.0 * p1, c.xy, c.x * m));
+  c.yd = fma(p1, c.ay, fma(2.0 * p2, c.xy, c.y * m));
+  const double mp2 = 2.0 * fma(3.0 * k3, c.r4, fma(2.0 * k2, c.r2, k1));
+  c.dxx = fma(6.0 * p2, c.x, fma(2.0 * p1, c.y, fma(mp2, xx, m)));
+  c.dxy = fma(2.0 * p2, c.y, fma(2.0 * p1, c.x, mp2 * c.xy));
+  c.dyy = fma(6.0 * p1, c.y, fma(2.0 * p2, c.x, fma(mp2, yy, m)));
+}
+
+__device__ __forceinline__ void huber_row_tail(const ObsCommon& c, double b0, double b1, double b2, double rw, double* v) {
+#pragma clang fp contract(off)
+  v[9] = 2.0 * fma(b2, c.a1, -(b1 * c.a2)); v[10] = 2.0 * fma(b0, c.a2, -(b2 * c.a0)); v[11] = 2.0 * fma(b1, c.a0, -(b0 * c.a1));
+  v[12] = b0; v[13] = b1; v[14] = b2; v[15] = rw;
+}
+
+__device__ __forceinline__ void huber_row_u(const double* k, const ObsCommon& c, double r, double* v, double w) {
+#pragma clang fp contract(off)
+  const double fx = k[0] * w;
+  v[0] = c.xd * w; v[1] = 0.0; v[2] = w; v[3] = 0.0;
+  const double fxx = fx * c.x;
+  v[4] = fxx * c.r2; v[5] = fxx * c.r4; v[6] = fx * 2.0 * c.xy; v[7] = fx * c.ax; v[8] = fxx * c.r6;
+  const double b0 = fx * c.dxx * c.iz, b1 = fx * c.dxy * c.iz, b2 = -fma(b1, c.y, b0 * c.x);
+  huber_row_tail(c, b0, b1, b2, r * w, v);
+}
+
+__device__ __forceinline__ void huber_row_v(const double* k, const ObsCommon& c, double r, double* v, double w) {
+#pragma clang fp contract(off)
+  const double fy = k[1] * w;
+  v[0] = 0.0; v[1] = c.yd * w; v[2] = 0.0; v[3] = w;
+  const double fyy = fy * c.y;
+  v[4] = fyy * c.r2; v[5] = fyy * c.r4; v[6] = fy * c.ay; v[7] = fy * 2.0 * c.xy; v[8] = fyy * c.r6;
+  const double b0 = fy * c.dxy * c.iz, b1 = fy * c.dyy * c.iz, b2 = -fma(b0, c.x, b1 * c.y);
+  huber_row_tail(c, b0, b1, b2, r * w, v);
+}
+
+__device__ __forceinline__ void huber_residuals(const double* k, const ObsCommon& c, double u, double vm, double& ru, double& rv) {
+#pragma clang fp contract(off)
+  ru = fma(k[0], c.xd, k[2]) - u;
+  rv = fma(k[1], c.yd, k[3]) - vm;
+}
+
 __device__ __forceinline__ void intr_huber(double a, double s, double& rho, double& sr) {
   const double b = a * a;
   const double y = rsqrt_pos(s);
diff --git a/camera_calibrator_amd/csrc/cc_intrinsics_huber.hpp b/camera_calibrator_amd/csrc/cc_intrinsics_huber.hpp
--- a/camera_calibrator_amd/csrc/cc_intrinsics_huber.hpp
+++ b/camera_calibrator_amd/csrc/cc_intrinsics_huber.hpp
@@ -4,65 +4,6 @@
 #include "cc_intrinsics_dev.hpp"
 
 namespace cc {
-
-__device__ __forceinline__ void huber_obs_common(const double* k, const double* R, const double* t,
-                                                 double X0, double X1, double X2, ObsCommon& c) {
-#pragma clang fp contract(off)
-  c.a0 = fma(R[2], X2, fma(R[1], X1, R[0] * X0));
-  c.a1 = fma(R[5], X2, fma(R[3], X0, R[4] * X1));
-  c.a2 = fma(R[8], X2, fma(R[6], X0, R[7] * X1));
-  const double xc = c.a0 + t[0], yc = c.a1 + t[1], zc = c.a2 + t[2];
-  c.iz = 1.0 / zc;
-  c.x = xc * c.iz;
-  c.y = yc * c.iz;
-  const double k1 = k[4], k2 = k[5], p1 = k[6], p2 = k[7], k3 = k[8];
-  const double xx = c.x * c.x, yy = c.y * c.y;
-  c.xy = c.x * c.y;
-  c.r2 = fma(c.y, c.y, xx);
-  c.r4 = c.r2 * c.r2;
-  c.r6 = c.r4 * c.r2;
-  const double m = fma(k3, c.r6, fma(k2, c.r4, fma(k1, c.r2, 1.0)));
-  c.ax = fma(2.0, xx, c.r2);
-  c.ay = fma(2.0, yy, c.r2);
-  c.xd = fma(p2, c.ax, fma(2.0 * p1, c.xy, c.x * m));
-  c.yd = fma(p1, c.ay, fma(2.0 * p2, c.xy, c.y * m));
-  const double mp2 = 2.0 * fma(3.0 * k3, c.r4, fma(2.0 * k2, c.r2, k1));
-  c.dxx = fma(6.0 * p2, c.x, fma(2.0 * p1, c.y, fma(mp2, xx, m)));
-  c.dxy = fma(2.0 * p2, c.y, fma(2.0 * p1, c.x, mp2 * c.xy));
-  c.dyy = fma(6.0 * p1, c.y, fma(2.0 * p2, c.x, fma(mp2, yy, m)));
-}
-
-__device__ __forceinline__ void huber_row_tail(const ObsCommon& c, double b0, double b1, double b2, double rw, double* v) {
-#pragma clang fp contract(off)
-  v[9] = 2.0 * fma(b2, c.a1, -(b1 * c.a2)); v[10] = 2.0 * fma(b0, c.a2, -(b2 * c.a0)); v[11] = 2.0 * fma(b1, c.a0, -(b0 * c.a1));
-  v[12] = b0; v[13] = b1; v[14] = b2; v[15] = rw;
-}
-
-__device__ __forceinline__ void huber_row_u(const double* k, const ObsCommon& c, double r, double* v, double w) {
-#pragma clang fp contract(off)
-  const double fx = k[0] * w;
-  v[0] = c.xd * w; v[1] = 0.0; v[2] = w; v[3] = 0.0;
-  const double fxx = fx * c.x;
-  v[4] = fxx * c.r2; v[5] = fxx * c.r4; v[6] = fx * 2.0 * c.xy; v[7] = fx * c.ax; v[8] = fxx * c.r6;
-  const double b0 = fx * c.dxx * c.iz, b1 = fx * c.dxy * c.iz, b2 = -fma(b1, c.y, b0 * c.x);
-  huber_row_tail(c, b0, b1, b2, r * w, v);
-}
-
-__device__ __forceinline__ void huber_row_v(const double* k, const ObsCommon& c, double r, double* v, double w) {
-#pragma clang fp contract(off)
-  const double fy = k[1] * w;
-  v[0] = 0.0; v[1] = c.yd * w; v[2] = 0.0; v[3] = w;
-  const double fyy = fy * c.y;
-  v[4] = fyy * c.r2; v[5] = fyy * c.r4; v[6] = fy * c.ay; v[7] = fy * 2.0 * c.xy; v[8] = fyy * c.r6;
-  const double b0 = fy * c.dxy * c.iz, b1 = fy * c.dyy * c.iz, b2 = -fma(b0, c.x, b1 * c.y);
-  huber_row_tail(c, b0, b1, b2, r * w, v);
-}
-
-__device__ __forceinline__ void huber_residuals(const double* k, const ObsCommon& c, double u, double vm, double& ru, double& rv) {
-#pragma clang fp contract(off)
-  ru = fma(k[0], c.xd, k[2]) - u;
-  rv = fma(k[1], c.yd, k[3]) - vm;
-}
 
 __global__ __launch_bounds__(kSweepThreads, 4) void k_intr_sweep_huber(IntrDev P, int flags, double huber_a) {
   extern __shared__ __attribute__((aligned(16))) char smem_raw[];
diff --git a/camera_calibrator_amd/csrc/cc_intrinsics_persist.hip b/camera_calibrator_amd/csrc/cc_intrinsics_persist.hip
--- a/camera_calibrator_amd/csrc/cc_intrinsics_persist.hip
+++ b/camera_calibrator_amd/csrc/cc_intrinsics_persist.hip
@@ -1,5 +1,6 @@
 #include "cc_intrinsics_persist.hpp"
 #include "cc_persist_dev.hpp"
+#include "cc_persist_pack.hpp"
 #include "cc_persist_publish.hpp"
 #include "cc_persist_sum.hpp"
 
@@ -11,14 +12,15 @@
 enum { TM_Y = 0, TM_POSE = 60, TM_SP = 76, TM_STEP = 84, TM_R = 100, TM_T = 109, TM_KC = 112, TM_STEP2 = 122, TM_XN2 = 123,
        TM_QW = 124, TM_STAT = 128  };
 enum { WG_INTR = 0 , WG_X = 64 , WG_DS = 66 ,
-       WG_SS = 80 , WG_R0 = 96 , WG_OPT = 100 ,
+       WG_SS = 80 , WG_R0 = 96 ,
+       WG_RO = 97 , WG_OPT = 100 ,
        WG_TAB = 104 ,
        WG_TGI = 416 , WG_TZ = 456  };
 
 static_assert(TM_POSE - TM_Y >= 6 * 10 && TM_SP - TM_POSE >= 2 * 8 && TM_STEP - TM_SP >= 6 && TM_R - TM_STEP >= 15 && TM_T - TM_R >= 9 && TM_KC - TM_T >= 3 &&
               TM_STEP2 - TM_KC >= 9 && TM_QW - TM_XN2 >= 1 && TM_STAT - TM_QW >= 4 && TM_STAT + 4 + 9 <= 192,
               "per-team scratch: Y (6 x 10), two poses, pose scale, step (9 + 6), R, t, intrinsics, scalars, statistics row -- inside the 192 doubles persist_lds_doubles gives a team");
-static_assert(WG_X - WG_INTR >= 2 * 16 && WG_DS - WG_X >= 2 && WG_SS - WG_DS >= 9 && WG_R0 - WG_SS >= 9 && WG_OPT - WG_R0 >= 1 && WG_TAB - WG_OPT >= 4 &&
+static_assert(WG_X - WG_INTR >= 2 * 16 && WG_DS - WG_X >= 2 && WG_SS - WG_DS >= 9 && WG_R0 - WG_SS >= 9 && WG_RO - WG_R0 >= 1 && WG_OPT - WG_RO >= 1 && WG_TAB - WG_OPT >= 4 &&
               WG_TZ - WG_TGI >= 80 / 2 && WG_TZ + 80 / 2 <= 512,
               "workgroup scratch: both intrinsics, broadcast (2 + 9), scales, options, tables of the 80-slot row -- inside the 512 doubles of persist_lds_doubles");
 
@@ -211,6 +213,7 @@
   cc_iteration* s_log = reinterpret_cast<cc_iteration*>(lds + 1264);
   int* s_int = reinterpret_cast<int*>(lds + 1296);
   u64* s_seq = reinterpret_cast<u64*>(lds + 1300);
+  double* s_ccprev = lds + 1301;
   const int tid = threadIdx.x, wave = tid >> 6;
   static_assert(sizeof(cc_iteration) <= 32 * 8, "log record scratch");
   if (tid < (int)(sizeof(LmCtl) / 8)) reinterpret_cast<double*>(s_ctl)[tid] = 0.0;
@@ -219,7 +222,7 @@
   if (tid == 48 && P.host_pub) *s_seq = *P.pub_seq + 1ull;
   __syncthreads();
   if (tid < 9) s_intr[tid] = (Q.restart ? P.init_intr : P.intr)[tid];
-  if (tid == 0) s_int[1] = 0;
+  if (tid == 0) { s_int[1] = 0; s_int[3] = 0; s_int[5] = 0; s_int[6] = 0; s_int[7] = 0; *s_ccprev = 0.0; }
   __syncthreads();
   const LmOpts& o = *s_opts;
   const uint32_t mask = P.mask;
@@ -246,6 +249,7 @@
     if (tid == 0) {
       LmCtl c = *s_ctl;
       const int len0 = c.log_len, prev_cur = c.cur & 1, was_valid = c.step_valid;
+      const int ro_now = s_int[3];
       const double prev_radius = c.radius;
       const double* kc0 = s_intr + (c.cur ? 16 : 0);
       const double* kc1 = s_intr + (c.cur ? 0 : 16);
@@ -278,7 +282,22 @@
       *s_ctl = c;
       s_int[1] = c.log_len != len0;
       s_int[2] = phase0 ? (!c.done && c.radius == o.initial_radius)
-                        : (was_valid && !c.done && (c.cur & 1) == (prev_cur ^ 1) && c.radius == persist_spec_radius(prev_radius, o.max_radius));
+                        : (!ro_now && was_valid && !c.done && (c.cur & 1) == (prev_cur ^ 1) && c.radius == persist_spec_radius(prev_radius, o.max_radius));
+      const bool accepted = !phase0 && (c.cur & 1) != prev_cur;
+      if (ro_now) {
+        s_int[6]++;
+        if (!c.done) {
+          if (Q.final_sweep == 1) s_int[5] = 1;
+          if (accepted) s_int[7]++;
+        }
+      }
+      int pred = 0;
+      if (!c.done && s_int[0] && Q.final_sweep != 0 && !s_int[5] && !P.x.on && (phase0 || accepted)) {
+        const double cc_k = phase0 ? 0.0 : s_log->cost_change;
+        pred = Q.final_sweep == 2 || c.iter + 1 >= o.max_iterations || persist_predicts_end(cc_k, *s_ccprev, o.function_tolerance, c.x_cost);
+      }
+      if (accepted) *s_ccprev = s_log->cost_change;
+      s_int[3] = pred;
       s_bc[0] = (double)((c.done ? 1 : 0) | ((c.cur & 1) << 3));
       s_bc[1] = c.radius;
 #pragma unroll
@@ -286,6 +305,7 @@
     }
     __syncthreads();
     const bool hit = s_int[2] != 0;
+    const int pred_flag = s_int[3] ? 32 : 0;
     if (s_ctl->done || !hit) {
       if (tid < 22) ag_st(Q.xbox + tid, granule(e2, s_bc[tid >> 1], tid & 1));
       if (s_ctl->done) break;
@@ -354,7 +374,7 @@
         s_intr[(cur ^ 1) * 16 + lane] = k_l + d;
       }
       if (lane == 0) {
-        s_bc[0] = (double)((go ? 0 : 1) | (go && ok ? 2 : 0) | (hit ? 4 : 0) | (cur << 3));
+        s_bc[0] = (double)((go ? 0 : 1) | (go && ok ? 2 : 0) | (hit ? 4 : 0) | (cur << 3) | pred_flag);
         s_bc[1] = radius;
         s_bc[12] = gmax;
       }
@@ -402,6 +422,7 @@
   }
   if (lane < 32 && failed == 0u) P.intr[lane] = intr_l;
   if (owes_record && lane < kLogWords) reinterpret_cast<u64*>(P.log + (log_len - 1))[lane] = log_l;
+  if (lane < 2) Q.fs_counts[lane] = (unsigned)s_int[6 + lane];
 }
 
 template <int TEAMS>
@@ -449,6 +470,14 @@
     for (int j = 0; j < 9; ++j)
       for (int k = j; k < 9; ++k) { pj[oo] = (unsigned char)j; pk[oo] = (unsigned char)k; ++oo; }
   }
+  if (tid == 34) {
+    bool fits = true;
+    for (int k = 0; k < TEAMS; ++k) {
+      const int64_t fk = (int64_t)blockIdx.x * TEAMS + k;
+      if (fk < P.F && P.off[fk + 1] - P.off[fk] > (int64_t)kPackMaxPasses * kSweepThreads) fits = false;
+    }
+    s_wg[WG_RO] = fits ? 1.0 : 0.0;
+  }
   if (tid >= 64 && tid < 64 + 16) s_wg[WG_X + tid - 64] = 0.0;
   if (tid >= 80 && tid < 80 + 16) s_wg[WG_SS + tid - 80] = 1.0;
   __syncthreads();
@@ -492,12 +521,13 @@
   int cur = 0;
   double radius = 1.0;
   bool step_valid = true, failed = false;
+  bool ends_next = false;
   for (int round = 0; round < Q.max_rounds; ++round) {
     const unsigned e1 = Q.epoch0 + 3u * (unsigned)round + 1u, e2 = e1 + 1u, e3 = e1 + 2u;
     const bool phase0 = round == 0;
     const bool do_sweep = phase0 || step_valid;
     const int dst = phase0 ? cur : (cur ^ 1);
-    d4 acc0, acc1;
+    const bool resid_only = ends_next && do_sweep && __builtin_amdgcn_readfirstlane((int)s_wg[WG_RO]) != 0;
     if (do_sweep) {
       CC_FRESH_TID(tid);
       const int ttid = tid & 255, lane = tid & 63;
@@ -562,6 +592,12 @@
         const double qw = wave_sum(qterm);
         if (lane == 0) sm[TM_QW + twave] = qw;
       }
+    }
+    auto full_sweep = [&](const bool with_stats) {
+    d4 acc0, acc1;
+    {
+      CC_FRESH_TID(tid);
+      const int ttid = tid & 255, lane = tid & 63;
       double R[9], tt[3], kk[9];
 #pragma unroll
       for (int i = 0; i < 9; ++i) R[i] = rfl(sm[TM_R + i]);
@@ -572,6 +608,7 @@
       double* stage = s_stage + wave * kStageDoublesPerWave;
       acc0 = d4{0.0, 0.0, 0.0, 0.0};
       acc1 = d4{0.0, 0.0, 0.0, 0.0};
+      if (npass == 0) { nm = float2{0.f, 0.f}; nX0 = nX1 = nX2 = 0.f; }
       for (int p = 0; p < npass; ++p) {
         const int64_t idx = s0 + (int64_t)p * kSweepThreads + ttid;
         const bool valid = idx < s1;
@@ -584,15 +621,16 @@
           nX0 = P.xyz[ic * 3]; nX1 = P.xyz[ic * 3 + 1]; nX2 = P.xyz[ic * 3 + 2];
         }
         ObsCommon oc;
-        obs_common(kk, R, tt, (double)X0, (double)X1, (double)X2, oc);
-        double v[16];
+        huber_obs_common<TEAMS == 1>(kk, R, tt, (double)X0, (double)X1, (double)X2, oc);
+        double v[16], ru, rv;
         const double wrow = valid ? 1.0 : 0.0;
-        row_u(kk, oc, (double)m.x, v, wrow);
+        huber_residuals(kk, oc, (double)m.x, (double)m.y, ru, rv);
+        huber_row_u(kk, oc, ru, v, wrow);
         stage_row(stage, lane, v);
         wave_lds_fence();
         gram_rows_ahead(stage, lane, acc0, acc1);
         wave_lds_fence();
-        row_v(kk, oc, (double)m.y, v, wrow);
+        huber_row_v(kk, oc, rv, v, wrow);
         stage_row(stage, lane, v);
         wave_lds_fence();
         gram_rows_ahead(stage, lane, acc0, acc1);
@@ -600,7 +638,7 @@
       }
       __syncthreads();
     }
-    if (do_sweep) {
+    {
       CC_FRESH_TID(tid);
       const int ttid = tid & 255, lane = tid & 63;
 #pragma unroll
@@ -608,14 +646,86 @@
       __syncthreads();
       const double g = gram_entry_held(mask, ttid) ? 0.0 : (s_blk[ttid] + s_blk[256 + ttid]) + (s_blk[512 + ttid] + s_blk[768 + ttid]);
       s_G[(team * 2 + dst) * 256 + ttid] = g;
-      if (ttid == 255) {
+      if (with_stats && ttid == 255) {
         sm[TM_STAT + ST_COST] = 0.5 * g;
         sm[TM_STAT + ST_QMODEL] = (sm[TM_QW] + sm[TM_QW + 1]) + (sm[TM_QW + 2] + sm[TM_QW + 3]);
         sm[TM_STAT + ST_STEP2] = sm[TM_STEP2];
         sm[TM_STAT + ST_XNORM2] = sm[TM_XN2];
       }
-      if (phase0 && ttid < 9 * 17 && ttid % 17 == 0) sm[TM_STAT + 4 + ttid / 17] = g;
-      __syncthreads();
+      if (with_stats && phase0 && ttid < 9 * 17 && ttid % 17 == 0) sm[TM_STAT + 4 + ttid / 17] = g;
+      __syncthreads();
+    }
+    };
+    auto resid_sweep = [&]() {
+    {
+      CC_FRESH_TID(tid);
+      const int ttid = tid & 255, lane = tid & 63;
+      double R[9], tt[3], kk[9];
+#pragma unroll
+      for (int i = 0; i < 9; ++i) R[i] = rfl(sm[TM_R + i]);
+#pragma unroll
+      for (int i = 0; i < 3; ++i) tt[i] = rfl(sm[TM_T + i]);
+#pragma unroll
+      for (int i = 0; i < 9; ++i) kk[i] = rfl(sm[TM_KC + i]);
+      for (int p = 0; p < npass; ++p) {
+        const int64_t idx = s0 + (int64_t)p * kSweepThreads + ttid;
+        const bool valid = idx < s1;
+        const float2 m = nm;
+        const float X0 = nX0, X1 = nX1, X2 = nX2;
+        {
+          const int64_t nidx = p + 1 < npass ? idx + kSweepThreads : s0 + ttid;
+          const int64_t ic = nidx < s1 ? nidx : safe0;
+          nm = uv2[ic];
+          nX0 = P.xyz[ic * 3]; nX1 = P.xyz[ic * 3 + 1]; nX2 = P.xyz[ic * 3 + 2];
+        }
+        ObsCommon oc;
+        huber_obs_common<TEAMS == 1>(kk, R, tt, (double)X0, (double)X1, (double)X2, oc);
+        double ru, rv;
+        huber_residuals(kk, oc, (double)m.x, (double)m.y, ru, rv);
+        const double wrow = valid ? 1.0 : 0.0;
+        tstage[pack_write_slot(twave, p, 0, lane)] = ru * wrow;
+        tstage[pack_write_slot(twave, p, 1, lane)] = rv * wrow;
+      }
+      __syncthreads();
+    }
+    {
+      CC_FRESH_TID(tid);
+      const int lane = tid & 63;
+      if (has_frame && twave == (team & 3)) {
+        const int64_t n = s1 - s0, wr = n - (int64_t)(pack_read_chain(lane) >> 1) * 64;
+        const int mine = pack_read_chain(lane) < kPackChains && wr > 0 ? pack_chain_steps((int)((wr + kSweepThreads - 1) / kSweepThreads)) : 0;
+        const int steps = pack_chain_steps((int)((n + kSweepThreads - 1) / kSweepThreads));
+        d4 acc = d4{0.0, 0.0, 0.0, 0.0};
+        for (int s0_ = 0; s0_ < steps; s0_ += kPackStepsPerPass) {
+          double a[kPackStepsPerPass];
+#pragma unroll
+          for (int u = 0; u < kPackStepsPerPass; ++u) {
+            const double v = tstage[pack_read_slot(s0_ + u, lane)];
+            a[u] = s0_ + u < mine ? v : 0.0;
+          }
+          __builtin_amdgcn_sched_barrier(0);
+#pragma unroll
+          for (int u = 0; u < kPackStepsPerPass; ++u) acc = __builtin_amdgcn_mfma_f64_16x16x4f64(a[u], a[u], acc, 0, 0, 0);
+          __builtin_amdgcn_sched_barrier(0);
+        }
+        double c[4];
+#pragma unroll
+        for (int w = 0; w < 4; ++w)
+          c[w] = lane_bcast(acc[pack_diag_reg(2 * w)], pack_diag_lane(2 * w)) + lane_bcast(acc[pack_diag_reg(2 * w + 1)], pack_diag_lane(2 * w + 1));
+        const double g = (c[0] + c[1]) + (c[2] + c[3]);
+        if (lane == 0) {
+          sm[TM_STAT + ST_COST] = 0.5 * g;
+          sm[TM_STAT + ST_QMODEL] = (sm[TM_QW] + sm[TM_QW + 1]) + (sm[TM_QW + 2] + sm[TM_QW + 3]);
+          sm[TM_STAT + ST_STEP2] = sm[TM_STEP2];
+          sm[TM_STAT + ST_XNORM2] = sm[TM_XN2];
+        }
+      }
+      __syncthreads();
+    }
+    };
+    if (do_sweep) {
+      if (resid_only) resid_sweep();
+      else full_sweep(true);
     }
     {
       CC_FRESH_TID(tid);
@@ -767,36 +877,43 @@
       }
     }
     if (wave == 3 && (int)blockIdx.x < kPartialCols)
-      own_columns<THREADS / kPartialCols>(box, Q.lbox, Q.G, (int)blockIdx.x, tag, s_stage + 2048, Q.fail, tid0, (phase0 ? Q.first_shift : Q.timeout_shift));
+      own_columns<THREADS / kPartialCols>(box, Q.lbox, Q.G, (int)blockIdx.x, tag, s_stage + 2048, Q.fail, tid_e, (phase0 ? Q.first_shift : Q.timeout_shift));
     };
     auto wait_bcast = [&](const unsigned tag) {
       CC_FRESH_TID(tid);
-      if (wave == 0 && !bcast_wait(Q.xbox, tag, 11, s_wg + WG_X, Q.fail, tid & 63, (phase0 ? Q.first_shift : Q.timeout_shift))) s_wg[WG_X] = 17.0;
+      if (wave == 0 && !bcast_wait(Q.xbox, tag, 11, s_wg + WG_X, Q.fail, tid & 63, (phase0 ? Q.first_shift : Q.timeout_shift))) {
+        int gave_up = 17;
+        asm volatile("" : "+s"(gave_up));
+        s_wg[WG_X] = (double)gave_up;
+      }
       __syncthreads();
     };
 
-    const bool spec = do_sweep;
+    const bool spec = do_sweep && !ends_next;
     const double radius_spec = phase0 ? s_wg[WG_R0] : persist_spec_radius(radius, s_wg[WG_OPT + 3]);
     if (spec) eliminate_and_post(dst, radius_spec, phase0, Q.pbox, e2);
     wait_bcast(e2);
-    int fl = (int)s_wg[WG_X];
+    int fl = __builtin_amdgcn_readfirstlane((int)s_wg[WG_X]);
     if (fl & 16) failed = true;
     if (fl & 1) { cur = (fl >> 3) & 1; break; }
     if (fl & 4) {
       cur = dst;
-      radius = radius_spec;
+      radius = rfl(radius_spec);
     } else {
       cur = (fl >> 3) & 1;
-      radius = s_wg[WG_X + 1];
+      radius = rfl(s_wg[WG_X + 1]);
+      if (resid_only && cur == dst) full_sweep(false);
       eliminate_and_post(cur, radius, false, Q.rbox, e3);
       wait_bcast(e3);
-      fl = (int)s_wg[WG_X];
+      fl = __builtin_amdgcn_readfirstlane((int)s_wg[WG_X]);
       if (fl & 16) failed = true;
       if (fl & 1) { cur = (fl >> 3) & 1; break; }
     }
     step_valid = (fl & 2) != 0;
-  }
-  if (!failed && ag_ld32(Q.fail) == 0u && has_frame && (tid0 & 255) < 7) P.pose[((size_t)cur * P.F + f) * 8 + (tid0 & 255)] = sm[TM_POSE + cur * 8 + (tid0 & 255)];
+    ends_next = (fl & 32) != 0;
+  }
+  CC_FRESH_TID(tid_w);
+  if (!failed && ag_ld32(Q.fail) == 0u && has_frame && (tid_w & 255) < 7) P.pose[((size_t)cur * P.F + f) * 8 + (tid_w & 255)] = sm[TM_POSE + cur * 8 + (tid_w & 255)];
   asm volatile("" ::"v"(nm.x), "v"(nX0), "v"(nX1), "v"(nX2));
 }
 
diff --git a/camera_calibrator_amd/csrc/cc_intrinsics_persist.hpp b/camera_calibrator_amd/csrc/cc_intrinsics_persist.hpp
--- a/camera_calibrator_amd/csrc/cc_intrinsics_persist.hpp
+++ b/camera_calibrator_amd/csrc/cc_intrinsics_persist.hpp
@@ -23,7 +23,15 @@
   int32_t restart;
   int32_t timeout_shift;
   int32_t first_shift;
+  int32_t final_sweep;
+  unsigned* fs_counts;
 };
+
+inline __host__ __device__ bool persist_predicts_end(double cc_k, double cc_prev, double function_tolerance, double x_cost) {
+  if (!(cc_k > 0.0) || !(cc_prev > 0.0)) return false;
+  const double ratio = cc_k / cc_prev;
+  return cc_k * (ratio < 1.0 ? ratio : 1.0) <= function_tolerance * x_cost;
+}
 
 int persist_resident_workgroups(int device, int teams, int* out);
 void persist_launch(const IntrDev& P, const PersistDev& Q, bool drop_control, hipStream_t stream);
diff --git a/camera_calibrator_amd/csrc/cc_persist_pack.hpp b/camera_calibrator_amd/csrc/cc_persist_pack.hpp
--- /dev/null
+++ b/camera_calibrator_amd/csrc/cc_persist_pack.hpp
@@ -0,0 +1,31 @@
+#pragma once
+
+#ifdef __HIPCC__
+#define CC_PPACK_FN __host__ __device__ __forceinline__
+#else
+#define CC_PPACK_FN inline
+#endif
+
+namespace cc {
+
+constexpr int kPackChains = 8;
+constexpr int kPackStepsPerPass = 16;
+constexpr int kPackSlotsPerStep = 32;
+constexpr int kPackMaxPasses = 8;
+
+CC_PPACK_FN int pack_chain(int wave, int lane) { return 2 * wave + ((lane >> 2) & 1); }
+CC_PPACK_FN int pack_step(int pass, int rs, int lane) { return (2 * pass + rs) * 8 + (lane >> 3); }
+CC_PPACK_FN int pack_sub(int lane) { return lane & 3; }
+CC_PPACK_FN int pack_slot(int step, int k, int chain) { return step * kPackSlotsPerStep + k * kPackChains + chain; }
+CC_PPACK_FN int pack_write_slot(int wave, int pass, int rs, int lane) {
+  return pack_slot(pack_step(pass, rs, lane), pack_sub(lane), pack_chain(wave, lane));
+}
+
+CC_PPACK_FN int pack_read_chain(int lane) { return lane & 15; }
+CC_PPACK_FN int pack_read_slot(int step, int lane) { return pack_slot(step, lane >> 4, lane & (kPackChains - 1)); }
+CC_PPACK_FN int pack_chain_steps(int npass) { return npass * kPackStepsPerPass; }
+
+CC_PPACK_FN int pack_diag_lane(int chain) { return (chain & 3) * 16 + chain; }
+CC_PPACK_FN int pack_diag_reg(int chain) { return chain >> 2; }
+
+}
diff --git a/include/cc_solver.h b/include/cc_solver.h
--- a/include/cc_solver.h
+++ b/include/cc_solver.h
@@ -137,6 +137,8 @@
 int cc_intrinsics_exchange_attach(cc_intrinsics* h, int32_t rank, int32_t nranks, const uint8_t* handles);
 
 int cc_intrinsics_set_huber(cc_intrinsics* h, double a_pixels);
+int cc_intrinsics_set_final_sweep(cc_intrinsics* h, int32_t mode);
+int cc_intrinsics_final_sweep_counts(cc_intrinsics* h, int32_t* residual_only, int32_t* redone);
 int cc_intrinsics_obs_cost(cc_intrinsics* h, double* obs_cost);
 int cc_intrinsics_optimize_views_huber(const cc_options* opt, int32_t device, int64_t n_frames, const float* const* uv_views,
                                        const float* const* xyz_views, const int64_t* counts, double* intr9, uint32_t const_mask,
```

After: 34.96 billion residuals/s, median of 6. 5.9% higher.
